# Mange/raingun

Hardware: AMD Instinct MI355X
Metric: Mrays/sec (primary+shadow+secondary) at 3840×2160, depth 5; 1/2/4/8 MI355X (higher is better)
Workload: dtype f64

## Files before the change

include/raingun_debug.h:

```cpp
#ifndef RAINGUN_DEBUG_H
#define RAINGUN_DEBUG_H

#include "raingun.h"

#ifdef __cplusplus
extern "C" {
#endif

rg_status rg_debug_set_path(rg_scene *scene, int32_t path);

typedef struct rg_bvh_info {
    int32_t built;
    int32_t enabled;
    int32_t nodes;
    int32_t leaves;
    int32_t depth;
    float margin;
    float origin_bound;
    int32_t lane_stack;
    int64_t lbuf_bytes;
} rg_bvh_info;
rg_status rg_debug_set_bvh(rg_scene *scene, int32_t enable);
rg_status rg_debug_bvh_info(const rg_scene *scene, rg_bvh_info *info);

rg_status rg_debug_set_lightbuf(rg_scene *scene, int32_t enable);
int32_t rg_debug_lightbuf_count(const rg_scene *scene);

rg_status rg_debug_set_lane_depth(rg_scene *scene, int32_t min_depth);

rg_status rg_debug_set_tile_order(rg_scene *scene, int32_t mode);

rg_status rg_debug_set_image_bands(rg_scene *scene, int32_t bands);

rg_status rg_debug_set_host_split(rg_scene *scene, int32_t pct);

rg_status rg_debug_fail_split_a(rg_scene *scene, int32_t count);

rg_status rg_debug_set_host_ring(rg_scene *scene, int32_t flush_small, int32_t group_small, int32_t flush_big,
                                 int32_t group_big, int32_t multi_light_one);

rg_status rg_debug_set_host_tile_shape(rg_scene *scene, int32_t tile_wlog);

rg_status rg_debug_set_aa_band_rows(rg_scene *scene, int32_t rows);

rg_status rg_debug_set_aa_adaptive_timing(rg_scene *scene, int32_t enable);
rg_status rg_debug_aa_adaptive_info(const rg_scene *scene, float ms[5], uint32_t *flagged, uint32_t *listed_tiles,
                                    uint32_t *bands_launched);

rg_status rg_debug_set_multi(rg_scene *scene, int32_t mode, int32_t stand_in, int32_t bands, int32_t only_rank);

int rg_debug_gather_noop(const void *send, void *recv, size_t count, int datatype, int root, void *comm,
                         void *stream);

rg_status rg_debug_counters(const rg_scene *scene, uint64_t out[16]);

rg_status rg_debug_counter_words(const rg_scene *scene, int32_t first, int32_t n, uint64_t *out);

rg_status rg_debug_last_plain(const rg_scene *scene, int32_t *plain);

rg_status rg_debug_set_exact_div(rg_scene *scene, int32_t enable);
rg_status rg_debug_camera_check(const rg_scene *scene, uint32_t width, uint32_t height, double fov,
                                uint64_t *mismatches, int32_t *admitted);

rg_status rg_debug_unscaled_check(const rg_scene *scene, int32_t op, const double *a, const double *b, uint32_t n,
                                  uint64_t *mismatches);

#ifdef __cplusplus
}
#endif

#endif
```

raingun_amd/_abi.py:

```python
from __future__ import annotations

import ctypes as C
import os
from pathlib import Path

PKG_DIR = Path(__file__).resolve().parent
REPO_DIR = PKG_DIR.parent
LIB_PATH = PKG_DIR / "libraingun_hip.so"

RG_OK = 0
RG_ERR_INVALID_ARGUMENT = -1
RG_ERR_PORTRAIT = -2
RG_ERR_AABB_NORMAL = -3
RG_ERR_NAN_DISTANCE = -4
RG_ERR_TRANSMISSION = -5
RG_ERR_TEXTURE = -6
RG_ERR_DEVICE = -10
RG_ERR_OUT_OF_MEMORY = -11
RG_ERR_CANCELLED = -12
RG_ERR_COLLECTIVE = -13
RG_ERR_PENDING = -14

BODY_SPHERE, BODY_PLANE, BODY_DISK, BODY_AABB = 0, 1, 2, 3
COLORATION_COLOR, COLORATION_TEXTURE = 0, 1
SURFACE_DIFFUSE, SURFACE_REFLECTING, SURFACE_REFRACTIVE = 0, 1, 2
LIGHT_DIRECTIONAL, LIGHT_SPHERICAL = 0, 1


class rg_material(C.Structure):
    _fields_ = [
        ("coloration", C.c_uint32),
        ("color", C.c_float * 3),
        ("texture", C.c_int32),
        ("x_offset", C.c_float),
        ("y_offset", C.c_float),
        ("albedo", C.c_float),
        ("surface", C.c_uint32),
        ("reflectivity", C.c_float),
        ("index", C.c_float),
        ("transparency", C.c_float),
    ]


class rg_body(C.Structure):
    _fields_ = [
        ("kind", C.c_uint32),
        ("_pad", C.c_uint32),
        ("p", C.c_double * 7),
        ("material", rg_material),
    ]


class rg_light(C.Structure):
    _fields_ = [
        ("kind", C.c_uint32),
        ("color", C.c_float * 3),
        ("intensity", C.c_float),
        ("_pad", C.c_uint32),
        ("v", C.c_double * 3),
    ]


class rg_texture(C.Structure):
    _fields_ = [("width", C.c_uint32), ("height", C.c_uint32), ("rgba", C.POINTER(C.c_uint8))]


class rg_scene_desc(C.Structure):
    _fields_ = [
        ("fov", C.c_double),
        ("default_color", C.c_float * 3),
        ("max_recursion_depth", C.c_uint32),
        ("n_bodies", C.c_uint32),
        ("bodies", C.POINTER(rg_body)),
        ("n_lights", C.c_uint32),
        ("lights", C.POINTER(rg_light)),
        ("n_textures", C.c_uint32),
        ("textures", C.POINTER(rg_texture)),
    ]


class rg_ray_counts(C.Structure):
    _fields_ = [("primary", C.c_uint64), ("shadow", C.c_uint64), ("secondary", C.c_uint64)]

    def as_dict(self) -> dict:
        return {"primary": int(self.primary), "shadow": int(self.shadow), "secondary": int(self.secondary)}

    def total(self) -> int:
        return int(self.primary) + int(self.shadow) + int(self.secondary)


class rg_stats(C.Structure):
    _fields_ = [
        ("rays", rg_ray_counts),
        ("kernel_ms", C.c_float),
        ("error_pixel", C.c_int32),
        ("_pad", C.c_uint32),
    ]


class rg_tiling(C.Structure):
    _fields_ = [("tile_rows", C.c_uint32), ("tile_stride", C.c_uint32), ("tile_offset", C.c_uint32)]


class rg_camera(C.Structure):
    _fields_ = [("eye", C.c_double * 3), ("right", C.c_double * 3), ("up", C.c_double * 3),
                ("forward", C.c_double * 3)]


class rg_aov(C.Structure):
    _fields_ = [("body", C.c_void_p), ("depth", C.c_void_p), ("normal", C.c_void_p), ("uv", C.c_void_p),
                ("albedo", C.c_void_p)]


class rg_bvh_info(C.Structure):
    _fields_ = [("built", C.c_int32), ("enabled", C.c_int32), ("nodes", C.c_int32), ("leaves", C.c_int32),
                ("depth", C.c_int32), ("margin", C.c_float), ("origin_bound", C.c_float), ("lane_stack", C.c_int32),
                ("lbuf_bytes", C.c_int64)]


TILE_CALLBACK = C.CFUNCTYPE(C.c_int32, C.c_uint32, C.c_uint32, C.c_uint32, C.POINTER(C.c_uint8), C.c_void_p)

EXPORTED_SYMBOLS = (
    "rg_abi_version",
    "rg_status_string",
    "rg_device_count",
    "rg_scene_create",
    "rg_scene_destroy",
    "rg_scene_set_max_depth",
    "rg_render_image",
    "rg_render_tiles_async",
    "rg_render_tiles_pipelined",
    "rg_render_tiles",
    "rg_tiling_rows",
    "rg_render_stream",
    "rg_trace",
    "rg_host_register",
    "rg_host_unregister",
    "rg_scene_release_stream",
    "rg_stream_status",
    "rg_render_multi",
    "rg_render_image_aa",
    "rg_render_aa_async",
    "rg_resolve_box",
    "rg_render_image_aa_adaptive",
    "rg_render_aa_adaptive",
    "rg_edge_mask",
    "rg_camera_look_at",
    "rg_scene_set_camera",
    "rg_render_aov",
    "rg_render_aov_async",
)
DEBUG_SYMBOLS = ("rg_debug_set_path", "rg_debug_set_bvh", "rg_debug_bvh_info", "rg_debug_counters",
                 "rg_debug_set_lightbuf", "rg_debug_lightbuf_count",
                 "rg_debug_set_tile_order", "rg_debug_set_lane_depth", "rg_debug_set_image_bands", "rg_debug_set_host_split",
                 "rg_debug_fail_split_a", "rg_debug_set_host_ring", "rg_debug_set_host_tile_shape", "rg_debug_set_multi", "rg_debug_gather_noop",
                 "rg_debug_counter_words", "rg_debug_set_aa_band_rows",
                 "rg_debug_set_aa_adaptive_timing", "rg_debug_aa_adaptive_info", "rg_debug_last_plain",
                 "rg_debug_set_exact_div", "rg_debug_camera_check", "rg_debug_unscaled_check")
FRAMES_SYMBOLS = ("rg_frames_create", "rg_frames_destroy", "rg_frames_step", "rg_frames_flush", "rg_frames_image",
                  "rg_frames_read_image", "rg_frames_status", "rg_frames_set_batch", "rg_frames_set_root_tiles", "rg_comm_id_bytes",
                  "rg_comm_unique_id", "rg_comm_init_rank", "rg_comm_info", "rg_comm_destroy", "rg_comm_gather_fn")
PATH_AUTO, PATH_LIGHT, PATH_HEAVY = -1, 0, 1


class RaingunError(RuntimeError):

    def __init__(self, status: int, what: str = ""):
        self.status = status
        msg = status_string(status) if _LIB is not None else str(status)
        super().__init__(f"{what}: {msg} (status {status})" if what else f"{msg} (status {status})")


_LIB: C.CDLL | None = None


def _declare(lib: C.CDLL) -> None:
    P = C.POINTER
    lib.rg_abi_version.restype = C.c_int32
    lib.rg_status_string.restype = C.c_char_p
    lib.rg_status_string.argtypes = [C.c_int32]
    lib.rg_device_count.restype = C.c_int32
    lib.rg_scene_create.restype = C.c_int32
    lib.rg_scene_create.argtypes = [P(rg_scene_desc), C.c_int32, P(C.c_void_p)]
    lib.rg_scene_destroy.restype = None
    lib.rg_scene_destroy.argtypes = [C.c_void_p]
    lib.rg_scene_set_max_depth.restype = C.c_int32
    lib.rg_scene_set_max_depth.argtypes = [C.c_void_p, C.c_uint32]
    lib.rg_camera_look_at.restype = C.c_int32
    lib.rg_camera_look_at.argtypes = [P(C.c_double), P(C.c_double), P(C.c_double), P(rg_camera)]
    lib.rg_scene_set_camera.restype = C.c_int32
    lib.rg_scene_set_camera.argtypes = [C.c_void_p, P(rg_camera)]
    lib.rg_render_image.restype = C.c_int32
    lib.rg_render_image.argtypes = [C.c_void_p, C.c_uint32, C.c_uint32, C.c_void_p, P(rg_stats)]
    lib.rg_render_tiles_async.restype = C.c_int32
    lib.rg_render_tiles_async.argtypes = [C.c_void_p, C.c_uint32, C.c_uint32, P(rg_tiling), C.c_void_p,
                                          C.c_void_p, C.c_void_p, P(rg_stats)]
    if hasattr(lib, "rg_render_tiles_pipelined"):
        lib.rg_render_tiles_pipelined.restype = C.c_int32
        lib.rg_render_tiles_pipelined.argtypes = [C.c_void_p, C.c_uint32, C.c_uint32, P(rg_tiling), C.c_void_p,
                                                  C.c_void_p, C.c_void_p]
    lib.rg_render_tiles.restype = C.c_int32
    lib.rg_render_tiles.argtypes = [C.c_void_p, C.c_uint32, C.c_uint32, P(rg_tiling), C.c_void_p, C.c_void_p,
                                    P(rg_stats)]
    lib.rg_tiling_rows.restype = C.c_uint32
    lib.rg_tiling_rows.argtypes = [C.c_uint32, P(rg_tiling)]
    lib.rg_render_stream.restype = C.c_int32
    lib.rg_render_stream.argtypes = [C.c_void_p, C.c_uint32, C.c_uint32, C.c_uint32, TILE_CALLBACK, C.c_void_p,
                                     P(rg_stats)]
    lib.rg_debug_set_path.restype = C.c_int32
    lib.rg_debug_set_path.argtypes = [C.c_void_p, C.c_int32]
    lib.rg_debug_set_bvh.restype = C.c_int32
    lib.rg_debug_set_bvh.argtypes = [C.c_void_p, C.c_int32]
    if hasattr(lib, "rg_debug_set_lightbuf"):
        lib.rg_debug_set_lightbuf.restype = C.c_int32
        lib.rg_debug_set_lightbuf.argtypes = [C.c_void_p, C.c_int32]
        lib.rg_debug_lightbuf_count.restype = C.c_int32
        lib.rg_debug_lightbuf_count.argtypes = [C.c_void_p]
    lib.rg_debug_bvh_info.restype = C.c_int32
    lib.rg_debug_bvh_info.argtypes = [C.c_void_p, P(rg_bvh_info)]
    lib.rg_debug_set_tile_order.restype = C.c_int32
    lib.rg_debug_set_tile_order.argtypes = [C.c_void_p, C.c_int32]
    lib.rg_debug_set_lane_depth.restype = C.c_int32
    lib.rg_debug_set_lane_depth.argtypes = [C.c_void_p, C.c_int32]
    lib.rg_debug_set_image_bands.restype = C.c_int32
    lib.rg_debug_set_image_bands.argtypes = [C.c_void_p, C.c_int32]
    if hasattr(lib, "rg_debug_set_host_split"):
        lib.rg_debug_set_host_split.restype = C.c_int32
        lib.rg_debug_set_host_split.argtypes = [C.c_void_p, C.c_int32]
    if hasattr(lib, "rg_debug_set_host_ring"):
        lib.rg_debug_set_host_ring.restype = C.c_int32
        lib.rg_debug_set_host_ring.argtypes = [C.c_void_p] + [C.c_int32] * 5
    if hasattr(lib, "rg_debug_fail_split_a"):
        lib.rg_debug_fail_split_a.restype = C.c_int32
        lib.rg_debug_fail_split_a.argtypes = [C.c_void_p, C.c_int32]
    if hasattr(lib, "rg_debug_set_multi"):
        lib.rg_debug_set_multi.restype = C.c_int32
        lib.rg_debug_set_multi.argtypes = [C.c_void_p, C.c_int32, C.c_int32, C.c_int32, C.c_int32]
    if hasattr(lib, "rg_debug_set_host_tile_shape"):
        lib.rg_debug_set_host_tile_shape.restype = C.c_int32
        lib.rg_debug_set_host_tile_shape.argtypes = [C.c_void_p, C.c_int32]
    lib.rg_debug_counters.restype = C.c_int32
    lib.rg_debug_counters.argtypes = [C.c_void_p, P(C.c_uint64)]
    if hasattr(lib, "rg_debug_counter_words"):
        lib.rg_debug_counter_words.restype = C.c_int32
        lib.rg_debug_counter_words.argtypes = [C.c_void_p, C.c_int32, C.c_int32, P(C.c_uint64)]
    if hasattr(lib, "rg_debug_last_plain"):
        lib.rg_debug_last_plain.restype = C.c_int32
        lib.rg_debug_last_plain.argtypes = [C.c_void_p, P(C.c_int32)]
    if hasattr(lib, "rg_debug_set_exact_div"):
        lib.rg_debug_set_exact_div.restype = C.c_int32
        lib.rg_debug_set_exact_div.argtypes = [C.c_void_p, C.c_int32]
        lib.rg_debug_camera_check.restype = C.c_int32
        lib.rg_debug_camera_check.argtypes = [C.c_void_p, C.c_uint32, C.c_uint32, C.c_double, P(C.c_uint64), P(C.c_int32)]
    if hasattr(lib, "rg_debug_unscaled_check"):
        lib.rg_debug_unscaled_check.restype = C.c_int32
        lib.rg_debug_unscaled_check.argtypes = [C.c_void_p, C.c_int32, C.c_void_p, C.c_void_p, C.c_uint32, P(C.c_uint64)]
    lib.rg_frames_create.restype = C.c_int32
    lib.rg_frames_create.argtypes = [C.c_void_p, C.c_uint32, C.c_uint32, C.c_uint32, C.c_int32, C.c_int32,
                                     C.c_int32, C.c_void_p, C.c_void_p, P(C.c_void_p)]
    lib.rg_frames_destroy.restype = None
    lib.rg_frames_destroy.argtypes = [C.c_void_p]
    lib.rg_frames_step.restype = C.c_int32
    lib.rg_frames_step.argtypes = [C.c_void_p]
    lib.rg_frames_flush.restype = C.c_int32
    lib.rg_frames_flush.argtypes = [C.c_void_p]
    lib.rg_frames_image.restype = C.c_void_p
    lib.rg_frames_image.argtypes = [C.c_void_p]
    lib.rg_frames_read_image.restype = C.c_int32
    lib.rg_frames_read_image.argtypes = [C.c_void_p, C.c_void_p]
    lib.rg_trace.restype = C.c_int32
    lib.rg_trace.argtypes = [C.c_void_p, C.c_void_p, C.c_uint32, C.c_void_p, C.c_void_p]
    lib.rg_host_register.restype = C.c_int32
    lib.rg_host_register.argtypes = [C.c_void_p, C.c_size_t]
    lib.rg_host_unregister.restype = C.c_int32
    lib.rg_host_unregister.argtypes = [C.c_void_p]
    lib.rg_scene_release_stream.restype = C.c_int32
    lib.rg_scene_release_stream.argtypes = [C.c_void_p, C.c_void_p]
    lib.rg_stream_status.restype = C.c_int32
    lib.rg_stream_status.argtypes = [C.c_void_p, C.c_void_p, P(C.c_int32)]
    lib.rg_render_multi.restype = C.c_int32
    lib.rg_render_multi.argtypes = [C.c_void_p, C.c_uint32, C.c_uint32, C.c_int32, C.c_uint32, C.c_void_p,
                                    P(rg_stats)]
    if hasattr(lib, "rg_render_image_aa"):
        lib.rg_render_image_aa.restype = C.c_int32
        lib.rg_render_image_aa.argtypes = [C.c_void_p, C.c_uint32, C.c_uint32, C.c_uint32, C.c_void_p, C.c_void_p,
                                           P(rg_stats)]
        lib.rg_render_aa_async.restype = C.c_int32
        lib.rg_render_aa_async.argtypes = [C.c_void_p, C.c_uint32, C.c_uint32, C.c_uint32, C.c_void_p, C.c_void_p,
                                           C.c_void_p, P(rg_stats)]
        lib.rg_resolve_box.restype = C.c_int32
        lib.rg_resolve_box.argtypes = [C.c_int32, C.c_void_p, C.c_uint32, C.c_uint32, C.c_uint32, C.c_void_p,
                                       C.c_void_p]
        lib.rg_debug_set_aa_band_rows.restype = C.c_int32
        lib.rg_debug_set_aa_band_rows.argtypes = [C.c_void_p, C.c_int32]
    if hasattr(lib, "rg_render_image_aa_adaptive"):
        lib.rg_render_image_aa_adaptive.restype = C.c_int32
        lib.rg_render_image_aa_adaptive.argtypes = [C.c_void_p, C.c_uint32, C.c_uint32, C.c_uint32, C.c_uint32,
                                                    C.c_void_p, C.c_void_p, C.c_void_p, P(rg_stats)]
        lib.rg_render_aa_adaptive.restype = C.c_int32
        lib.rg_render_aa_adaptive.argtypes = [C.c_void_p, C.c_uint32, C.c_uint32, C.c_uint32, C.c_uint32, C.c_void_p,
                                              C.c_void_p, C.c_void_p, C.c_void_p, P(rg_stats)]
        lib.rg_debug_set_aa_adaptive_timing.restype = C.c_int32
        lib.rg_debug_set_aa_adaptive_timing.argtypes = [C.c_void_p, C.c_int32]
        lib.rg_debug_aa_adaptive_info.restype = C.c_int32
        lib.rg_debug_aa_adaptive_info.argtypes = [C.c_void_p, P(C.c_float), P(C.c_uint32), P(C.c_uint32), P(C.c_uint32)]
        lib.rg_edge_mask.restype = C.c_int32
        lib.rg_edge_mask.argtypes = [C.c_int32, C.c_void_p, C.c_uint32, C.c_uint32, C.c_uint32, C.c_void_p,
                                     P(C.c_uint32)]
    if hasattr(lib, "rg_render_aov"):
        lib.rg_render_aov.restype = C.c_int32
        lib.rg_render_aov.argtypes = [C.c_void_p, C.c_uint32, C.c_uint32, P(rg_aov), P(rg_stats)]
        lib.rg_render_aov_async.restype = C.c_int32
        lib.rg_render_aov_async.argtypes = [C.c_void_p, C.c_uint32, C.c_uint32, P(rg_tiling), P(rg_aov), C.c_void_p,
                                            P(rg_stats)]
    lib.rg_frames_status.restype = C.c_int32
    lib.rg_frames_status.argtypes = [C.c_void_p, P(C.c_int32)]
    if hasattr(lib, "rg_frames_set_batch"):
        lib.rg_frames_set_batch.restype = C.c_int32
        lib.rg_frames_set_batch.argtypes = [C.c_void_p, C.c_int32]
    if hasattr(lib, "rg_frames_set_root_tiles"):
        lib.rg_frames_set_root_tiles.restype = C.c_int32
        lib.rg_frames_set_root_tiles.argtypes = [C.c_void_p, C.c_int32]
    if hasattr(lib, "rg_comm_init_rank"):
        lib.rg_comm_id_bytes.restype = C.c_int32
        lib.rg_comm_unique_id.restype = C.c_int32
        lib.rg_comm_unique_id.argtypes = [C.c_void_p]
        lib.rg_comm_init_rank.restype = C.c_int32
        lib.rg_comm_init_rank.argtypes = [C.c_void_p, C.c_int32, C.c_int32, C.c_int32, P(C.c_void_p)]
        lib.rg_comm_info.restype = C.c_int32
        lib.rg_comm_info.argtypes = [C.c_void_p, P(C.c_int32), P(C.c_int32), P(C.c_int32)]
        lib.rg_comm_destroy.restype = C.c_int32
        lib.rg_comm_destroy.argtypes = [C.c_void_p]
        lib.rg_comm_gather_fn.restype = C.c_void_p
        lib.rg_comm_gather_fn.argtypes = []


def lib() -> C.CDLL:
    global _LIB
    if _LIB is None:
        path = os.environ.get("RAINGUN_HIP_LIB") or str(LIB_PATH)
        if not Path(path).exists():
            raise RuntimeError(
                f"{path} is missing: build it with `make -C raingun_amd/csrc` (or __graft_entry__.build()). "
                "There is no CPU fallback for the render path.")
        try:
            import torch
        except ImportError:
            pass
        lib_ = C.CDLL(path)
        _declare(lib_)
        _LIB = lib_
    return _LIB


def status_string(status: int) -> str:
    return lib().rg_status_string(int(status)).decode()


def check(status: int, what: str = "") -> None:
    if status != RG_OK:
        raise RaingunError(status, what)


class HostRegistration:

    def __init__(self, arr):
        self.arr = arr
        check(lib().rg_host_register(arr.ctypes.data, arr.nbytes), "rg_host_register")

    def close(self) -> None:
        if self.arr is not None:
            lib().rg_host_unregister(self.arr.ctypes.data)
            self.arr = None

    def __enter__(self):
        return self.arr

    def __exit__(self, *exc):
        self.close()
```

raingun_amd/csrc/rg_aov.hip:

```cpp
#include <hip/hip_runtime.h>

#include "../../include/raingun.h"
#include "rg_aov_kernel.h"
#include "rg_device.h"
#include "rg_internal.h"
#include "rg_launchers.h"

#pragma clang fp contract(off)

#ifndef RG_AOV_TILE_WLOG
#define RG_AOV_TILE_WLOG 5
#endif
#ifndef RG_AOV_BLOCKS_PER_CU
#define RG_AOV_BLOCKS_PER_CU 16
#endif

namespace {

template <bool CAMERA, bool F32F, bool BVH>
hipError_t launch_shade(const RgKernelArgs *a, const RgAovOut *o, dim3 grid, size_t lds, hipStream_t stream) {
    if (o->normal || o->uv || o->albedo)
        hipLaunchKernelGGL((rg_aov_kernel<CAMERA, F32F, BVH, true>), grid, dim3(RG_AOV_BLOCK), lds, stream, *a, *o);
    else
        hipLaunchKernelGGL((rg_aov_kernel<CAMERA, F32F, BVH, false>), grid, dim3(RG_AOV_BLOCK), lds, stream, *a, *o);
    return hipGetLastError();
}

template <bool CAMERA>
hipError_t launch_flavour(const RgKernelArgs *a, const RgAovOut *o, dim3 grid, size_t lds, hipStream_t stream) {
    if (a->n_nodes > 0) return launch_shade<CAMERA, true, true>(a, o, grid, lds, stream);
    if (rg_heavy_path(*a)) return launch_shade<CAMERA, true, false>(a, o, grid, lds, stream);
    return launch_shade<CAMERA, false, false>(a, o, grid, lds, stream);
}

}

extern "C" hipError_t rg_launch_aov(const RgKernelArgs *a, const RgAovOut *o, hipStream_t stream) {
    if (a->out_rows == 0 || a->width == 0 || a->tile_wlog < 3 || a->tile_wlog > 6) return hipErrorInvalidValue;
    int dev = 0, cus = 0;
    hipError_t e = hipGetDevice(&dev);
    if (e == hipSuccess) e = hipDeviceGetAttribute(&cus, hipDeviceAttributeMultiprocessorCount, dev);
    if (e != hipSuccess) return e;
    const unsigned long long ntiles = rg_tile_count(*a), per_block = RG_AOV_BLOCK / 64u;
    const unsigned long long want = (ntiles + per_block - 1ull) / per_block;
    const unsigned long long cap = (unsigned long long)(cus > 0 ? cus : 1) * RG_AOV_BLOCKS_PER_CU;
    const dim3 grid((unsigned)(want < cap ? want : cap));
    const size_t lds = a->lane_stack > 0 ? ((size_t)(a->lane_stack + 1) * 4u) * RG_AOV_BLOCK : 0u;
    return a->camera ? launch_flavour<true>(a, o, grid, lds, stream) : launch_flavour<false>(a, o, grid, lds, stream);
}

namespace {

bool any_layer(const rg_aov *v) { return v->body || v->depth || v->normal || v->uv || v->albedo; }

RgKernelArgs aov_args(const rg_scene *s, rg_launch_ctx *cx, uint32_t W, uint32_t H, const rg_tiling &t, uint32_t rows) {
    RgKernelArgs a = rg_make_args(s);
    a.counters = cx->counters + (size_t)cx->cur * RG_COUNTER_WORDS;
    a.counters_next = cx->counters + (size_t)(1 - cx->cur) * RG_COUNTER_WORDS;
    a.err_sticky = cx->sticky;
    a.width = W;
    a.height = H;
    a.tile_rows = t.tile_rows;
    a.tile_stride = t.tile_stride;
    a.tile_offset = t.tile_offset;
    a.tile_group = 1u;
    a.out_rows = rows;
    a.width_d = (double)W;
    a.height_d = (double)H;
    a.aspect = a.width_d / a.height_d;
    a.tile_wlog = RG_AOV_TILE_WLOG;
    if (s->has_camera) {
        a.camera = 1u;
        for (int k = 0; k < 3; ++k) {
            a.cam_eye[k] = s->camera.eye[k];
            a.cam_right[k] = s->camera.right[k];
            a.cam_up[k] = s->camera.up[k];
            a.cam_forward[k] = s->camera.forward[k];
        }
    }
    return a;
}

}

extern "C" {

rg_status rg_render_aov_async(const rg_scene *s, uint32_t width, uint32_t height, const rg_tiling *tiling,
                              const rg_aov *dev, void *stream, rg_stats *stats) {
    if (!s || !dev || !any_layer(dev) || width == 0 || height == 0 || !tiling || !rg_tiling_valid(tiling))
        return RG_ERR_INVALID_ARGUMENT;
    if (width < height) return RG_ERR_PORTRAIT;
    const uint32_t rows = rg_tiling_rows(height, tiling);
    if ((unsigned long long)rows * width >= (1ull << 32) || (unsigned long long)height * width >= (1ull << 32))
        return RG_ERR_INVALID_ARGUMENT;
    if (!ok(hipSetDevice(s->device))) return RG_ERR_DEVICE;
    hipStream_t st = static_cast<hipStream_t>(stream);
    rg_launch_ctx *cx = rg_ctx_for(s, st);
    if (!cx) return RG_ERR_OUT_OF_MEMORY;
    s->last = cx;
    RgKernelArgs a = aov_args(s, cx, width, height, *tiling, rows);
    const RgAovOut o{dev->body, dev->depth, dev->normal, dev->uv, dev->albedo};
    cx->last_counters = a.counters;
    cx->last_plain = 0;
    if (stats && !ok(hipEventRecord(cx->ev0, st))) return RG_ERR_DEVICE;
    if (rows > 0) {
        if (!ok(rg_launch_aov(&a, &o, st))) return RG_ERR_DEVICE;
        cx->cur = 1 - cx->cur;
    }
    if (!stats) return RG_OK;
    unsigned long long c[4];
    if (!ok(hipEventRecord(cx->ev1, st)) ||
        !ok(hipMemcpyAsync(c, a.counters, sizeof c, hipMemcpyDeviceToHost, st)) || !ok(hipStreamSynchronize(st)))
        return RG_ERR_DEVICE;
    float ms = 0.0f;
    (void)hipEventElapsedTime(&ms, cx->ev0, cx->ev1);
    stats->kernel_ms = ms;
    return rg_snap_status(c, stats);
}

rg_status rg_render_aov(const rg_scene *s, uint32_t width, uint32_t height, const rg_aov *out, rg_stats *stats) {
    if (!s || !out || !any_layer(out) || width == 0 || height == 0) return RG_ERR_INVALID_ARGUMENT;
    if (width < height) return RG_ERR_PORTRAIT;
    const unsigned long long npx = (unsigned long long)width * height;
    if (npx >= (1ull << 32)) return RG_ERR_INVALID_ARGUMENT;
    if (!ok(hipSetDevice(s->device))) return RG_ERR_DEVICE;
    void *const host[5] = {out->body, out->depth, out->normal, out->uv, out->albedo};
    const size_t px_bytes[5] = {4, 8, 12, 8, 12};
    void *d[5] = {nullptr, nullptr, nullptr, nullptr, nullptr};
    rg_status st = RG_OK;
    for (int k = 0; k < 5 && st == RG_OK; ++k)
        if (host[k] && !ok(hipMalloc(&d[k], (size_t)npx * px_bytes[k]))) {
            (void)hipGetLastError();
            st = RG_ERR_OUT_OF_MEMORY;
        }
    if (st == RG_OK) {
        const rg_aov dev{static_cast<int32_t *>(d[0]), static_cast<double *>(d[1]), static_cast<float *>(d[2]),
                         static_cast<float *>(d[3]), static_cast<float *>(d[4])};
        const rg_tiling whole = {height, 1, 0};
        rg_stats local;
        st = rg_render_aov_async(s, width, height, &whole, &dev, nullptr, stats ? stats : &local);
        if (st == RG_OK || st == RG_ERR_AABB_NORMAL || st == RG_ERR_NAN_DISTANCE)
            for (int k = 0; k < 5; ++k)
                if (host[k] && !ok(hipMemcpy(host[k], d[k], (size_t)npx * px_bytes[k], hipMemcpyDeviceToHost)))
                    st = RG_ERR_DEVICE;
    }
    for (int k = 0; k < 5; ++k)
        if (d[k]) (void)hipFree(d[k]);
    return st;
}

}
```

raingun_amd/csrc/rg_capi.hip:

```cpp
#include <hip/hip_runtime.h>

#include <algorithm>
#include <cstring>

#include "../../include/raingun.h"
#include "../../include/raingun_debug.h"
#include "rg_device.h"
#include "rg_exact.h"
#include "rg_internal.h"
#include "rg_launchers.h"

#pragma clang fp contract(off)

#ifndef RG_LANE_MIN_DEPTH
#define RG_LANE_MIN_DEPTH 1
#endif

void rg_image_res_release(rg_image_res &r) {
    rg_bands_release(r);
    if (r.h_frame) (void)hipHostFree(r.h_frame);
    if (r.h_flags) (void)hipHostFree(r.h_flags);
    if (r.h_cancel) (void)hipHostFree(r.h_cancel);
    r = rg_image_res{};
}
// ... 286 lines not shown

rg_status rg_render_stream(const rg_scene *s, uint32_t width, uint32_t height, uint32_t tile_rows,
                           rg_tile_callback on_tile, void *user, rg_stats *stats) {
    if (!s || !on_tile || width == 0 || height == 0 || tile_rows == 0) return RG_ERR_INVALID_ARGUMENT;
    if (width < height) return RG_ERR_PORTRAIT;
    if ((unsigned long long)height * width >= (1ull << 32)) return RG_ERR_INVALID_ARGUMENT;
    if (!ok(hipSetDevice(s->device))) return RG_ERR_DEVICE;
    rg_status st = ensure_image_res(s, 1);
    if (st != RG_OK) return st;
    rg_image_res &r = s->img;
    const size_t row4 = (size_t)width * 4, bytes = (size_t)height * row4;
    const uint32_t wl = (uint32_t)s->host_tile_wlog;
    const auto [TH, tiles_x, grid_rows, ntiles] = host_tile_grid(width, height, wl);
    (void)grid_rows;
    size_t cancel_cap = r.h_cancel ? 64 : 0;
    if ((st = rg_grow(RG_MEM_PINNED_ZEROED, r.h_frame, r.h_frame_cap, bytes + 4)) != RG_OK ||
        (st = rg_grow(RG_MEM_PINNED_ZEROED, r.h_flags, r.h_flags_cap, (ntiles + 1) * 4)) != RG_OK ||
        (st = rg_grow(RG_MEM_PINNED_ZEROED, r.h_cancel, cancel_cap, 64)) != RG_OK)
        return st;
    void *frame_dev = rg_host_device_ptr(r.h_frame, bytes);
    uint32_t *flags_dev = static_cast<uint32_t *>(rg_host_device_ptr(r.h_flags, ntiles * 4 + 4));
    const uint32_t *cancel_dev = static_cast<const uint32_t *>(rg_host_device_ptr(r.h_cancel, 4));
    if (!frame_dev || !flags_dev || !cancel_dev) return RG_ERR_DEVICE;
    __atomic_store_n(r.h_cancel, 0u, __ATOMIC_RELEASE);
    if (++r.seq == 0) r.seq = 1;
    const uint32_t seq = r.seq;
    hipStream_t rs = r.rs[0];
    const rg_tiling whole = {height, 1, 0};
    if (!ok(hipEventRecord(r.ev_t0, rs))) return RG_ERR_DEVICE;
    rg_launch_desc d = frame_launch(width, height, whole, frame_dev, rs, r.h_snap);
    d.tile_flags = flags_dev;
    d.frame_seq = seq;
    d.cancel = cancel_dev;
    d.tile_wlog = wl;
    d.host_frame = true;
    st = rg_launch_tiles(s, d);
    if (st != RG_OK) return rg_bands_drain(r, st);
    if (!ok(hipEventRecord(r.ev_t1, rs))) return rg_bands_drain(r, RG_ERR_DEVICE);
    const uint8_t *frame = static_cast<const uint8_t *>(r.h_frame);
    for (uint32_t y0 = 0; y0 < height; y0 += tile_rows) {
        const uint32_t n = std::min(tile_rows, height - y0);
        if ((st = wait_tiles(r.h_flags, (size_t)(y0 / TH) * tiles_x, ((size_t)(y0 + n) + TH - 1u) / TH * tiles_x, seq,
                             r.ev_t1)) != RG_OK)
            break;
        if (on_tile(y0, n, width, frame + (size_t)y0 * row4, user) != 0) {
            __atomic_store_n(r.h_cancel, 1u, __ATOMIC_RELEASE);
            st = RG_ERR_CANCELLED;
            break;
        }
    }
    if (!ok(hipStreamSynchronize(rs))) return rg_bands_drain(r, RG_ERR_DEVICE);
    const rg_status err = rg_finish_stats(r.h_snap, 1, r.ev_t0, r.ev_t1, stats);
    if (st == RG_OK && err != RG_OK) return err;
    return st;
}

rg_status rg_debug_set_path(rg_scene *s, int32_t path) {
    if (!s || path < RG_PATH_AUTO || path > RG_PATH_HEAVY) return RG_ERR_INVALID_ARGUMENT;
    s->path = path;
    return RG_OK;
}

rg_status rg_debug_set_bvh(rg_scene *s, int32_t enable) {
    if (!s || (enable != 0 && enable != 1)) return RG_ERR_INVALID_ARGUMENT;
    s->bvh_enabled = enable != 0;
    return RG_OK;
}

rg_status rg_debug_set_lightbuf(rg_scene *s, int32_t enable) {
    if (!s || (enable != 0 && enable != 1)) return RG_ERR_INVALID_ARGUMENT;
    s->lbuf_enabled = enable != 0;
    return RG_OK;
}

int32_t rg_debug_lightbuf_count(const rg_scene *s) {
    if (!s || !s->host || !s->bvh_enabled || !s->lbuf_enabled || s->n_nodes == 0) return 0;
    int32_t n = 0;
    for (int32_t i = 0; i < s->n_lbuf; ++i) n += s->host->lbuf[(size_t)i].kind != RG_LB_NONE;
    return n;
}

rg_status rg_debug_bvh_info(const rg_scene *s, rg_bvh_info *info) {
    if (!s || !info) return RG_ERR_INVALID_ARGUMENT;
    *info = s->bvh_info;
    info->enabled = s->bvh_enabled && s->n_nodes > 0;
    return RG_OK;
}

rg_status rg_debug_set_lane_depth(rg_scene *s, int32_t min_depth) {
    if (!s) return RG_ERR_INVALID_ARGUMENT;
    s->lane_min_depth = min_depth < 0 ? RG_LANE_MIN_DEPTH : min_depth;
    return RG_OK;
}

rg_status rg_debug_set_tile_order(rg_scene *s, int32_t mode) {
    if (!s || mode < -1 || mode > 1) return RG_ERR_INVALID_ARGUMENT;
    s->tile_order = mode;
    return RG_OK;
}

rg_status rg_debug_set_image_bands(rg_scene *s, int32_t bands) {
    if (!s || bands < -2 || bands > RG_IMAGE_MAX_BANDS) return RG_ERR_INVALID_ARGUMENT;
    s->image_bands = bands;
    return RG_OK;
}

rg_status rg_debug_set_host_split(rg_scene *s, int32_t pct) {
    if (!s || pct < 0 || pct > 99) return RG_ERR_INVALID_ARGUMENT;
    s->host_split_pct = pct;
    return RG_OK;
}

rg_status rg_debug_set_host_ring(rg_scene *s, int32_t flush_small, int32_t group_small, int32_t flush_big,
                                  int32_t group_big, int32_t multi_light_one) {
    if (!s || flush_small < -1 || flush_small > 16 || group_small < -1 || flush_big < -1 || flush_big > 16 ||
        group_big < -1 || multi_light_one < -1 || multi_light_one > 1)
        return RG_ERR_INVALID_ARGUMENT;
    if (flush_small >= 0) s->ring_flush_small = flush_small;
    if (group_small >= 0) s->ring_group_small = group_small;
    if (flush_big >= 0) s->ring_flush_big = flush_big;
    if (group_big >= 0) s->ring_group_big = group_big;
    if (multi_light_one >= 0) s->multi_light_one = multi_light_one != 0;
    return RG_OK;
}

rg_status rg_debug_fail_split_a(rg_scene *s, int32_t count) {
    if (!s || count < 0) return RG_ERR_INVALID_ARGUMENT;
    s->split_fail_a = count;
    return RG_OK;
}

rg_status rg_debug_set_host_tile_shape(rg_scene *s, int32_t tile_wlog) {
    if (!s || !(tile_wlog == 0 || (tile_wlog >= 3 && tile_wlog <= 6))) return RG_ERR_INVALID_ARGUMENT;
    s->host_tile_wlog = tile_wlog == 0 ? RG_HOST_TILE_WLOG : tile_wlog;
    s->host_tile_forced = tile_wlog != 0;
    return RG_OK;
}

rg_status rg_debug_counters(const rg_scene *s, uint64_t out[16]) {
    if (!s || !out) return RG_ERR_INVALID_ARGUMENT;
    if (!ok(hipSetDevice(s->device))) return RG_ERR_DEVICE;
    if (!ok(hipStreamSynchronize(s->last->stream)) ||
        !ok(hipMemcpy(out, s->last->last_counters, 16 * sizeof(uint64_t), hipMemcpyDeviceToHost)))
        return RG_ERR_DEVICE;
    return RG_OK;
}

rg_status rg_debug_last_plain(const rg_scene *s, int32_t *plain) {
    if (!s || !plain || !s->last) return RG_ERR_INVALID_ARGUMENT;
    *plain = s->last->last_plain;
    return RG_OK;
}

rg_status rg_debug_set_exact_div(rg_scene *s, int32_t enable) {
    if (!s || (enable != 0 && enable != 1)) return RG_ERR_INVALID_ARGUMENT;
    s->exact_div = enable != 0;
    return RG_OK;
}

rg_status rg_debug_camera_check(const rg_scene *s, uint32_t width, uint32_t height, double fov, uint64_t *mismatches,
                                int32_t *admitted) {
    if (!s || !mismatches || width == 0 || height == 0 || (unsigned long long)width * height >= (1ull << 32))
        return RG_ERR_INVALID_ARGUMENT;
    if (!ok(hipSetDevice(s->device))) return RG_ERR_DEVICE;
    RgKernelArgs a = rg_make_args(s);
    a.width = width;
    a.height = height;
    a.width_d = (double)width;
    a.height_d = (double)height;
    a.aspect = a.width_d / a.height_d;
    a.fov_adjustment = rg_fov_adjustment(fov);
    a.inv_w = 1.0 / a.width_d;
    a.inv_h = 1.0 / a.height_d;
    if (admitted)
        *admitted = rg_recip_div_ok(width) && rg_recip_div_ok(height) && rg_camera_unscaled_ok(a.fov_adjustment, a.aspect);
    unsigned long long *d_bad = nullptr, bad = 0;
    if (!ok(hipMalloc(&d_bad, sizeof bad))) return RG_ERR_OUT_OF_MEMORY;
    rg_status st = RG_OK;
    if (!ok(hipMemset(d_bad, 0, sizeof bad)) || !ok(rg_launch_camera_check(&a, d_bad, nullptr)) ||
        !ok(hipMemcpy(&bad, d_bad, sizeof bad, hipMemcpyDeviceToHost)))
        st = RG_ERR_DEVICE;
    (void)hipFree(d_bad);
    *mismatches = bad;
    return st;
}

rg_status rg_debug_unscaled_check(const rg_scene *s, int32_t op, const double *a, const double *b, uint32_t n,
                                  uint64_t *mismatches) {
    if (!s || !a || !mismatches || n == 0 || n > (1u << 24) || op < 0 || op > 3 || (op == 2 && !b))
        return RG_ERR_INVALID_ARGUMENT;
    if (!ok(hipSetDevice(s->device))) return RG_ERR_DEVICE;
    const size_t bytes = (size_t)n * sizeof(double);
    double *d_a = nullptr, *d_b = nullptr, *d_out = nullptr;
    unsigned long long *d_bad = nullptr, bad = 0;
    rg_status st = RG_OK;
    if (!ok(hipMalloc(&d_a, bytes)) || (op == 2 && !ok(hipMalloc(&d_b, bytes))) || !ok(hipMalloc(&d_out, 2 * bytes)) ||
        !ok(hipMalloc(&d_bad, sizeof bad)))
        st = RG_ERR_OUT_OF_MEMORY;
    else if (!ok(hipMemcpy(d_a, a, bytes, hipMemcpyHostToDevice)) ||
             (op == 2 && !ok(hipMemcpy(d_b, b, bytes, hipMemcpyHostToDevice))) || !ok(hipMemset(d_out, 0, 2 * bytes)) ||
             !ok(hipMemset(d_bad, 0, sizeof bad)) || !ok(rg_launch_unscaled_check(op, d_a, d_b, n, d_out, d_bad, nullptr)) ||
             !ok(hipMemcpy(&bad, d_bad, sizeof bad, hipMemcpyDeviceToHost)))
        st = RG_ERR_DEVICE;
    (void)hipFree(d_a);
    (void)hipFree(d_b);
    (void)hipFree(d_out);
    (void)hipFree(d_bad);
    *mismatches = bad;
    return st;
}

rg_status rg_debug_counter_words(const rg_scene *s, int32_t first, int32_t n, uint64_t *out) {
    if (!s || !out || first < 0 || n < 0 || first + n > RG_COUNTER_WORDS) return RG_ERR_INVALID_ARGUMENT;
    if (!ok(hipSetDevice(s->device))) return RG_ERR_DEVICE;
    if (!ok(hipStreamSynchronize(s->last->stream)) ||
        !ok(hipMemcpy(out, s->last->last_counters + first, (size_t)n * sizeof(uint64_t), hipMemcpyDeviceToHost)))
        return RG_ERR_DEVICE;
    return RG_OK;
}

rg_status rg_trace(const rg_scene *s, const double *rays, uint32_t n, double *dist, int32_t *body) {
    if (!s || (n && (!rays || !dist || !body))) return RG_ERR_INVALID_ARGUMENT;
    if (n == 0) return RG_OK;
    if (!ok(hipSetDevice(s->device))) return RG_ERR_DEVICE;
    void *d_rays = nullptr, *d_dist = nullptr, *d_body = nullptr;
    rg_status st = RG_OK;
    if (!ok(hipMalloc(&d_rays, (size_t)n * 48)) || !ok(hipMalloc(&d_dist, (size_t)n * 8)) ||
        !ok(hipMalloc(&d_body, (size_t)n * 4)))
        st = RG_ERR_OUT_OF_MEMORY;
    rg_launch_ctx *cx = rg_ctx_for(s, nullptr);
    if (!cx) st = RG_ERR_OUT_OF_MEMORY;
    RgKernelArgs a = rg_make_args(s);
    unsigned long long c[4] = {0, 0, 0, 0};
    unsigned long long *cs = cx ? cx->counters + (size_t)cx->cur * RG_COUNTER_WORDS : nullptr;
    if (st == RG_OK) { s->last = cx; a.counters = cs; }
    if (st == RG_OK && (!ok(hipMemcpy(d_rays, rays, (size_t)n * 48, hipMemcpyHostToDevice)) ||
                        !ok(hipMemset(cs, 0, sizeof c)) ||
                        !ok(rg_launch_trace(&a, (const double *)d_rays, n, (double *)d_dist, (int32_t *)d_body, nullptr)) ||
                        !ok(hipMemcpy(dist, d_dist, (size_t)n * 8, hipMemcpyDeviceToHost)) ||
                        !ok(hipMemcpy(body, d_body, (size_t)n * 4, hipMemcpyDeviceToHost)) ||
                        !ok(hipMemcpy(c, cs, sizeof c, hipMemcpyDeviceToHost)) ||
                        !ok(hipMemset(cs, 0, RG_COUNTER_WORDS * sizeof(unsigned long long)))))
        st = RG_ERR_DEVICE;
    if (d_rays) (void)hipFree(d_rays);
    if (d_dist) (void)hipFree(d_dist);
    if (d_body) (void)hipFree(d_body);
    if (st == RG_OK && c[3] != 0) st = rg_snap_status(c, nullptr);
    return st;
}

}
```

raingun_amd/csrc/rg_device.h:

```cpp
#pragma once
#include <stdint.h>

#if !defined(__HIP__) && !defined(__HIPCC__)
#define __device__
#define __host__
#define __forceinline__ inline
#endif

#ifdef __HIP_DEVICE_COMPILE__
#define RG_CONST __attribute__((address_space(4)))
#else
#define RG_CONST
#endif
template <class T>
__device__ __forceinline__ const RG_CONST T *rg_cptr(const T *p) { return (const RG_CONST T *)p; }

struct alignas(16) RgSph { double cx, cy, cz, r2; };
struct alignas(16) RgSphF { float cx, cy, cz, r2hi; };
struct alignas(16) RgSphF2 { float cchi, thrp, cc32; int32_t id; };
struct alignas(16) RgPln { double ox, oy, oz, nx, ny, nz, on, pad; };
struct alignas(16) RgDsk { double ox, oy, oz, nx, ny, nz, r, on; };
struct alignas(16) RgBox { double lo[3], hi[3]; };

struct alignas(16) RgBvhNode {
    float lox[4], loy[4], loz[4], hix[4], hiy[4], hiz[4];
    int32_t child[4];
    int32_t nchild;
    int32_t pad[3];
};

#define RG_LANE_NODE_BITS 12
#define RG_LANE_STACK_MAX 16

struct RgBodyDev {
    int32_t kind;
    int32_t pad;
    double p[7];
};

struct RgMatDev {
    int32_t coloration;
    float color[3];
    int32_t tex;
    float xoff, yoff;
    float albedo_pi;
    int32_t surface;
    float reflectivity;
    float index;
    float transparency;
};

struct RgLightDev {
    int32_t kind;
    float color[3];
    float intensity;
    int32_t pad;
    double v[3];
    double dn[3];
    double pad2;
};

struct RgLightBufDev;

struct RgTexDev {
    const uint32_t *texels;
    int32_t w, h;
};

struct RgTexMagic {
    uint32_t mw, shw, mh, shh;
};
struct RgPlnAxes {
    double xa[3], ya[3];
};

struct RgKernelArgs {
    const RgSph *sph;
    const double *sph_cc;
    const RgSphF *sphf;
    const RgSphF2 *sphf2;
    const int32_t *sph_id;
    const RgPln *pln;
    const int32_t *pln_id;
    const RgDsk *dsk;
    const int32_t *dsk_id;
    const RgBox *box;
    const int32_t *box_id;
    int32_t n_sph, n_pln, n_dsk, n_box;
    const RgBvhNode *nodes;
    int32_t n_nodes;
    int32_t lane_stack;
    int32_t lane_min_depth;
    float bvh_obound;
    double bvh_rbound;
    double bvh_margin;
    double bvh_extent;
    const RgBodyDev *bodies;
    const RgMatDev *mats;
    const RgLightDev *lights;
    const RgTexDev *texs;
    int32_t n_bodies, n_lights, n_textures;
    uint32_t lds_lstack_bytes;
    uint32_t lds_sphf, lds_sph, lds_cc, lds_nodes, lds_pln, lds_dsk, lds_box, lds_bodies, lds_mats, lds_lights, lds_texs, lds_hot_bytes, lds_total_bytes;
    int32_t path;
    uint32_t width, height;
    uint32_t tile_rows, tile_stride, tile_offset, out_rows;
    uint32_t tile_group;
    uint32_t tile_base;
    double fov_adjustment;
    double aspect;
    float def[3];
    uint32_t max_depth;
    uint32_t *rgba;
    float *rgb;
    const uint32_t *tile_perm;
    unsigned long long *counters;
    unsigned long long *counters_next;
    void *deep_stack;
    uint32_t deep_stride;
    int32_t nan_scene;
    unsigned long long *err_sticky;
    uint32_t *tile_flags;
    uint32_t frame_seq;
    const uint32_t *cancel;
    uint32_t tile_wlog;
    uint32_t defer_px;
    const double *prim_sx, *prim_sy;
    uint32_t pipelined;
    double width_d, height_d;
    unsigned long long *snap_out;
    uint32_t max_grid_threads;
    uint32_t image_rows;
    uint32_t out_tile_mul, out_tile_add;
    const void *lds_blob;
    const RgLightBufDev *lbuf;
    const uint32_t *lb_start;
    const uint32_t *lb_ent;
    int32_t n_lbuf;
    int32_t lb_cam;
    uint32_t lds_lbuf;
    uint32_t ring_flush, ring_group;
    const uint8_t *px_mask;
    uint32_t tile_limit, px_k, px_w;
    uint32_t plain_veto;
    double inv_w, inv_h;
    uint32_t tiles_x_m, tiles_x_sh, tile_rows_shift, tile_rows_m, tile_rows_sh, rows_identity;
    uint32_t lds_texm, lds_axes, lds_plain_bytes;
    uint32_t camera;
    double cam_eye[3], cam_right[3], cam_up[3], cam_forward[3];
};

__host__ __device__ inline uint32_t rg_tile_w(const RgKernelArgs &a) { return 1u << a.tile_wlog; }
__host__ __device__ inline uint32_t rg_tile_h(const RgKernelArgs &a) { return 64u >> a.tile_wlog; }
__host__ __device__ inline uint32_t rg_tiles_x(const RgKernelArgs &a) { return (a.width + rg_tile_w(a) - 1u) >> a.tile_wlog; }
__host__ __device__ inline uint32_t rg_tiles_y(const RgKernelArgs &a) { return (a.out_rows + rg_tile_h(a) - 1u) / rg_tile_h(a); }
__host__ __device__ inline unsigned long long rg_tile_count(const RgKernelArgs &a) {
    return (unsigned long long)rg_tiles_x(a) * rg_tiles_y(a);
}

#define RG_FRAME_BYTES 88

#ifndef RG_RING_FLUSH_SMALL
#define RG_RING_FLUSH_SMALL 4
#endif
#ifndef RG_RING_GROUP_SMALL
#define RG_RING_GROUP_SMALL 1
#endif
#ifndef RG_RING_FLUSH_BIG
#define RG_RING_FLUSH_BIG 8
#endif
#ifndef RG_RING_GROUP_BIG
#define RG_RING_GROUP_BIG 8
#endif
#ifndef RG_RING_BIG_TILES
#define RG_RING_BIG_TILES 50000u
#endif
#ifndef RG_MULTI_LIGHT_ONE
#define RG_MULTI_LIGHT_ONE 1
#endif
#ifndef RG_LB
#define RG_LB 3
#endif
#ifndef RG_LB_SMALL
#define RG_LB_SMALL 2
#endif
#ifndef RG_LB_ONE
#define RG_LB_ONE 1
#endif
#ifndef RG_HEAVY_WPS
#define RG_HEAVY_WPS 3
#endif
#define RG_BVH_MAX_WAVES 16
#ifndef RG_HEAVY_SCENE_BODIES
#define RG_HEAVY_SCENE_BODIES 32
#endif

#define RG_PATH_AUTO -1
#define RG_PATH_LIGHT 0
#define RG_PATH_HEAVY 1

__host__ __device__ __forceinline__ bool rg_heavy_path(const RgKernelArgs &a) {
    bool heavy = a.n_sph + a.n_pln + a.n_dsk + a.n_box >= RG_HEAVY_SCENE_BODIES;
    if (a.path != RG_PATH_AUTO) heavy = a.path == RG_PATH_HEAVY;
    if (a.n_lights > RG_LB) heavy = true;
    return heavy;
}

#define RG_COUNTER_WORDS (16 + 16 * 16 + 16)
#define RG_DONE_WORD (16 + 16 * 16)
```

raingun_amd/csrc/rg_internal.h:

```cpp
#pragma once
#include <hip/hip_runtime.h>

#include <cstddef>
#include <cstring>
#include <initializer_list>
#include <memory>
#include <vector>

#include "../../include/raingun.h"
#include "../../include/raingun_debug.h"
#include "rg_bands.h"
#include "rg_copy_pool.h"
#include "rg_device.h"
#include "rg_lightbuf_ray.h"
#include "rg_tile_deal.h"

inline bool ok(hipError_t e) { return e == hipSuccess; }

struct rg_launch_ctx {
    hipStream_t stream = nullptr;
    unsigned long long *counters = nullptr;
    int cur = 0;
    unsigned long long *last_counters = nullptr;
    int last_plain = 0;
    unsigned long long *sticky = nullptr;
    uint32_t *tile_cost = nullptr, *tile_perm = nullptr;
    size_t tile_cap = 0;
    struct PermKey {
        uint32_t width, height, tile_rows, tile_stride, tile_offset, tile_base, out_rows, tile_wlog, max_depth, n_lights,
            tile_group;
        double fov;
        const void *mats;
        bool camera = false;
        double cam[12] = {};
        bool operator==(const PermKey &o) const {
            if (camera != o.camera || std::memcmp(cam, o.cam, sizeof cam) != 0) return false;
            return width == o.width && height == o.height && tile_rows == o.tile_rows && tile_stride == o.tile_stride &&
                   tile_offset == o.tile_offset && tile_base == o.tile_base && out_rows == o.out_rows &&
                   tile_group == o.tile_group &&
                   tile_wlog == o.tile_wlog && max_depth == o.max_depth &&
                   n_lights == o.n_lights && fov == o.fov && mats == o.mats;
        }
    };
    bool perm_valid = false;
    PermKey perm_key{};
    void *deep = nullptr;
    size_t deep_bytes = 0;
    double *prim = nullptr;
    size_t prim_cap = 0;
    uint32_t prim_w = 0, prim_h = 0;
    double prim_fov = 0.0;
    uint32_t rdiv_w = 0, rdiv_h = 0;
    bool rdiv_ok = false;
    hipEvent_t ev0 = nullptr, ev1 = nullptr;
};

#ifndef RG_IMAGE_STREAM_CUMASK
#define RG_IMAGE_STREAM_CUMASK 1
#endif
#ifndef RG_HOST_TILE_WLOG_LIGHT
#define RG_HOST_TILE_WLOG_LIGHT 6
#endif
#ifndef RG_HOST_TILE_WLOG
#define RG_HOST_TILE_WLOG 4
#endif
struct rg_image_res : rg_band_res {
    void *h_frame = nullptr;
    size_t h_frame_cap = 0;
    uint32_t *h_flags = nullptr;
    size_t h_flags_cap = 0;
    uint32_t seq = 0;
    uint32_t *h_cancel = nullptr;
};

#define RG_AA_MAX_SAMPLES 8
struct rg_aa_res : rg_band_res {
    hipEvent_t ev_fork = nullptr;
    void *slot_rgba[2] = {nullptr, nullptr};
    void *slot_rgb[2] = {nullptr, nullptr};
    size_t slot_cap[2] = {0, 0};
    hipStream_t base_stream = nullptr;
    hipEvent_t ev_list = nullptr;
    uint8_t *d_mask = nullptr;
    size_t d_mask_cap = 0;
    uint32_t *d_list = nullptr;
    size_t d_list_cap = 0;
    uint32_t *d_counts = nullptr;
    size_t d_counts_cap = 0;
    uint32_t *h_counts = nullptr;
    size_t h_counts_cap = 0;
    bool timing = false;
    std::vector<hipEvent_t> ev_mark;
    size_t n_marks = 0;
    float pass_ms[5] = {0, 0, 0, 0, 0};
    uint32_t flagged = 0, listed_tiles = 0, bands_launched = 0;
};

struct rg_host_tables {
    std::vector<RgSph> sph;
    std::vector<RgSphF> sphf;
    std::vector<RgSphF2> sphf2;
    std::vector<double> sph_cc;
    std::vector<int32_t> sph_id, pln_id, dsk_id, box_id;
    std::vector<RgPln> pln;
    std::vector<RgDsk> dsk;
    std::vector<RgBox> box;
    std::vector<RgBodyDev> bodies;
    std::vector<RgMatDev> mats;
    std::vector<RgLightDev> lights;
    std::vector<RgBvhNode> nodes;
    std::vector<RgLightBufDev> lbuf;
    std::vector<uint32_t> lb_start, lb_ent;
    std::vector<uint32_t> tex_w, tex_h;
    std::vector<std::vector<uint32_t>> texels;
};

struct rg_multi_res;
struct rg_frames;

struct rg_scene {
    int device = 0;
    double fov = 90.0;
    float def[3] = {0, 0, 0};
    uint32_t max_depth = 10;
    int32_t n_sph = 0, n_pln = 0, n_dsk = 0, n_box = 0, n_bodies = 0, n_lights = 0, n_textures = 0;
    bool nan_scene = false;
    std::vector<void *> allocations;
    RgSph *sph = nullptr;
    double *sph_cc = nullptr;
    RgSphF *sphf = nullptr;
    RgSphF2 *sphf2 = nullptr;
    int32_t path = RG_PATH_AUTO;
    int32_t *sph_id = nullptr, *pln_id = nullptr, *dsk_id = nullptr, *box_id = nullptr;
    RgPln *pln = nullptr;
    RgDsk *dsk = nullptr;
    RgBox *box = nullptr;
    RgBodyDev *bodies = nullptr;
    RgMatDev *mats = nullptr;
    RgLightDev *lights = nullptr;
    RgTexDev *texs = nullptr;
    RgBvhNode *nodes = nullptr;
    int32_t n_nodes = 0;
    int32_t lane_stack = 0;
    int32_t lane_min_depth = 1;
    bool bvh_enabled = true;
    RgLightBufDev *lbuf = nullptr;
    uint32_t *lb_start = nullptr, *lb_ent = nullptr;
    int32_t n_lbuf = 0;
    int32_t lb_cam = -1;
    int32_t n_lbdesc = 0;
    bool lbuf_enabled = true;
    bool exact_div = true;
    bool has_camera = false;
    rg_camera camera{};
    float bvh_obound = 0.0f;
    double bvh_rbound = 0.0, bvh_margin = 0.0, bvh_extent = 0.0;
    rg_bvh_info bvh_info{};
    int tile_order = -1;
    int image_bands = 0;
    int host_split_pct = 0;
    mutable int split_fail_a = 0;
    int ring_flush_small = RG_RING_FLUSH_SMALL, ring_group_small = RG_RING_GROUP_SMALL;
    int ring_flush_big = RG_RING_FLUSH_BIG, ring_group_big = RG_RING_GROUP_BIG;
    bool multi_light_one = RG_MULTI_LIGHT_ONE != 0;
    int host_tile_wlog = RG_HOST_TILE_WLOG;
    bool host_tile_forced = false;
    int multi_mode = 0;
    bool multi_stand_in = false;
    int multi_bands = 0;
    int multi_only_rank = -1;
    std::shared_ptr<const rg_host_tables> host;
    std::vector<RgTexDev> tex_desc;
    void *lds_blob = nullptr;
    uint32_t lds_blob_layout[14] = {};
    mutable std::vector<rg_launch_ctx *> ctxs;
    mutable rg_launch_ctx *last = nullptr;
    mutable rg_image_res img;
    int aa_band_rows = 0;
    mutable rg_aa_res aa;
    mutable rg_multi_res *multi = nullptr;
    mutable std::vector<rg_frames *> frames;
};

void rg_frames_detach_scene(rg_frames *f);

RgKernelArgs rg_make_args(const rg_scene *s);

struct rg_launch_desc {
    uint32_t width = 0, height = 0;
    rg_tiling tiling{};
    uint8_t *rgba = nullptr;
    float *rgb = nullptr;
    hipStream_t stream = nullptr;
    unsigned long long *snap = nullptr;
    bool timed = false;
    uint32_t *tile_flags = nullptr;
    uint32_t frame_seq = 0;
    const uint32_t *cancel = nullptr;
    uint32_t tile_wlog = 3;
    bool host_frame = false;
    bool pipelined = false;
    bool image_rows = false;
    uint32_t tile_first = 0, tile_count = 0xFFFFFFFFu;
    uint32_t tile_group = 1;
    const uint32_t *tile_list = nullptr;
    uint32_t tile_limit = 0;
    const uint8_t *px_mask = nullptr;
    uint32_t px_k = 1, px_w = 0;
};

rg_status rg_launch_tiles(const rg_scene *s, const rg_launch_desc &d, rg_launch_ctx **ctx_out = nullptr);

rg_status rg_snap_status(const unsigned long long *snap, rg_stats *stats);

rg_status rg_render_host(const rg_scene *s, uint32_t width, uint32_t height, const rg_tiling *tiling,
                         uint8_t *rgba_out, float *rgb_out, rg_stats *stats);

bool rg_host_is_pinned(const void *p, size_t bytes);
void *rg_host_device_ptr(void *p, size_t bytes);

rg_status rg_scene_replica(const rg_scene *src, int32_t device, rg_scene **out);
void rg_scene_free(rg_scene *s);
void rg_sync_settings(rg_scene *dst, const rg_scene *src);

void rg_multi_release(const rg_scene *s);

#pragma GCC visibility push(hidden)

rg_launch_ctx *rg_ctx_for(const rg_scene *s, hipStream_t stream);
void rg_ctx_destroy(rg_launch_ctx *c);

enum rg_mem { RG_MEM_DEVICE, RG_MEM_PINNED, RG_MEM_PINNED_ZEROED };
struct rg_grow_buf {
    void **p;
    size_t bytes;
    template <class T>
    rg_grow_buf(T *&q, size_t n) : p(reinterpret_cast<void **>(&q)), bytes(n) {}
};
rg_status rg_grow(rg_mem kind, size_t &cap, size_t want, std::initializer_list<rg_grow_buf> bufs,
                  bool clear_error = true);
template <class T>
rg_status rg_grow(rg_mem kind, T *&p, size_t &cap, size_t bytes) {
    return rg_grow(kind, cap, bytes, {{p, bytes}});
}

double rg_fov_adjustment(double fov);
bool rg_scene_heavy(const rg_scene *s);
const void *rg_lds_blob_for(const rg_scene *s, const RgKernelArgs &a);

uint32_t rg_host_tile_wlog(const rg_scene *s);
void rg_image_res_release(rg_image_res &r);
void rg_aa_res_release(rg_aa_res &r);

hipError_t rg_launch_pack_rgb(const void *rgba, void *rgb, size_t npx, hipStream_t stream);
hipError_t rg_launch_reinterleave(const void *gathered, const void *root_part, void *image, uint32_t width,
                                  uint32_t height, uint32_t tile_rows, uint32_t world, size_t slot_bytes,
                                  hipStream_t stream, uint32_t root = 1);

#pragma GCC visibility pop
```

raingun_amd/csrc/rg_k_trace.h:

```cpp
#pragma once
#include <hip/hip_runtime.h>

#include "rg_bvh_ray.h"
#include "rg_device.h"
#include "rg_k_bvh.h"
#include "rg_k_intersect.h"
#include "rg_k_math.h"

#pragma clang fp contract(off)

namespace rgk {

template <bool F32F, bool BVH, bool NODB = false, class Src>
__device__ __forceinline__ void trace_primary(const RgKernelArgs &a, const Src &src, V3 d, Closest &c) {
    if constexpr (!BVH) sph_primary<F32F>(a, src, d, c);
    [[maybe_unused]] LbRange cam{0u, 0u, false};
    if constexpr (BVH) {
        if (a.lb_cam >= 0) cam = lbuf_begin(a, src, a.lb_cam, d, 0.0, 0.0, 0.0);
    }
    for (int i = 0; i < a.n_pln; ++i) {
        RG_REGION(RGR_PRIM_PLANE);
        const RgPln p = src.getp(i);
        double den = (p.nx * d.x + p.ny * d.y) + p.nz * d.z;
        if (den > 1e-6) {
            RG_REGION(RGR_PRIM_PLANE_DIV);
            double dist = p.on / den;
            if (dist >= 0.0) closest_add(c, dist, rg_cptr(a.pln_id)[i]);
        }
    }
    [[maybe_unused]] const V3 o = v3(0.0, 0.0, 0.0);
    if constexpr (!NODB) {
    for (int i = 0; i < a.n_dsk; ++i) {
        RG_REGION(RGR_DISK);
        const RgDsk k = src.getd(i);
        double t;
        if (disk_hit(k, o, d, t)) closest_add(c, t, rg_cptr(a.dsk_id)[i]);
    }
    if (a.n_box > 0) {
        RG_REGION(RGR_BOX);
        V3 inv = v3(1.0 / d.x, 1.0 / d.y, 1.0 / d.z);
        int sx = inv.x < 0.0, sy = inv.y < 0.0, sz = inv.z < 0.0;
        for (int i = 0; i < a.n_box; ++i) {
            RG_REGION(RGR_BOX);
            const RgBox b = src.getb(i);
            double t;
            if (aabb_hit(b, o, inv, sx, sy, sz, t)) closest_add(c, t, rg_cptr(a.box_id)[i]);
        }
    }
    }
    if constexpr (BVH) {
        const bool ok = !c.nan && rg_bvh_ray_ok(a.bvh_obound, 0.0, 0.0, 0.0, d.x, d.y, d.z);
        RG_STAT(8, RG_LANES(!ok));
        if (!ok) {
            [[maybe_unused]] const unsigned long long t0 = RG_CLOCK();
            sph_primary<F32F>(a, src, d, c);
            RG_STAT(13, RG_CLOCK() - t0);
        }
        const bool walk = ok && !cam.use;
        if (ok && cam.use) cambuf_primary(a, src, cam, d, (float)d.x, (float)d.y, (float)d.z, c);
        if (walk) {
            bool need = true, unused = false;
            bvh_spheres<0>(a, src, o, d, false, 0.0, 0.0, c, unused, need);
        }
    }
}

template <bool F32F, bool BVH, bool NODB = false, class Src>
__device__ __forceinline__ void trace_query(const RgKernelArgs &a, const Src &src, const Ray &r, bool shadow, double ld,
                                            Closest &c, bool &occl, bool lane_walk = false, int light = -1) {
    const V3 o = r.o, d = r.d;
    bool need = true;
    if constexpr (!BVH) {
        if (!sph_query<F32F>(a, src, o, d, shadow, ld, c, occl, need)) return;
    }
    [[maybe_unused]] LbRange lbr{0u, 0u, false};
    if constexpr (BVH) {
        if (shadow && light >= 0 && light < a.n_lbuf) {
            const V3 lp = lbuf_light_pos(src, light);
            lbr = lbuf_begin(a, src, light, o, lp.x, lp.y, lp.z);
        }
    }
    for (int i = 0; i < a.n_pln; ++i) {
        const RgPln p = src.getp(i);
        double den = (p.nx * d.x + p.ny * d.y) + p.nz * d.z;
        RG_REGION(RGR_QC_PLANE);
        if (den > 1e-6 && need) {
            double vx = p.ox - o.x, vy = p.oy - o.y, vz = p.oz - o.z;
            double dist = ((vx * p.nx + vy * p.ny) + vz * p.nz) / den;
            if (dist >= 0.0) {
                if (shadow) {
                    if (!(dist > ld)) { occl = true; need = false; }
                } else {
                    closest_add(c, dist, rg_cptr(a.pln_id)[i]);
                }
            }
        }
    }
    if constexpr (NODB && !BVH) return;
    if (!__any(need)) return;
    if constexpr (!NODB) {
    for (int i = 0; i < a.n_dsk; ++i) {
        RG_REGION(RGR_DISK);
        const RgDsk k = src.getd(i);
        double t;
        if (need && disk_hit(k, o, d, t)) {
            if (shadow) {
                if (!(t > ld)) { occl = true; need = false; }
            } else {
                closest_add(c, t, rg_cptr(a.dsk_id)[i]);
            }
        }
    }
    if (a.n_box > 0 && __any(need)) {
        RG_REGION(RGR_BOX);
        V3 inv = v3(1.0 / d.x, 1.0 / d.y, 1.0 / d.z);
        int sx = inv.x < 0.0, sy = inv.y < 0.0, sz = inv.z < 0.0;
        for (int i = 0; i < a.n_box; ++i) {
            RG_REGION(RGR_BOX);
            const RgBox b = src.getb(i);
            double t;
            if (need && aabb_hit(b, o, inv, sx, sy, sz, t)) {
                if (shadow) {
                    if (!(t > ld)) { occl = true; need = false; }
                } else {
                    closest_add(c, t, rg_cptr(a.box_id)[i]);
                }
            }
        }
    }
    }
    if constexpr (BVH) {
        if (!__any(need)) return;
        double t0s = 0.0;
        float grow = 0.0f;
        const int cls = (need && !c.nan) ? rg_bvh_classify(a.bvh_obound, a.bvh_rbound, a.bvh_margin, a.bvh_extent,
                                                           o.x, o.y, o.z, d.x, d.y, d.z, t0s, grow)
                                         : RG_BVH_SCAN;
        const bool lb = shadow && need && cls == RG_BVH_TRAVERSE && grow == 0.0f && lbr.use;
        if (lb) lbuf_shadow(a, src, light, lbr, o, d, ld, occl, need);
        const bool ok = need && cls == RG_BVH_TRAVERSE && !lb;
#ifdef RG_BVH_STATS
        {
            RG_STAT(8, RG_LANES(need && cls == RG_BVH_SCAN));
            RG_STAT(9, RG_LANES(need && cls == RG_BVH_TRAVERSE && grow > 0.0f));
            RG_STAT(10, RG_LANES(need && cls == RG_BVH_NO_SPHERE));
            RG_STAT(11, RG_LANES(need && c.nan));
        }
#endif
        if (need && cls == RG_BVH_SCAN) {
            [[maybe_unused]] const unsigned long long t0 = RG_CLOCK();
            bool nd = true;
            sph_query<F32F>(a, src, o, d, shadow, ld, c, occl, nd);
            RG_STAT(13, RG_CLOCK() - t0);
        }
        const bool grown = ok && grow > 0.0f;
        const bool per_lane = ok && !grown && a.lane_stack > 0 && __any(ok && !grown && lane_walk);
        if (per_lane) bvh_lane(a, src, o, d, shadow, ld, t0s, c, occl, need);
        if (ok && !grown && !per_lane) {
            bvh_spheres<1>(a, src, o, d, shadow, ld, t0s, c, occl, need);
        }
        if (grown) {
            bvh_spheres<1, true>(a, src, o, d, shadow, ld, t0s, c, occl, need, grow);
        }
    }
}

__device__ __forceinline__ bool ray_exotic(V3 o, V3 d) {
    const bool ok = fabs(o.x) < 1e100 && fabs(o.y) < 1e100 && fabs(o.z) < 1e100 && fabs(d.x) < 1e50 &&
                    fabs(d.y) < 1e50 && fabs(d.z) < 1e50;
    return !ok;
}

#ifndef RG_SHADOW_GROUP
#define RG_SHADOW_GROUP 2
#endif

template <int LB>
struct ShadowBatch {
    V3 d[LB];
    double ld[LB];
};

template <int LB, bool NODB = false, class Src>
__device__ __forceinline__ void trace_shadow(const RgKernelArgs &a, const Src &src, V3 o, const ShadowBatch<LB> &sb,
                                             uint32_t full, uint32_t &occl) {
    constexpr int G = RG_SHADOW_GROUP;
    const int n = a.n_sph, nfull = n - n % G;
    for (int i = 0; i < n;) {
        const int g = i < nfull ? G : 1;
        RG_REGION(RGR_SH_GROUP);
        RgSph s[G];
        double hx[G], hy[G], hz[G], hh[G], adj[G][LB], opp[G][LB];
        bool cand[G][LB];
        bool any = false;
#pragma unroll
        for (int k = 0; k < G; ++k) {
            if (k < g) {
                s[k] = src.get(i + k);
                hx[k] = s[k].cx - o.x; hy[k] = s[k].cy - o.y; hz[k] = s[k].cz - o.z;
                hh[k] = (hx[k] * hx[k] + hy[k] * hy[k]) + hz[k] * hz[k];
#pragma unroll
                for (int l = 0; l < LB; ++l) {
                    adj[k][l] = (hx[k] * sb.d[l].x + hy[k] * sb.d[l].y) + hz[k] * sb.d[l].z;
                    opp[k][l] = hh[k] - adj[k][l] * adj[k][l];
                    cand[k][l] = !(opp[k][l] > s[k].r2) && !((occl >> l) & 1u);
                    any |= cand[k][l];
                }
            }
        }
        if (any) {
            RG_REGION(RGR_SH_TAIL);
#pragma unroll
            for (int k = 0; k < G; ++k) {
#pragma unroll
                for (int l = 0; l < LB; ++l) {
                    double t;
#ifdef RG_REGION_STATS
                    if (k < g && cand[k][l]) RG_REGION(RGR_SH_PAIR);
#endif
                    if (k < g && cand[k][l] && sphere_tail(s[k].r2, opp[k][l], adj[k][l], t) && !(t > sb.ld[l]))
                        occl |= 1u << l;
                }
            }
        }
        i += g;
        if ((i & 7) == 0 && !__any(occl != full)) return;
    }
    if (!__any(occl != full)) return;
    for (int i = 0; i < a.n_pln; ++i) {
        const RgPln p = src.getp(i);
        const double vx = p.ox - o.x, vy = p.oy - o.y, vz = p.oz - o.z;
        const double num = (vx * p.nx + vy * p.ny) + vz * p.nz;
        RG_REGION(RGR_SH_PLANE);
#pragma unroll
        for (int l = 0; l < LB; ++l) {
            const double den = (p.nx * sb.d[l].x + p.ny * sb.d[l].y) + p.nz * sb.d[l].z;
            if (den > 1e-6 && !((occl >> l) & 1u)) {
                bool hit;
                if (sb.ld[l] == __builtin_inf() && num >= 0.0) {
                    hit = true;
                } else {
                    RG_REGION(RGR_SH_PLANE_DIV);
                    const double dist = num / den;
                    hit = dist >= 0.0 && !(dist > sb.ld[l]);
                }
                if (hit) occl |= 1u << l;
            }
        }
    }
    if constexpr (NODB) return;
    if (!__any(occl != full)) return;
    for (int i = 0; i < a.n_dsk; ++i) {
        RG_REGION(RGR_DISK);
        const RgDsk k = src.getd(i);
#pragma unroll
        for (int l = 0; l < LB; ++l) {
            double t;
            if (!((occl >> l) & 1u) && disk_hit(k, o, sb.d[l], t) && !(t > sb.ld[l])) occl |= 1u << l;
        }
    }
    if (a.n_box > 0 && __any(occl != full)) {
        RG_REGION(RGR_BOX);
#pragma unroll
        for (int l = 0; l < LB; ++l) {
            const V3 d = sb.d[l];
            const V3 inv = v3(1.0 / d.x, 1.0 / d.y, 1.0 / d.z);
            const int sx = inv.x < 0.0, sy = inv.y < 0.0, sz = inv.z < 0.0;
            for (int i = 0; i < a.n_box; ++i) {
                RG_REGION(RGR_BOX);
                const RgBox b = src.getb(i);
                double t;
                if (!((occl >> l) & 1u) && aabb_hit(b, o, inv, sx, sy, sz, t) && !(t > sb.ld[l])) occl |= 1u << l;
            }
        }
    }
}

}
```

raingun_amd/csrc/rg_launch.hip:

```cpp
#include <hip/hip_runtime.h>

#include <algorithm>
#include <cstddef>
#include <cstring>
#include <new>
#include <vector>

#include "../../include/raingun.h"
#include "../../include/raingun_debug.h"
#include "rg_device.h"
#include "rg_exact.h"
#include "rg_internal.h"
#include "rg_launchers.h"

#pragma clang fp contract(off)

namespace {

int frames_needed(uint32_t max_depth) { return max_depth > 1 ? (int)max_depth - 1 : 1; }

rg_status decode_error(unsigned long long word, int32_t *pixel) {
    if (word == 0) return RG_OK;
    const unsigned long long key = ~word;
    if (pixel) *pixel = (int32_t)(key >> 8);
// ... 28 lines not shown
    a.counters_next = cx->counters + (size_t)(1 - cx->cur) * RG_COUNTER_WORDS;
    a.err_sticky = cx->sticky;
    a.width = d.width;
    a.height = d.height;
    a.tile_rows = d.tiling.tile_rows;
    a.tile_stride = d.tiling.tile_stride;
    a.tile_offset = d.tiling.tile_offset;
    a.tile_group = d.tile_group;
    a.tile_base = d.tile_first;
    a.out_rows = out_rows;
    a.aspect = (double)d.width / (double)d.height;
    a.width_d = (double)d.width;
    a.height_d = (double)d.height;
    if (cx->rdiv_w != d.width || cx->rdiv_h != d.height) {
        cx->rdiv_ok = rg_recip_div_ok(d.width) && rg_recip_div_ok(d.height);
        cx->rdiv_w = d.width;
        cx->rdiv_h = d.height;
    }
    a.inv_w = 1.0 / a.width_d;
    a.inv_h = 1.0 / a.height_d;
    a.plain_veto = (cx->rdiv_ok && s->exact_div) ? 0u : 1u;
    if (s->has_camera) {
        a.camera = 1u;
        for (int k = 0; k < 3; ++k) {
            a.cam_eye[k] = s->camera.eye[k];
            a.cam_right[k] = s->camera.right[k];
            a.cam_up[k] = s->camera.up[k];
            a.cam_forward[k] = s->camera.forward[k];
        }
        a.plain_veto |= 4u;
    }
    a.rgba = reinterpret_cast<uint32_t *>(d.rgba);
    a.rgb = d.rgb;
    a.tile_flags = d.tile_flags;
    a.frame_seq = d.frame_seq;
    a.cancel = d.cancel;
    a.tile_wlog = d.tile_wlog;
    a.defer_px = d.host_frame ? 1u : 0u;
    a.image_rows = d.image_rows ? 1u : 0u;
    a.pipelined = d.pipelined ? 1u : 0u;
    if (d.px_mask) {
        a.px_mask = d.px_mask;
        a.px_k = d.px_k;
        a.px_w = d.px_w;
        a.tile_perm = d.tile_list;
        a.tile_limit = d.tile_limit;
    }
    if (d.host_frame) {
        const bool big = rg_tile_count(a) >= RG_RING_BIG_TILES;
        a.ring_flush = (uint32_t)std::max(0, big ? s->ring_flush_big : s->ring_flush_small);
        a.ring_group = (uint32_t)std::max(0, big ? s->ring_group_big : s->ring_group_small);
    }
    const RgMagicU32 mx = rg_magic_u32(rg_tiles_x(a)), mr = rg_magic_u32(a.tile_rows);
    a.tiles_x_m = mx.m;
    a.tiles_x_sh = mx.sh;
    a.tile_rows_m = mr.m;
    a.tile_rows_sh = mr.sh;
    a.tile_rows_shift = 32u;
    for (uint32_t k = 0; k < 32u; ++k)
        if (a.tile_rows == 1u << k) a.tile_rows_shift = k;
    a.rows_identity = (a.tile_stride == 1u && a.tile_offset == 0u && a.tile_base == 0u && a.tile_group <= 1u &&
                       a.out_tile_mul <= 1u)
                          ? 1u
                          : 0u;
    return a;
}

rg_status size_deep_frames(rg_launch_ctx *cx, RgKernelArgs &a, int frames, int disp) {
    if (!rg_launch_global_frames(&a, disp) || a.out_rows == 0) return RG_OK;
    size_t threads = 0;
    if (!ok(rg_render_grid_threads(&a, disp, &threads)) || threads == 0 || threads > 0xFFFFFFFFull)
        return RG_ERR_DEVICE;
    const size_t per_thread = (size_t)frames * RG_FRAME_BYTES;
    if (threads * per_thread > ((size_t)1 << 30)) {
        size_t free_b = 0, total_b = 0;
        if (!ok(hipMemGetInfo(&free_b, &total_b))) return RG_ERR_DEVICE;
        const size_t budget = std::min<size_t>(free_b / 2, (size_t)16 << 30);
        if (threads * per_thread > budget) {
            a.max_grid_threads = (uint32_t)std::min<size_t>(budget / per_thread, 0xFFFFFFFFu);
            if (!ok(rg_render_grid_threads(&a, disp, &threads)) || threads == 0) return RG_ERR_DEVICE;
            if (threads * per_thread > budget) return RG_ERR_OUT_OF_MEMORY;
        }
    }
    const rg_status st = rg_grow(RG_MEM_DEVICE, cx->deep, cx->deep_bytes, threads * per_thread);
    if (st != RG_OK) return st;
    a.deep_stack = cx->deep;
    a.deep_stride = (uint32_t)threads;
    return RG_OK;
}

rg_status refresh_prim_table(rg_launch_ctx *cx, RgKernelArgs &a, hipStream_t st) {
    const uint32_t width = a.width, height = a.height;
    if (cx->prim_w != width || cx->prim_h != height || cx->prim_fov != a.fov_adjustment || !cx->prim) {
        const size_t n = (size_t)width + height;
        const rg_status g = rg_grow(RG_MEM_DEVICE, cx->prim, cx->prim_cap, n * sizeof(double));
        if (g != RG_OK) return g;
        std::vector<double> tab(n);
        for (uint32_t x = 0; x < width; ++x)
            tab[x] = ((((double)x + 0.5) / (double)width) * 2.0 - 1.0) * a.aspect * a.fov_adjustment;
        for (uint32_t y = 0; y < height; ++y)
            tab[(size_t)width + y] = (1.0 - (((double)y + 0.5) / (double)height) * 2.0) * a.fov_adjustment;
        if (!ok(hipMemcpyAsync(cx->prim, tab.data(), n * sizeof(double), hipMemcpyHostToDevice, st)) ||
            !ok(hipStreamSynchronize(st)))
            return RG_ERR_DEVICE;
        cx->prim_w = width;
        cx->prim_h = height;
        cx->prim_fov = a.fov_adjustment;
    }
    a.prim_sx = cx->prim;
    a.prim_sy = cx->prim + width;
    return RG_OK;
}

rg_status order_tiles(const rg_scene *s, const rg_launch_desc &d, rg_launch_ctx *cx, RgKernelArgs &a) {
    if (!(s->tile_order == 1 || (s->tile_order < 0 && rg_heavy_path(a)))) return RG_OK;
    const size_t ntiles = (size_t)rg_tile_count(a);
    rg_launch_ctx::PermKey key{d.width, d.height, d.tiling.tile_rows, d.tiling.tile_stride,
                               d.tiling.tile_offset, d.tile_first, a.out_rows, d.tile_wlog, s->max_depth,
                               (uint32_t)s->n_lights, d.tile_group, a.fov_adjustment, s->mats};
    key.camera = a.camera != 0;
    for (int k = 0; key.camera && k < 3; ++k) {
        key.cam[k] = a.cam_eye[k];
        key.cam[3 + k] = a.cam_right[k];
        key.cam[6 + k] = a.cam_up[k];
        key.cam[9 + k] = a.cam_forward[k];
    }
    const bool cached = cx->perm_valid && cx->perm_key == key;
    if (!cached && rg_grow(RG_MEM_DEVICE, cx->tile_cap, ntiles,
                           {{cx->tile_cost, rg_tile_order_scratch_words((uint32_t)ntiles) * 4},
                            {cx->tile_perm, ntiles * 4}},
                           false) != RG_OK)
        return RG_ERR_OUT_OF_MEMORY;
    if (ntiles == 0) return RG_OK;
    if (!cached) {
        cx->perm_valid = false;
        if (!ok(rg_launch_tile_order(&a, cx->tile_cost, cx->tile_perm, d.stream))) return RG_ERR_DEVICE;
        cx->perm_valid = true;
        cx->perm_key = key;
    }
    a.tile_perm = cx->tile_perm;
    return RG_OK;
}

rg_status launch_and_snapshot(const rg_launch_desc &d, rg_launch_ctx *cx, RgKernelArgs &a, int disp) {
    hipStream_t st = d.stream;
    cx->last_counters = a.counters;
    unsigned long long *snap_dev =
        (d.snap && a.out_rows > 0)
            ? static_cast<unsigned long long *>(rg_host_device_ptr(d.snap, 4 * sizeof(*d.snap)))
            : nullptr;
    a.snap_out = snap_dev;
    if (a.out_rows > 0) {
        if (!ok(rg_launch_render(&a, disp, st, &cx->last_plain))) return RG_ERR_DEVICE;
        cx->cur = 1 - cx->cur;
    }
    if (d.timed && !ok(hipEventRecord(cx->ev1, st))) return RG_ERR_DEVICE;
    if (d.snap && !snap_dev &&
        !ok(hipMemcpyAsync(d.snap, a.counters, 4 * sizeof(unsigned long long), hipMemcpyDeviceToHost, st)))
        return RG_ERR_DEVICE;
    return RG_OK;
}

rg_launch_desc device_frame(uint32_t width, uint32_t height, const rg_tiling *tiling, uint8_t *rgba_dev,
                            float *rgb_dev, hipStream_t stream) {
    rg_launch_desc d;
    d.width = width;
    d.height = height;
    d.tiling = tiling ? *tiling : rg_tiling{};
    d.rgba = rgba_dev;
    d.rgb = rgb_dev;
    d.stream = stream;
    return d;
}

}

void rg_ctx_destroy(rg_launch_ctx *c) {
    if (c->counters) (void)hipFree(c->counters);
    if (c->sticky) (void)hipFree(c->sticky);
    if (c->tile_cost) (void)hipFree(c->tile_cost);
    if (c->tile_perm) (void)hipFree(c->tile_perm);
    if (c->deep) (void)hipFree(c->deep);
    if (c->prim) (void)hipFree(c->prim);
    if (c->ev0) (void)hipEventDestroy(c->ev0);
    if (c->ev1) (void)hipEventDestroy(c->ev1);
    delete c;
}

rg_launch_ctx *rg_ctx_for(const rg_scene *s, hipStream_t stream) {
    for (rg_launch_ctx *c : s->ctxs)
        if (c->stream == stream) return c;
    rg_launch_ctx *c = new (std::nothrow) rg_launch_ctx();
    if (!c) return nullptr;
    c->stream = stream;
    void *p = nullptr, *q = nullptr;
    if (!ok(hipMalloc(&p, 2 * RG_COUNTER_WORDS * sizeof(unsigned long long)))) { delete c; return nullptr; }
    c->counters = static_cast<unsigned long long *>(p);
    c->last_counters = c->counters;
    if (!ok(hipMemsetAsync(p, 0, 2 * RG_COUNTER_WORDS * sizeof(unsigned long long), stream))) {
        rg_ctx_destroy(c);
        return nullptr;
    }
    if (!ok(hipMalloc(&q, sizeof(unsigned long long))) || !ok(hipMemsetAsync(q, 0, sizeof(unsigned long long), stream))) {
        if (q) (void)hipFree(q);
        rg_ctx_destroy(c);
        return nullptr;
    }
    c->sticky = static_cast<unsigned long long *>(q);
    if (!ok(hipEventCreate(&c->ev0)) || !ok(hipEventCreate(&c->ev1))) {
        rg_ctx_destroy(c);
        return nullptr;
    }
    s->ctxs.push_back(c);
    return c;
}

rg_status rg_grow(rg_mem kind, size_t &cap, size_t want, std::initializer_list<rg_grow_buf> bufs, bool clear_error) {
    if (want <= cap) return RG_OK;
    for (const rg_grow_buf &b : bufs)
        if (*b.p) (void)(kind == RG_MEM_DEVICE ? hipFree(*b.p) : hipHostFree(*b.p));
    for (const rg_grow_buf &b : bufs) *b.p = nullptr;
    cap = 0;
    for (const rg_grow_buf &b : bufs) {
        void *q = nullptr;
        const hipError_t e = kind == RG_MEM_DEVICE   ? hipMalloc(&q, b.bytes)
                             : kind == RG_MEM_PINNED ? hipHostMalloc(&q, b.bytes, hipHostMallocDefault)
                                                     : hipHostMalloc(&q, b.bytes, hipHostMallocCoherent);
        if (!ok(e)) {
            if (clear_error) (void)hipGetLastError();
            return RG_ERR_OUT_OF_MEMORY;
        }
        if (kind == RG_MEM_PINNED_ZEROED) std::memset(q, 0, b.bytes);
        *b.p = q;
    }
    cap = want;
    return RG_OK;
}

rg_status rg_launch_tiles(const rg_scene *s, const rg_launch_desc &d, rg_launch_ctx **ctx_out) {
    uint32_t out_rows = 0;
    rg_status st = validate(s, d, &out_rows);
    if (st != RG_OK) return st;
    if (!ok(hipSetDevice(s->device))) return RG_ERR_DEVICE;
    rg_launch_ctx *cx = rg_ctx_for(s, d.stream);
    if (!cx) return RG_ERR_OUT_OF_MEMORY;
    s->last = cx;
    if (ctx_out) *ctx_out = cx;
    RgKernelArgs a = fill_args(s, d, cx, out_rows);
    const int frames = frames_needed(s->max_depth);
    const bool host_arrays = frames <= rg_host_array_frames() && rg_heavy_path(a);
    const int disp = ((d.host_frame && !host_arrays) || d.px_mask) ? std::max(frames, rg_max_array_frames() + 1) : frames;
    if ((st = size_deep_frames(cx, a, frames, disp)) != RG_OK) return st;
    if ((st = refresh_prim_table(cx, a, d.stream)) != RG_OK) return st;
    if (!rg_heavy_path(a)) {
        a.lds_blob = rg_lds_blob_for(s, a);
        if (!a.lds_blob) a.plain_veto |= 2u;
    }
    if (d.timed && !ok(hipEventRecord(cx->ev0, d.stream))) return RG_ERR_DEVICE;
    if (!d.px_mask && (st = order_tiles(s, d, cx, a)) != RG_OK) return st;
    return launch_and_snapshot(d, cx, a, disp);
}

rg_status rg_snap_status(const unsigned long long *snap, rg_stats *stats) {
    if (stats) {
        stats->rays.primary = snap[0];
        stats->rays.shadow = snap[1];
        stats->rays.secondary = snap[2];
        stats->error_pixel = -1;
    }
    return decode_error(snap[3], stats ? &stats->error_pixel : nullptr);
}

extern "C" {

uint32_t rg_tiling_rows(uint32_t height, const rg_tiling *t) { return rg_tiling_rows_grouped(height, t, 1); }

rg_status rg_scene_release_stream(rg_scene *s, void *stream) {
    if (!s) return RG_ERR_INVALID_ARGUMENT;
    hipStream_t hs = static_cast<hipStream_t>(stream);
    if (!hs) return RG_OK;
    if (!ok(hipSetDevice(s->device))) return RG_ERR_DEVICE;
    for (size_t i = 0; i < s->ctxs.size(); ++i) {
        if (s->ctxs[i]->stream != hs) continue;
        rg_launch_ctx *c = s->ctxs[i];
        (void)hipStreamSynchronize(hs);
        if (s->last == c) s->last = rg_ctx_for(s, nullptr);
        s->ctxs.erase(s->ctxs.begin() + (std::ptrdiff_t)i);
        rg_ctx_destroy(c);
        break;
    }
    return RG_OK;
}

rg_status rg_stream_status(const rg_scene *s, void *stream, int32_t *error_pixel) {
    if (!s) return RG_ERR_INVALID_ARGUMENT;
    if (error_pixel) *error_pixel = -1;
    if (!ok(hipSetDevice(s->device))) return RG_ERR_DEVICE;
    hipStream_t hs = static_cast<hipStream_t>(stream);
    for (rg_launch_ctx *c : s->ctxs) {
        if (c->stream != hs) continue;
        unsigned long long w = 0;
        if (!ok(hipStreamSynchronize(hs)) || !ok(hipMemcpy(&w, c->sticky, sizeof w, hipMemcpyDeviceToHost)) ||
            !ok(hipMemset(c->sticky, 0, sizeof w)))
            return RG_ERR_DEVICE;
        return decode_error(w, error_pixel);
    }
// ... 29 lines not shown
```

raingun_amd/csrc/rg_render_kernel.h:

```cpp
#pragma once
#include <hip/hip_runtime.h>

#include "../../include/raingun.h"
#include "rg_camera.h"
#include "rg_device.h"
#include "rg_k_bvh.h"
#include "rg_k_diag.h"
#include "rg_k_frames.h"
#include "rg_k_intersect.h"
#include "rg_k_math.h"
#include "rg_k_pool.h"
#include "rg_k_shade.h"
#include "rg_k_trace.h"
#include "rg_render_cfg.h"

#pragma clang fp contract(off)

using namespace rgk;

#ifndef RG_NQ
#define RG_NQ 8
#endif
#define RG_QUEUE_BASE 16
#define RG_QUEUE_STRIDE 16
#ifndef RG_PLAIN_CAMERA
#define RG_PLAIN_CAMERA 1
#endif
#ifndef RG_PLAIN_TILE
#define RG_PLAIN_TILE 1
#endif

struct Cold {
    const RgBodyDev *bodies;
    const RgMatDev *mats;
    const RgLightDev *lights;
    const RgTexDev *texs;
};

__device__ __forceinline__ void stage16(unsigned char *dst, const void *src, uint32_t bytes) {
    uint4 *d = reinterpret_cast<uint4 *>(dst);
    const uint4 *g = reinterpret_cast<const uint4 *>(src);
    for (uint32_t k = threadIdx.x; k < bytes / 16u; k += blockDim.x) d[k] = g[k];
}

template <int MAXD, bool LSPH, bool LCOLD, int WPS, int LBT, bool F32F, bool BVH, bool TASKS, int TPW = 0,
          bool HF = false, bool SPARSE = false, bool PLAIN = false>
__global__ __launch_bounds__(64 * rg_block_waves(LBT, WPS), rg_min_waves_per_eu(LBT, WPS))
void rg_render_kernel(RgKernelArgs a) {
    using K = RenderCfg<MAXD, LSPH, LCOLD, WPS, LBT, F32F, BVH, TASKS, TPW, HF, SPARSE, PLAIN>;
    constexpr int LB = K::lights_per_batch;
    constexpr bool UL = PLAIN && RG_PLAIN_ULIGHT != 0;
#ifdef RG_WAVE_TIMES
    const unsigned long long t_wave0 = wall_clock64();
    uint32_t wt_tiles = 0;
#endif
    const int n_lights = PLAIN ? LB : a.n_lights;
    const bool nan_scene = PLAIN ? false : a.nan_scene != 0;
    float *const out_rgb = PLAIN ? nullptr : a.rgb;
    const uint32_t *const tile_perm = PLAIN ? nullptr : a.tile_perm;
    if (blockIdx.x == 0 && a.counters_next)
        for (uint32_t k = threadIdx.x; k < RG_COUNTER_WORDS; k += blockDim.x) a.counters_next[k] = 0ull;
    extern __shared__ __attribute__((aligned(16))) unsigned char smem[];
    typename std::conditional<LSPH, SphLds, typename std::conditional<K::lds_nodes_only, SphNodesLds, SphScalar>::type>::type src;
    Cold T;
    const bool blob = K::light && LSPH && LCOLD && a.lds_blob != nullptr;
    if (blob) {
        const uint4 *g = reinterpret_cast<const uint4 *>(a.lds_blob);
        uint4 *d = reinterpret_cast<uint4 *>(smem);
        const uint32_t n16 = (PLAIN ? a.lds_plain_bytes : a.lds_total_bytes) / 16u;
        const uint32_t last = n16 - 1u;
        for (uint32_t k0 = threadIdx.x; k0 < n16; k0 += 4u * blockDim.x) {
            const uint32_t k1 = k0 + blockDim.x, k2 = k1 + blockDim.x, k3 = k2 + blockDim.x;
            const uint4 v0 = g[k0], v1 = g[min(k1, last)], v2 = g[min(k2, last)], v3 = g[min(k3, last)];
            d[k0] = v0;
            if (k1 < n16) d[k1] = v1;
            if (k2 < n16) d[k2] = v2;
            if (k3 < n16) d[k3] = v3;
        }
    }
    if constexpr (LSPH) {
        if (!blob) {
        stage16(smem + a.lds_sphf, a.sphf, (uint32_t)a.n_sph * (uint32_t)sizeof(RgSphF));
        stage16(smem + a.lds_sphf + (size_t)a.n_sph * sizeof(RgSphF), a.sphf2, (uint32_t)a.n_sph * (uint32_t)sizeof(RgSphF2));
        stage16(smem + a.lds_sph, a.sph, (uint32_t)a.n_sph * (uint32_t)sizeof(RgSph));
        stage16(smem + a.lds_cc, a.sph_cc, a.lds_nodes - a.lds_cc);
        if constexpr (BVH) {
            stage16(smem + a.lds_nodes, a.nodes, (uint32_t)a.n_nodes * (uint32_t)sizeof(RgBvhNode));
        }
        stage16(smem + a.lds_pln, a.pln, (uint32_t)a.n_pln * (uint32_t)sizeof(RgPln));
        stage16(smem + a.lds_dsk, a.dsk, (uint32_t)a.n_dsk * (uint32_t)sizeof(RgDsk));
        stage16(smem + a.lds_box, a.box, a.lds_lights - a.lds_box);
        stage16(smem + a.lds_lights, a.lights, (uint32_t)a.n_lights * (uint32_t)sizeof(RgLightDev));
        stage16(smem + a.lds_texs, a.texs, a.lds_lbuf - a.lds_texs);
        if constexpr (!PLAIN)
            if (a.lbuf) stage16(smem + a.lds_lbuf, a.lbuf, a.lds_bodies - a.lds_lbuf);
        }
        src.f = reinterpret_cast<const RgSphF *>(smem + a.lds_sphf);
        src.f2 = reinterpret_cast<const RgSphF2 *>(smem + a.lds_sphf + (size_t)a.n_sph * sizeof(RgSphF));
        src.s = reinterpret_cast<const RgSph *>(smem + a.lds_sph);
        src.cc = reinterpret_cast<const double *>(smem + a.lds_cc);
        src.pl = reinterpret_cast<const RgPln *>(smem + a.lds_pln);
        src.dk = reinterpret_cast<const RgDsk *>(smem + a.lds_dsk);
        src.bx = reinterpret_cast<const RgBox *>(smem + a.lds_box);
        src.nd = reinterpret_cast<const RgBvhNode *>(smem + a.lds_nodes);
        src.lb = reinterpret_cast<const RgLightBufDev *>(smem + a.lds_lbuf);
        src.lt = reinterpret_cast<const RgLightDev *>(smem + a.lds_lights);
    } else {
        src.s = rg_cptr(a.sph);
        src.cc = rg_cptr(a.sph_cc);
        src.f = rg_cptr(a.sphf);
        src.f2 = rg_cptr(a.sphf2);
        src.pl = rg_cptr(a.pln);
        src.dk = rg_cptr(a.dsk);
        src.bx = rg_cptr(a.box);
        if constexpr (K::lds_nodes_only) {
            stage16(smem + a.lds_lstack_bytes, a.nodes, (uint32_t)a.n_nodes * (uint32_t)sizeof(RgBvhNode));
            src.nd = reinterpret_cast<const RgBvhNode *>(smem + a.lds_lstack_bytes);
        } else {
            src.nd = rg_cptr(a.nodes);
        }
        src.lb = a.lbuf;
        src.lt = a.lights;
    }
    if constexpr (LSPH && LCOLD) {
        if (!blob) {
            stage16(smem + a.lds_bodies, a.bodies, (uint32_t)a.n_bodies * (uint32_t)sizeof(RgBodyDev));
            stage16(smem + a.lds_mats, a.mats, (uint32_t)a.n_bodies * (uint32_t)sizeof(RgMatDev));
        }
        T.bodies = reinterpret_cast<const RgBodyDev *>(smem + a.lds_bodies);
        T.mats = reinterpret_cast<const RgMatDev *>(smem + a.lds_mats);
    } else {
        T.bodies = a.bodies;
        T.mats = a.mats;
    }
    if constexpr (LSPH) {
        T.lights = reinterpret_cast<const RgLightDev *>(smem + a.lds_lights);
        T.texs = reinterpret_cast<const RgTexDev *>(smem + a.lds_texs);
    } else {
        T.lights = a.lights;
        T.texs = a.texs;
    }
    [[maybe_unused]] const PlainTex PT{reinterpret_cast<const RgTexMagic *>(smem + a.lds_texm),
                                       reinterpret_cast<const RgPlnAxes *>(smem + a.lds_axes)};
    if (TASKS || LSPH || LCOLD) {
        if constexpr (TASKS) pool_init();
        __syncthreads();
    }

    const int lane = threadIdx.x & 63;
    __shared__ uint32_t tile_px[K::tile_px_rows][64];
    uint32_t *my_px = &tile_px[K::host_frames ? threadIdx.x >> 6 : 0][lane];
    constexpr int RING = K::ring;
    __shared__ uint32_t ring_px[RING > 0 ? RG_LIGHT_BLOCK_WAVES : 1][RING > 0 ? RING : 1][64];
    __shared__ uint32_t ring_tile[RING > 0 ? RG_LIGHT_BLOCK_WAVES : 1][RING > 0 ? RING : 1];
    [[maybe_unused]] const uint32_t rw = RING > 0 ? (threadIdx.x >> 6) % RG_LIGHT_BLOCK_WAVES : 0u;
    [[maybe_unused]] uint32_t nring = 0;
    [[maybe_unused]] uint32_t grp_next = 0, grp_end = 0;
    constexpr int PK_PP = 0, PK_LIN = LB, PK_REFL = 2 * LB, PK_COL = 2 * LB + 1, PK_KIND = 2 * LB + 4,
                  PK_R = 2 * LB + 5, PK_N = 2 * LB + 6;
    __shared__ float park_lds[K::light ? RG_LIGHT_BLOCK_WAVES : 1][K::light ? PK_N : 1][64];
    float *park = &park_lds[K::light ? (threadIdx.x >> 6) % RG_LIGHT_BLOCK_WAVES : 0][0][lane];
#ifdef RG_BVH_STATS
    if (lane < 16) rg_stat_lds[(threadIdx.x >> 6) % RG_BVH_MAX_WAVES][lane] = 0ull;
#endif
    [[maybe_unused]] const unsigned long long t_kernel = RG_CLOCK();
#ifdef RG_WAVE_TIMES
    const unsigned long long t_staged = wall_clock64();
#endif
    const uint32_t twlog = K::host_frames ? a.tile_wlog : 3u, twmask = (1u << twlog) - 1u, th = 64u >> twlog;
    const uint32_t tiles_x = (a.width + twmask) >> twlog;
    const uint32_t ntiles = tiles_x * ((a.out_rows + th - 1u) / th);
    const C3 def = c3(a.def[0], a.def[1], a.def[2]);
    const int max_depth = (int)a.max_depth;
    [[maybe_unused]] const bool use_ring = RING > 0 && a.defer_px;
    [[maybe_unused]] const uint32_t ring_n = RING > 0 ? (a.ring_flush ? min(a.ring_flush, (uint32_t)(RING > 0 ? RING : 1)) : (uint32_t)RING) : 1u;
    [[maybe_unused]] const uint32_t ring_g = RING > 0 ? (a.ring_group ? min(a.ring_group, ring_n) : ring_n) : 1u;
    [[maybe_unused]] auto flush_ring = [&]() {
        for (uint32_t k = 0; k < nring; ++k) {
            const uint32_t tile = ring_tile[rw][k];
            const uint32_t ty = tile / tiles_x, tx = tile - ty * tiles_x;
            const uint32_t x = (tx << twlog) + ((uint32_t)lane & twmask);
            const uint32_t orow = ty * th + ((uint32_t)lane >> twlog);
            if (x < a.width && orow < a.out_rows) {
                const uint32_t row = a.image_rows ? out_row_to_y(a, orow) : out_row_of(a, orow);
                if (row != 0xFFFFFFFFu) a.rgba[(size_t)row * a.width + x] = ring_px[rw][k][lane];
            }
        }
        if (a.tile_flags) {
            __builtin_amdgcn_fence(__ATOMIC_RELEASE, "");
            if ((uint32_t)lane < nring)
                __hip_atomic_store(&a.tile_flags[ring_tile[rw][lane]], a.frame_seq, __ATOMIC_RELAXED,
                                   __HIP_MEMORY_SCOPE_SYSTEM);
        }
        nring = 0;
    };
    uint32_t n_prim = 0, n_shadow = 0, n_sec = 0;
    FrameStack<K::array_frames> stk;
    stk.init(a);

    uint32_t qi = blockIdx.x % RG_NQ, qtried = 0;
    int mode = MODE_DONE;
    Ray q;
    ShadowBatch<LB> sb;
    uint32_t occl_full = 0u;
    int qdepth = 0;
    V3 hp = v3(0, 0, 0), hn = v3(0, 0, 0);
    int hb = 0, hdepth = 0, li = 0;
    int nfan = 0;
    uint32_t fan_lanes = 0u;
    uint32_t fan_bits = 0u;
    C3 fin = c3(0, 0, 0), bcol = c3(0, 0, 0), ret = def;
    int sp = 0;
    Closest c;
    closest_init(c);
    bool have_result = false;
    uint32_t occl = 0u;
    size_t oidx = 0;
    uint32_t pixel = 0;
    int task = -1;
    bool tiles_left = true;
    [[maybe_unused]] uint32_t pf_k = 0u;
    [[maybe_unused]] bool pf_valid = false;
    uint32_t my_tile = 0xFFFFFFFFu;
    [[maybe_unused]] uint32_t tiles_taken = 0;
    [[maybe_unused]] bool counted = false;
#ifdef RG_TILE_TIMES
    uint32_t cur_tile = 0xFFFFFFFFu;
    unsigned long long t_tile = 0, t_query = 0;
    uint32_t tile_iters = 0;
#endif
    for (;;) {
        RG_REGION(RGR_LOOP);
        if constexpr (K::shadow_fan) {
            if (__any(nfan > 0)) {
                fan_bits = 0u;
#pragma unroll
                for (int k = 0; k < RG_SHADOW_FAN; ++k) {
                    const uint32_t b = (uint32_t)__shfl((int)occl, (int)((fan_lanes >> (6 * k)) & 63u), 64);
                    if (k < nfan) fan_bits |= (b & 1u) << k;
                }
            }
            if (mode == MODE_SHADOW_H) {
                mode = MODE_DONE;
                have_result = false;
            }
        }
        if (have_result) {
            bool unwind = false;
            bool shade = false;
            const int rmode = mode;
            if (TASKS && rmode == MODE_WAIT) {
                unwind = true;
            } else if (rmode == MODE_CLOSEST) {
                if (c.nan && c.nhit >= 2) raise_error(a, pixel, RG_ERR_NAN_DISTANCE);
                if (c.id < 0) {
                    ret = def;
                    unwind = true;
                } else {
                    const RgBodyDev b = T.bodies[c.id];
                    const RgMatDev m = T.mats[c.id];
                    RG_REGION(RGR_GETCOLOR);
                    if (b.kind == RG_BODY_SPHERE) RG_REGION(RGR_NORMAL_SPHERE);
                    V3 h = add(q.o, scl(q.d, c.t));
                    V3 n;
                    if (!surface_normal(b, h, n)) raise_error(a, pixel, RG_ERR_AABB_NORMAL);
                    if (m.surface != RG_SURFACE_REFRACTIVE) {
                        if constexpr (K::light) {
                            const bool textured = m.coloration != RG_COLORATION_COLOR;
                            uint32_t texel = 0u;
                            RG_REGION(RGR_BATCH);
#ifdef RG_REGION_STATS
                            if (textured) {
                                RG_REGION(RGR_TEXEL);
                                if (b.kind == RG_BODY_SPHERE) RG_REGION(RGR_UV_SPHERE);
                                else if (b.kind != RG_BODY_AABB) RG_REGION(RGR_UV_PLANE);
                            }
#endif
                            if (textured) texel = PLAIN ? texel_fetch_plain(T.texs, PT, m, b, c.id, h) : texel_fetch(T.texs, m, b, h);
                            else { park[64 * PK_COL] = m.color[0]; park[64 * (PK_COL + 1)] = m.color[1]; park[64 * (PK_COL + 2)] = m.color[2]; }
                            park[64 * PK_REFL] = m.albedo_pi;
                            const int kind = m.surface == RG_SURFACE_DIFFUSE ? 0 : qdepth + 1 < max_depth ? 2 : 1;
                            park[64 * PK_KIND] = __int_as_float(kind);
                            park[64 * PK_R] = m.reflectivity;
                            q.o = add(h, scl(n, SHADOW_BIAS));
                            if (kind == 2) q.d = sub(q.d, scl(n, 2.0 * dot(q.d, n)));
                            occl_full = 0u;
#pragma unroll
                            for (int l = 0; l < LB; ++l) {
                                if (l < n_lights) {
                                    const RgLightDev L = T.lights[l];
                                    if (L.kind != RG_LIGHT_DIRECTIONAL) RG_REGION(RGR_LIGHT_SPH);
                                    light_dir_dist<UL>(L, h, sb.d[l], sb.ld[l]);
                                    park[64 * (PK_PP + l)] = fmaxf((float)dot(n, sb.d[l]), 0.0f);
                                    park[64 * (PK_LIN + l)] = light_intensity(L, h);
                                    occl_full |= 1u << l;
                                    n_shadow++;
                                } else {
                                    sb.d[l] = v3(0.0, 0.0, 1.0);
                                    sb.ld[l] = 0.0;
                                }
                            }
                            if (textured) {
                                const C3 col = texel_color(texel);
                                park[64 * PK_COL] = col.r; park[64 * (PK_COL + 1)] = col.g; park[64 * (PK_COL + 2)] = col.b;
                            }
                            if (n_lights > 0) mode = MODE_SHADOW;
                            else shade = true;
                        } else {
                            bcol = surface_color(T.texs, m, b, h);
                            hb = c.id; hdepth = qdepth;
                            fin = c3(0.0f, 0.0f, 0.0f);
                            hp = h; hn = n; li = 0;
                            if (m.surface == RG_SURFACE_REFLECTING && qdepth + 1 < max_depth)
                                q.d = sub(q.d, scl(n, 2.0 * dot(q.d, n)));
                            shade = true;
                        }
                    } else {
                        RG_REGION(RGR_REFRACT);
                        float kr = (float)fresnel(q.d, n, m.index);
                        C3 surf = PLAIN ? surface_color_plain(T.texs, PT, m, b, c.id, h) : surface_color(T.texs, m, b, h);
                        int cd = qdepth + 1;
                        if (cd >= max_depth) {
                            Ray tr;
                            if (kr < 1.0f && !transmission(n, q.d, h, m.index, tr)) raise_error(a, pixel, RG_ERR_TRANSMISSION);
                            C3 col = cadd(cscl(def, kr), cscl(def, 1.0f - kr));
                            ret = cmul(cscl(col, m.transparency), surf);
                            unwind = true;
                        } else {
                            RG_REGION(RGR_PUSH_REFR);
                            auto &&f = stk[sp++];
                            f.f[0] = kr; f.f[1] = m.transparency;
                            f.f[2] = surf.r; f.f[3] = surf.g; f.f[4] = surf.b;
                            if constexpr (TASKS) f.cdepth = cd;
                            bool trace_t = false;
                            if (kr < 1.0f) {
                                if constexpr (TASKS) {
                                    Ray tr;
                                    if (transmission(n, q.d, h, m.index, tr)) {
                                        trace_t = true;
                                        const Ray rr = reflection(n, q.d, h);
                                        const int slot = pool_alloc(lane);
                                        if (slot >= 0) {
                                            double *pr = pool_of().ray[slot];
                                            pr[0] = rr.o.x; pr[1] = rr.o.y; pr[2] = rr.o.z;
                                            pr[3] = rr.d.x; pr[4] = rr.d.y; pr[5] = rr.d.z;
                                            pool_of().depth[slot] = cd;
                                            pool_of().pix[slot] = pixel;
                                            pool_publish(slot);
                                            f.type = FR_REFR_TASK | (slot << 8);
                                        } else {
                                            f.type = FR_REFR_T;
                                            f.rr[0] = rr.o.x; f.rr[1] = rr.o.y; f.rr[2] = rr.o.z;
                                            f.rr[3] = rr.d.x; f.rr[4] = rr.d.y; f.rr[5] = rr.d.z;
                                        }
                                        q = tr;
                                    }
                                } else {
                                    const Ray rr = reflection(n, q.d, h);
                                    f.rr[0] = rr.o.x; f.rr[1] = rr.o.y; f.rr[2] = rr.o.z;
                                    f.rr[3] = rr.d.x; f.rr[4] = rr.d.y; f.rr[5] = rr.d.z;
                                    f.type = FR_REFR_T;
                                    trace_t = transmission(n, q.d, h, m.index, q);
                                }
                                if (!trace_t) raise_error(a, pixel, RG_ERR_TRANSMISSION);
                            }
                            if (!trace_t) {
                                f.type = FR_REFR_R;
                                f.f[5] = def.r; f.f[6] = def.g; f.f[7] = def.b;
                                q = reflection(n, q.d, h);
                            }
                            qdepth = cd;
                            mode = MODE_CLOSEST;
                            n_sec++;
                        }
                    }
                }
            } else if (rmode == MODE_SHADOW) {
                shade = true;
            }
            if constexpr (K::light) {
              if (shade) {
                RG_REGION(RGR_SHADE);
                const C3 bc = c3(park[64 * PK_COL], park[64 * (PK_COL + 1)], park[64 * (PK_COL + 2)]);
                const float refl = park[64 * PK_REFL];
                C3 acc = c3(0.0f, 0.0f, 0.0f);
#pragma unroll
                for (int l = 0; l < LB; ++l) {
                    if (l < n_lights) {
                        const RgLightDev L = T.lights[l];
                        const float inten = !((occl >> l) & 1u) ? park[64 * (PK_LIN + l)] : 0.0f;
                        const float power = park[64 * (PK_PP + l)] * inten;
                        C3 lc = cscl(cscl(c3(L.color[0], L.color[1], L.color[2]), power), refl);
                        acc = cadd(acc, cmul(bc, lc));
                    }
                }
                C3 dcol = cclamp(acc);
                const int kind = __float_as_int(park[64 * PK_KIND]);
                if (kind == 0) {
                    ret = dcol;
                    unwind = true;
                } else {
                    if (kind == 1) {
                        const float r = park[64 * PK_R];
                        ret = cadd(cscl(dcol, 1.0f - r), cscl(def, r));
                        unwind = true;
                    } else {
                        RG_REGION(RGR_PUSH_REFL);
                        auto &&f = stk[sp++];
                        f.type = FR_REFL;
                        f.f[0] = dcol.r; f.f[1] = dcol.g; f.f[2] = dcol.b; f.f[3] = park[64 * PK_R];
                        qdepth = TASKS ? qdepth + 1 : sp;
                        mode = MODE_CLOSEST;
                        n_sec++;
                    }
                }
              }
            } else if (shade) {
                const RgMatDev m = T.mats[hb];
                if (rmode == MODE_SHADOW) {
                    const float refl = m.albedo_pi;
#pragma unroll
                    for (int l = 0; l < LB; ++l) {
                        if (li + l < a.n_lights) {
                            const RgLightDev L = T.lights[li + l];
                            float inten = !((occl >> l) & 1u) ? light_intensity(L, hp) : 0.0f;
                            float power = fmaxf((float)dot(hn, sb.d[l]), 0.0f) * inten;
                            C3 lc = cscl(cscl(c3(L.color[0], L.color[1], L.color[2]), power), refl);
                            fin = cadd(fin, cmul(bcol, lc));
                        }
                    }
                    if constexpr (K::shadow_fan) {
                        for (int k = 0; k < nfan; ++k) {
                            const RgLightDev L = T.lights[li + 1 + k];
                            V3 ldir;
                            double ldist;
                            light_dir_dist<UL>(L, hp, ldir, ldist);
                            float inten = !((fan_bits >> k) & 1u) ? light_intensity(L, hp) : 0.0f;
// ... 258 lines not shown
                        have_result = false;
                    } else {
                    q.o = v3(0.0, 0.0, 0.0);
                    if constexpr (fast_camera) q.d = normalize_camera(sx, sy);
                    else q.d = normalize(v3(sx, sy, -1.0));
                    n_prim++;
                    closest_init(c);
                    trace_primary<F32F, BVH, PLAIN>(a, src, q.d, c);
                    have_result = true;
                    }
                    mode = MODE_CLOSEST;
                    qdepth = 0;
                    task = -1;
                }
                continue;
            }
        }
        if constexpr (K::shadow_fan) {
            const int want = mode == MODE_SHADOW ? min(a.n_lights - li - 1, RG_SHADOW_FAN) : 0;
            unsigned long long owners = __ballot(want > 0);
            if (owners != 0ull) {
                unsigned long long idle = __ballot(mode == MODE_DONE);
                while (owners != 0ull && idle != 0ull) {
                    const int o = __builtin_ctzll(owners);
                    owners &= owners - 1ull;
                    const int w = __builtin_amdgcn_readlane(want, o);
                    const int oli = __builtin_amdgcn_readlane(li, o);
                    const int ohd = __builtin_amdgcn_readlane(hdepth, o);
                    const uint32_t opix = (uint32_t)__builtin_amdgcn_readlane((int)pixel, o);
                    const V3 ohp = v3(readlane_d(hp.x, o), readlane_d(hp.y, o), readlane_d(hp.z, o));
                    const V3 oso = v3(readlane_d(q.o.x, o), readlane_d(q.o.y, o), readlane_d(q.o.z, o));
                    uint32_t packed = 0u;
                    int k = 0;
                    for (; k < w && idle != 0ull; ++k) {
                        const int hl = __builtin_ctzll(idle);
                        idle &= idle - 1ull;
                        packed |= (uint32_t)hl << (6 * k);
                        if (lane == hl) {
                            hp = ohp;
                            q.o = oso;
                            hdepth = ohd;
                            pixel = opix;
                            light_dir_dist<UL>(T.lights[oli + 1 + k], hp, sb.d[0], sb.ld[0]);
                            li = oli + 1 + k;
                            mode = MODE_SHADOW_H;
                        }
                    }
                    if (lane == o) {
                        nfan = k;
                        fan_lanes = packed;
                        n_shadow += (uint32_t)k;
                    }
                }
            }
        }
        if constexpr (TASKS) {
            const bool idle = mode == MODE_DONE;
            const unsigned long long want = __ballot(idle);
            if (want != 0ull && pool_any_pending()) {
                if (idle) {
                    const int slot = pool_take((int)__builtin_amdgcn_mbcnt_hi((uint32_t)(want >> 32),
                                                   __builtin_amdgcn_mbcnt_lo((uint32_t)want, 0u)));
                    if (slot >= 0) {
                        const double *r = pool_of().ray[slot];
                        q.o = v3(r[0], r[1], r[2]);
                        q.d = v3(r[3], r[4], r[5]);
                        qdepth = pool_of().depth[slot];
                        pixel = pool_of().pix[slot];
                        task = slot;
                        mode = MODE_CLOSEST;
                        n_sec++;
                    }
                }
            }
        }
        const bool live = mode != MODE_DONE;
        const bool wave_live = __any(live);
        if constexpr (TASKS) {
            if (wave_live != counted) {
                if (lane == 0) atomicAdd(&pool_of().busy, wave_live ? 1 : -1);
                counted = wave_live;
            }
        }
        if (!wave_live) {
            if (tiles_left) continue;
            if constexpr (!TASKS) break;
            if (!pool_any_pending() && __hip_atomic_load(&pool_of().busy, __ATOMIC_RELAXED, __HIP_MEMORY_SCOPE_WORKGROUP) == 0)
                break;
            __builtin_amdgcn_s_sleep(4);
            continue;
        }
        const bool querying = mode == MODE_CLOSEST || mode == MODE_SHADOW || mode == MODE_SHADOW_H;
        if (!__any(querying)) {
            __builtin_amdgcn_s_sleep(2);
            have_result = mode == MODE_WAIT;
            continue;
        }
        KDiag::iter_stats<K::light>(a, lane, querying, mode, mode == MODE_CLOSEST ? qdepth : hdepth);
#ifdef RG_TILE_TIMES
        ++tile_iters;
        const unsigned long long t_q0 = wall_clock64();
#endif
        if (querying) {
            closest_init(c);
            occl = 0u;
        }
        if constexpr (!K::light) {
            if (querying) {
                bool o1 = false;
                Ray r1;
                r1.o = q.o;
                const bool shadow = mode == MODE_SHADOW || mode == MODE_SHADOW_H;
                r1.d = shadow ? sb.d[0] : q.d;
                const bool lane_walk = (shadow ? hdepth : qdepth) >= (int)a.lane_min_depth &&
                                       !(K::camera && !shadow && qdepth == 0);
                const bool exact = shadow && (a.nan_scene || ray_exotic(r1.o, r1.d));
                trace_query<F32F, BVH>(a, src, r1, shadow && !exact, sb.ld[0], c, o1, lane_walk, shadow ? li : -1);
                if (exact) {
                    o1 = c.id >= 0 && !(c.t > sb.ld[0]);
                    if (c.nan && c.nhit >= 2) raise_error(a, pixel, RG_ERR_NAN_DISTANCE);
                }
                occl = o1 ? 1u : 0u;
            }
        } else {
            bool exact = false;
            if (mode == MODE_SHADOW) {
                exact = nan_scene;
#pragma unroll
                for (int l = 0; l < LB; ++l) exact |= ((occl_full >> l) & 1u) && ray_exotic(q.o, sb.d[l]);
            }
            const int passes = mode == MODE_CLOSEST ? 1 : exact ? LB : 0;
            if (exact) occl = ~occl_full & ((1u << LB) - 1u);
            for (int l = 0; __any(l < passes); ++l) {
                if (l < passes && (mode == MODE_CLOSEST || ((occl_full >> l) & 1u))) {
                    RG_REGION(RGR_Q_CLOSEST);
                    Ray rq;
                    rq.o = q.o;
                    rq.d = q.d;
                    double ld = 0.0;
                    if (exact) {
#pragma unroll
                        for (int k = 0; k < LB; ++k)
                            if (k == l) { rq.d = sb.d[k]; ld = sb.ld[k]; }
                        closest_init(c);
                    }
                    bool unused = false;
                    trace_query<F32F, BVH, PLAIN>(a, src, rq, false, 0.0, c, unused);
                    if (exact) {
                        if (c.id >= 0 && !(c.t > ld)) occl |= 1u << l;
                        if (c.nan && c.nhit >= 2) raise_error(a, pixel, RG_ERR_NAN_DISTANCE);
                    }
                }
            }
            if (mode == MODE_SHADOW && !exact) {
                RG_REGION(RGR_Q_SHADOW);
                occl = ~occl_full & ((1u << LB) - 1u);
                trace_shadow<LB, PLAIN>(a, src, q.o, sb, (1u << LB) - 1u, occl);
            }
        }
#ifdef RG_TILE_TIMES
        t_query += wall_clock64() - t_q0;
#endif
        have_result = querying || mode == MODE_WAIT;
    }
    if (K::host_frames && my_tile != 0xFFFFFFFFu && (a.defer_px || a.tile_flags)) {
        bool ringed = false;
        if constexpr (RING > 0) {
            if (use_ring) {
                ring_px[rw][nring][lane] = *my_px;
                if (lane == 0) ring_tile[rw][nring] = my_tile;
                ++nring;
                ringed = true;
            }
        }
        if (!ringed) flush_tile(a, oidx, *my_px, my_tile, lane);
    }
    if constexpr (RING > 0) {
        if (use_ring) flush_ring();
    }
#ifdef RG_TILE_TIMES
    if (cur_tile != 0xFFFFFFFFu && lane == 0 && a.rgb) {
        a.rgb[cur_tile] = (float)(wall_clock64() - t_tile) * 0.01f;
        a.rgb[ntiles + cur_tile] = (float)tile_iters;
        a.rgb[2 * ntiles + cur_tile] = (float)(t_tile & 0xFFFFFFull);
        a.rgb[3 * ntiles + cur_tile] = (float)t_query * 0.01f;
    }
#endif

    RG_STAT(14, RG_CLOCK() - t_kernel);
    RG_STAT(15, 1);
#ifdef RG_WAVE_TIMES
    if (lane == 0 && a.rgb) {
        const unsigned long long t_end = wall_clock64();
        uint32_t *wt = reinterpret_cast<uint32_t *>(a.rgb) + 4u * (blockIdx.x * (blockDim.x / 64u) + (threadIdx.x >> 6));
        wt[0] = (uint32_t)t_wave0;
        wt[1] = (uint32_t)(t_staged - t_wave0);
        wt[2] = (uint32_t)(t_end - t_wave0);
        wt[3] = wt_tiles;
    }
#endif
#ifdef RG_BVH_STATS
    if (lane >= 4 && lane < 16) atomicAdd(&a.counters[lane], rg_stat_lds[(threadIdx.x >> 6) % RG_BVH_MAX_WAVES][lane]);
#endif
    unsigned long long p64 = wave_sum(n_prim), s64 = wave_sum(n_shadow), q64 = wave_sum(n_sec);
    if (lane == 0) {
        if (p64) atomicAdd(&a.counters[0], p64);
        if (s64) atomicAdd(&a.counters[1], s64);
        if (q64) atomicAdd(&a.counters[2], q64);
        if (a.snap_out) {
            __builtin_amdgcn_s_waitcnt(0);
            const unsigned long long waves = (unsigned long long)gridDim.x * (blockDim.x >> 6);
            if (atomicAdd(&a.counters[RG_DONE_WORD], 1ull) == waves - 1ull) {
#pragma unroll
                for (int k = 0; k < 4; ++k)
                    a.snap_out[k] = __hip_atomic_load(&a.counters[k], __ATOMIC_RELAXED, __HIP_MEMORY_SCOPE_AGENT);
            }
        }
    }
}
```

raingun_amd/csrc/rg_scene.hip:

```cpp
#include <hip/hip_runtime.h>

#include <algorithm>
#include <cmath>
#include <cstring>
#include <memory>
#include <new>
#include <vector>

#include "../../include/raingun.h"
#include "../../include/raingun_debug.h"
#include "rg_bvh.h"
#include "rg_camera.h"
#include "rg_device.h"
#include "rg_exact.h"
#include "rg_lightbuf.h"
#include "rg_internal.h"

#pragma clang fp contract(off)

#ifndef RG_BVH_MIN_SPHERES
#define RG_BVH_MIN_SPHERES 16
#endif

namespace {

template <class T>
rg_status upload(rg_scene *s, T **dst, const T *src, size_t n) {
    *dst = nullptr;
    if (n == 0) return RG_OK;
    void *p = nullptr;
    if (!ok(hipMalloc(&p, n * sizeof(T)))) return RG_ERR_OUT_OF_MEMORY;
    s->allocations.push_back(p);
    if (!ok(hipMemcpy(p, src, n * sizeof(T), hipMemcpyHostToDevice))) return RG_ERR_DEVICE;
    *dst = static_cast<T *>(p);
    return RG_OK;
}

double dot3(const double *a, const double *b) { return (a[0] * b[0] + a[1] * b[1]) + a[2] * b[2]; }

float f32_up(double v) {
    float f = (float)v;
    if ((double)f < v) f = std::nextafter(f, HUGE_VALF);
    return f;
}

void make_filter_records(const double *p, RgSphF &f, RgSphF2 &f2) {
    const double u = 5.9604644775390625e-08;
    const double r2 = p[3] * p[3];
    const double cc = dot3(p, p);
    f.cx = (float)p[0];
    f.cy = (float)p[1];
    f.cz = (float)p[2];
    f.r2hi = std::max(f32_up(r2 * (1.0 + 4.0 * u)), 1e-30f);
    f2.cchi = f32_up(cc * (1.0 + 1e-6));
    f2.cc32 = (float)cc;
    const double kd1 = u * (16.2 + 26.2 * 1.00001) * 1.01;
    f2.thrp = f32_up(((double)f.r2hi + kd1 * (double)f2.cchi) * (1.0 + 1e-6));
    f2.id = -1;
}

double fov_adjustment(double fov) { return std::tan(fov * (3.14159265358979323846 / 180.0) / 2.0); }

int body_params(uint32_t kind) { return kind == RG_BODY_SPHERE ? 4 : kind == RG_BODY_DISK ? 7 : 6; }

bool exotic_value(double v) { return !(std::fabs(v) < 1e100); }

void release(rg_scene *s) {
    if (!s) return;
    (void)hipSetDevice(s->device);
    for (rg_frames *f : s->frames) rg_frames_detach_scene(f);
    s->frames.clear();
    rg_multi_release(s);
    rg_image_res_release(s->img);
    rg_aa_res_release(s->aa);
    for (void *p : s->allocations) (void)hipFree(p);
    s->allocations.clear();
    if (s->lds_blob) (void)hipFree(s->lds_blob);
    s->lds_blob = nullptr;
    for (rg_launch_ctx *c : s->ctxs) rg_ctx_destroy(c);
    s->ctxs.clear();
    delete s;
}

rg_status upload_tables(rg_scene *s, const rg_host_tables &h) {
    rg_status st = RG_OK;
#define RG_UP(dst, vec) \
    if (st == RG_OK) st = upload(s, &s->dst, h.vec.data(), h.vec.size())
    RG_UP(sph, sph);
    RG_UP(sph_cc, sph_cc);
    RG_UP(sphf, sphf);
    RG_UP(sphf2, sphf2);
    RG_UP(sph_id, sph_id);
    RG_UP(pln, pln);
    RG_UP(pln_id, pln_id);
    RG_UP(dsk, dsk);
    RG_UP(dsk_id, dsk_id);
    RG_UP(box, box);
    RG_UP(box_id, box_id);
    RG_UP(bodies, bodies);
    RG_UP(mats, mats);
    RG_UP(lights, lights);
    RG_UP(nodes, nodes);
    RG_UP(lbuf, lbuf);
    RG_UP(lb_start, lb_start);
    RG_UP(lb_ent, lb_ent);
#undef RG_UP
    std::vector<RgTexDev> texs(h.tex_w.size());
    for (size_t i = 0; st == RG_OK && i < texs.size(); ++i) {
        texs[i].w = (int32_t)h.tex_w[i];
        texs[i].h = (int32_t)h.tex_h[i];
        texs[i].texels = nullptr;
        if (h.texels[i].empty()) continue;
        uint32_t *dp = nullptr;
        st = upload(s, &dp, h.texels[i].data(), h.texels[i].size());
        texs[i].texels = dp;
    }
    if (st == RG_OK) st = upload(s, &s->texs, texs.data(), texs.size());
    s->tex_desc = texs;
    return st;
}

void copy_scalars(rg_scene *dst, const rg_scene *src) {
    dst->fov = src->fov;
    std::memcpy(dst->def, src->def, sizeof dst->def);
    dst->max_depth = src->max_depth;
    dst->n_sph = src->n_sph;
    dst->n_pln = src->n_pln;
    dst->n_dsk = src->n_dsk;
    dst->n_box = src->n_box;
    dst->n_bodies = src->n_bodies;
    dst->n_lights = src->n_lights;
    dst->n_textures = src->n_textures;
    dst->n_nodes = src->n_nodes;
    dst->n_lbuf = src->n_lbuf;
    dst->lb_cam = src->lb_cam;
    dst->n_lbdesc = src->n_lbdesc;
    dst->lane_stack = src->lane_stack;
    dst->nan_scene = src->nan_scene;
    dst->bvh_obound = src->bvh_obound;
    dst->bvh_rbound = src->bvh_rbound;
    dst->bvh_margin = src->bvh_margin;
    dst->bvh_extent = src->bvh_extent;
    dst->bvh_info = src->bvh_info;
}

}


RgKernelArgs rg_make_args(const rg_scene *s) {
    RgKernelArgs a;
    std::memset(&a, 0, sizeof a);
    a.sph = s->sph;
    a.sph_cc = s->sph_cc;
    a.sphf = s->sphf;
    a.sphf2 = s->sphf2;
    a.path = s->path;
    a.sph_id = s->sph_id;
    a.pln = s->pln;
    a.pln_id = s->pln_id;
    a.dsk = s->dsk;
    a.dsk_id = s->dsk_id;
    a.box = s->box;
    a.box_id = s->box_id;
    a.n_sph = s->n_sph;
    a.n_pln = s->n_pln;
    a.n_dsk = s->n_dsk;
    a.n_box = s->n_box;
    const bool bvh = s->bvh_enabled && s->n_nodes > 0;
    a.nodes = bvh ? s->nodes : nullptr;
    a.n_nodes = bvh ? s->n_nodes : 0;
    a.bvh_obound = s->bvh_obound;
    a.bvh_rbound = s->bvh_rbound;
    a.bvh_margin = s->bvh_margin;
    a.bvh_extent = s->bvh_extent;
    const bool lbuf = bvh && s->lbuf_enabled && (s->n_lbuf > 0 || s->lb_cam >= 0);
    a.lbuf = lbuf ? s->lbuf : nullptr;
    a.lb_start = lbuf ? s->lb_start : nullptr;
    a.lb_ent = lbuf ? s->lb_ent : nullptr;
    a.n_lbuf = lbuf ? s->n_lbuf : 0;
    a.lb_cam = lbuf ? s->lb_cam : -1;
    a.bodies = s->bodies;
    a.mats = s->mats;
    a.lights = s->lights;
    a.texs = s->texs;
    a.n_bodies = s->n_bodies;
    a.n_lights = s->n_lights;
    a.n_textures = s->n_textures;
    a.nan_scene = s->nan_scene ? 1 : 0;
    const bool lane = bvh && rg_heavy_path(a) && s->lane_stack > 0 && s->lane_min_depth < 1 << 20;
    a.lane_stack = lane ? s->lane_stack : 0;
    a.lane_min_depth = lane ? s->lane_min_depth : 1 << 30;
    a.lds_lstack_bytes = lane ? ((uint32_t)(a.lane_stack + 1) * 4u) * 256u * RG_HEAVY_WPS : 0u;
    auto al16 = [](uint32_t v) { return (v + 15u) & ~15u; };
    a.lds_sphf = a.lds_lstack_bytes;
    a.lds_sph = a.lds_sphf + (uint32_t)s->n_sph * (uint32_t)(sizeof(RgSphF) + sizeof(RgSphF2));
    a.lds_cc = a.lds_sph + (uint32_t)s->n_sph * (uint32_t)sizeof(RgSph);
    a.lds_nodes = al16(a.lds_cc + (uint32_t)s->n_sph * 8u);
    a.lds_pln = a.lds_nodes + (uint32_t)a.n_nodes * (uint32_t)sizeof(RgBvhNode);
    a.lds_dsk = a.lds_pln + (uint32_t)s->n_pln * (uint32_t)sizeof(RgPln);
    a.lds_box = a.lds_dsk + (uint32_t)s->n_dsk * (uint32_t)sizeof(RgDsk);
    a.lds_lights = al16(a.lds_box + (uint32_t)s->n_box * (uint32_t)sizeof(RgBox));
    a.lds_texs = a.lds_lights + (uint32_t)s->n_lights * (uint32_t)sizeof(RgLightDev);
    a.lds_lbuf = al16(a.lds_texs + (uint32_t)s->n_textures * (uint32_t)sizeof(RgTexDev));
    a.lds_bodies = a.lds_lbuf + (a.lbuf ? (uint32_t)s->n_lbdesc * (uint32_t)sizeof(RgLightBufDev) : 0u);
    a.lds_hot_bytes = a.lds_bodies;
    a.lds_mats = a.lds_bodies + (uint32_t)s->n_bodies * (uint32_t)sizeof(RgBodyDev);
    a.lds_total_bytes = a.lds_mats + (uint32_t)s->n_bodies * (uint32_t)sizeof(RgMatDev);
    a.lds_texm = a.lds_total_bytes;
    a.lds_axes = a.lds_texm + (uint32_t)s->n_textures * (uint32_t)sizeof(RgTexMagic);
    a.lds_plain_bytes = a.lds_axes + (uint32_t)s->n_bodies * (uint32_t)sizeof(RgPlnAxes);
    a.def[0] = s->def[0];
    a.def[1] = s->def[1];
    a.def[2] = s->def[2];
    a.max_depth = s->max_depth;
    a.fov_adjustment = fov_adjustment(s->fov);
    a.tile_wlog = 3;
    return a;
}

double rg_fov_adjustment(double fov) { return fov_adjustment(fov); }

bool rg_scene_heavy(const rg_scene *s) {
    RgKernelArgs a;
    std::memset(&a, 0, sizeof a);
    a.n_sph = s->n_sph;
    a.n_pln = s->n_pln;
    a.n_dsk = s->n_dsk;
    a.n_box = s->n_box;
    a.path = s->path;
    a.n_lights = s->n_lights;
    return rg_heavy_path(a);
}

const void *rg_lds_blob_for(const rg_scene *s, const RgKernelArgs &a) {
    const uint32_t layout[14] = {a.lds_sphf, a.lds_sph, a.lds_cc, a.lds_nodes, a.lds_pln, a.lds_dsk, a.lds_box,
                                 a.lds_bodies, a.lds_mats, a.lds_lights, a.lds_texs, a.lds_total_bytes,
                                 (uint32_t)a.n_nodes, (uint32_t)a.n_sph};
    rg_scene *m = const_cast<rg_scene *>(s);
    if (m->lds_blob && std::memcmp(layout, m->lds_blob_layout, sizeof layout) == 0) return m->lds_blob;
    if (!s->host || a.lds_total_bytes == 0 || a.lds_total_bytes % 16u != 0u || a.lds_plain_bytes % 16u != 0u)
        return nullptr;
    const rg_host_tables &h = *s->host;
    std::vector<unsigned char> img(a.lds_plain_bytes, 0);
    auto put = [&](uint32_t off, const void *src, size_t bytes) {
        if (bytes && off + bytes <= img.size()) std::memcpy(img.data() + off, src, bytes);
    };
    put(a.lds_sphf, h.sphf.data(), h.sphf.size() * sizeof(RgSphF));
    put(a.lds_sphf + (uint32_t)(h.sphf.size() * sizeof(RgSphF)), h.sphf2.data(), h.sphf2.size() * sizeof(RgSphF2));
    put(a.lds_sph, h.sph.data(), h.sph.size() * sizeof(RgSph));
    put(a.lds_cc, h.sph_cc.data(), h.sph_cc.size() * sizeof(double));
    if (a.n_nodes > 0) put(a.lds_nodes, h.nodes.data(), h.nodes.size() * sizeof(RgBvhNode));
    put(a.lds_pln, h.pln.data(), h.pln.size() * sizeof(RgPln));
    put(a.lds_dsk, h.dsk.data(), h.dsk.size() * sizeof(RgDsk));
    put(a.lds_box, h.box.data(), h.box.size() * sizeof(RgBox));
    put(a.lds_bodies, h.bodies.data(), h.bodies.size() * sizeof(RgBodyDev));
    put(a.lds_mats, h.mats.data(), h.mats.size() * sizeof(RgMatDev));
    put(a.lds_lights, h.lights.data(), h.lights.size() * sizeof(RgLightDev));
    put(a.lds_texs, s->tex_desc.data(), s->tex_desc.size() * sizeof(RgTexDev));
    if (a.lbuf) put(a.lds_lbuf, h.lbuf.data(), h.lbuf.size() * sizeof(RgLightBufDev));
    std::vector<RgTexMagic> texm(h.tex_w.size(), RgTexMagic{0, 0, 0, 0});
    for (size_t t = 0; t < texm.size(); ++t) {
        if (h.tex_w[t] == 0 || h.tex_h[t] == 0) continue;
        const RgMagicU32 mw = rg_magic_u32(h.tex_w[t]), mh = rg_magic_u32(h.tex_h[t]);
        texm[t] = RgTexMagic{mw.m, mw.sh, mh.m, mh.sh};
    }
    put(a.lds_texm, texm.data(), texm.size() * sizeof(RgTexMagic));
    std::vector<RgPlnAxes> axes(h.bodies.size());
    std::memset(axes.data(), 0, axes.size() * sizeof(RgPlnAxes));
    for (size_t b = 0; b < axes.size(); ++b)
        if (h.bodies[b].kind == RG_BODY_PLANE) rg_plane_axes(&h.bodies[b].p[3], axes[b].xa, axes[b].ya);
    put(a.lds_axes, axes.data(), axes.size() * sizeof(RgPlnAxes));
    void *p = nullptr;
    if (!ok(hipMalloc(&p, img.size()))) { (void)hipGetLastError(); return nullptr; }
    if (!ok(hipMemcpy(p, img.data(), img.size(), hipMemcpyHostToDevice))) { (void)hipFree(p); return nullptr; }
    if (m->lds_blob) {
        m->allocations.push_back(m->lds_blob);
    }
    m->lds_blob = p;
    std::memcpy(m->lds_blob_layout, layout, sizeof layout);
    return p;
}

rg_status rg_scene_replica(const rg_scene *src, int32_t device, rg_scene **out) {
    *out = nullptr;
    if (!src->host) return RG_ERR_INVALID_ARGUMENT;
    rg_scene *s = new (std::nothrow) rg_scene();
    if (!s) return RG_ERR_OUT_OF_MEMORY;
    s->device = device;
    copy_scalars(s, src);
    rg_sync_settings(s, src);
    s->host = src->host;
    if (!ok(hipSetDevice(device))) { release(s); return RG_ERR_DEVICE; }
    rg_status st = upload_tables(s, *src->host);
    if (st == RG_OK && !(s->last = rg_ctx_for(s, nullptr))) st = RG_ERR_OUT_OF_MEMORY;
    if (st != RG_OK) { release(s); return st; }
    *out = s;
    return RG_OK;
}

void rg_scene_free(rg_scene *s) { release(s); }

void rg_sync_settings(rg_scene *dst, const rg_scene *src) {
    dst->max_depth = src->max_depth;
    dst->path = src->path;
    dst->bvh_enabled = src->bvh_enabled;
    dst->lbuf_enabled = src->lbuf_enabled;
    dst->exact_div = src->exact_div;
    dst->has_camera = src->has_camera;
    dst->camera = src->camera;
    dst->lane_min_depth = src->lane_min_depth;
    dst->tile_order = src->tile_order;
    dst->ring_flush_small = src->ring_flush_small;
    dst->ring_group_small = src->ring_group_small;
    dst->ring_flush_big = src->ring_flush_big;
    dst->ring_group_big = src->ring_group_big;
}

extern "C" {

rg_status rg_scene_create(const rg_scene_desc *d, int32_t device, rg_scene **out) {
    if (!d || !out) return RG_ERR_INVALID_ARGUMENT;
    *out = nullptr;
    if ((d->n_bodies && !d->bodies) || (d->n_lights && !d->lights) || (d->n_textures && !d->textures))
        return RG_ERR_INVALID_ARGUMENT;
    int ndev = 0;
    if (hipGetDeviceCount(&ndev) != hipSuccess || device < 0 || device >= ndev) return RG_ERR_DEVICE;
    bool nan_scene = false;
    for (uint32_t i = 0; i < d->n_bodies; ++i) {
        const rg_body &b = d->bodies[i];
        if (b.kind > RG_BODY_AABB || b.material.coloration > RG_COLORATION_TEXTURE ||
            b.material.surface > RG_SURFACE_REFRACTIVE)
            return RG_ERR_INVALID_ARGUMENT;
        if (b.material.coloration == RG_COLORATION_TEXTURE) {
            int32_t t = b.material.texture;
            if (t < 0 || (uint32_t)t >= d->n_textures || !d->textures[t].rgba || d->textures[t].width == 0 ||
                d->textures[t].height == 0 || d->textures[t].width > 0x7fffffffu || d->textures[t].height > 0x7fffffffu)
                return RG_ERR_TEXTURE;
        }
        for (int k = 0; k < body_params(b.kind); ++k) nan_scene |= exotic_value(b.p[k]);
    }
    for (uint32_t i = 0; i < d->n_lights; ++i) {
        if (d->lights[i].kind > RG_LIGHT_SPHERICAL) return RG_ERR_INVALID_ARGUMENT;
        for (int k = 0; k < 3; ++k) nan_scene |= exotic_value(d->lights[i].v[k]);
    }

    rg_scene *s = new (std::nothrow) rg_scene();
    if (!s) return RG_ERR_OUT_OF_MEMORY;
    std::shared_ptr<rg_host_tables> hp(new (std::nothrow) rg_host_tables());
    if (!hp) { delete s; return RG_ERR_OUT_OF_MEMORY; }
    rg_host_tables &h = *hp;
    s->device = device;
    s->fov = d->fov;
    std::memcpy(s->def, d->default_color, sizeof s->def);
    s->max_depth = d->max_recursion_depth;
    s->nan_scene = nan_scene;
    if (!ok(hipSetDevice(device))) { release(s); return RG_ERR_DEVICE; }

    std::vector<double> sph_raw;
    h.bodies.resize(d->n_bodies);
    h.mats.resize(d->n_bodies);
    for (uint32_t i = 0; i < d->n_bodies; ++i) {
        const rg_body &b = d->bodies[i];
        const double *p = b.p;
        h.bodies[i].kind = (int32_t)b.kind;
        h.bodies[i].pad = 0;
        std::memcpy(h.bodies[i].p, b.p, sizeof h.bodies[i].p);
        const rg_material &m = b.material;
        RgMatDev &md = h.mats[i];
        md.coloration = (int32_t)m.coloration;
        std::memcpy(md.color, m.color, sizeof md.color);
        md.tex = m.texture;
        md.xoff = m.x_offset;
        md.yoff = m.y_offset;
        md.albedo_pi = m.albedo / 3.14159265358979323846f;
        md.surface = (int32_t)m.surface;
        md.reflectivity = m.reflectivity;
        md.index = m.index;
        md.transparency = m.transparency;
        switch (b.kind) {
        case RG_BODY_SPHERE:
            h.sph.push_back(RgSph{p[0], p[1], p[2], p[3] * p[3]});
            h.sphf.emplace_back();
            h.sphf2.emplace_back();
            make_filter_records(p, h.sphf.back(), h.sphf2.back());
            h.sphf2.back().id = (int32_t)i;
            h.sph_cc.push_back(dot3(p, p));
            h.sph_id.push_back((int32_t)i);
            sph_raw.insert(sph_raw.end(), p, p + 4);
            break;
        case RG_BODY_PLANE:
            h.pln.push_back(RgPln{p[0], p[1], p[2], p[3], p[4], p[5], dot3(p, p + 3), 0.0});
            h.pln_id.push_back((int32_t)i);
            break;
        case RG_BODY_DISK:
            h.dsk.push_back(RgDsk{p[0], p[1], p[2], p[3], p[4], p[5], p[6], dot3(p, p + 3)});
            h.dsk_id.push_back((int32_t)i);
            break;
        default:
            h.box.push_back(RgBox{{p[0], p[1], p[2]}, {p[3], p[4], p[5]}});
            h.box_id.push_back((int32_t)i);
            break;
        }
    }
    RgBvhBuild bvh;
    if (!nan_scene && (int)h.sph.size() >= RG_BVH_MIN_SPHERES && rg_build_bvh(sph_raw.data(), (int)h.sph.size(), bvh)) {
        auto permute = [&](auto &v) {
            auto old = v;
            for (size_t j = 0; j < bvh.order.size(); ++j) v[j] = old[bvh.order[j]];
        };
        permute(h.sph);
        permute(h.sphf);
        permute(h.sphf2);
        permute(h.sph_cc);
        permute(h.sph_id);
        s->bvh_obound = bvh.obound;
        s->bvh_rbound = bvh.rbound;
        s->bvh_margin = bvh.margin;
        s->bvh_extent = bvh.extent;
        s->bvh_info.built = 1;
        s->bvh_info.nodes = (int32_t)bvh.nodes.size();
        s->bvh_info.leaves = bvh.leaves;
        s->bvh_info.depth = bvh.depth;
        s->bvh_info.lane_stack = bvh.lane_stack;
        s->bvh_info.margin = (float)bvh.margin;
        s->bvh_info.origin_bound = bvh.obound;
        h.nodes = bvh.nodes;
    }
    if (h.sph_cc.size() % 2) h.sph_cc.push_back(0.0);
    h.lights.resize(d->n_lights);
    for (uint32_t i = 0; i < d->n_lights; ++i) {
        const rg_light &l = d->lights[i];
        RgLightDev &ld = h.lights[i];
        ld.kind = (int32_t)l.kind;
        std::memcpy(ld.color, l.color, sizeof ld.color);
        ld.intensity = l.intensity;
        ld.pad = 0;
        std::memcpy(ld.v, l.v, sizeof ld.v);
        double nx = -l.v[0], ny = -l.v[1], nz = -l.v[2];
        double inv = 1.0 / std::sqrt((nx * nx + ny * ny) + nz * nz);
        ld.dn[0] = nx * inv;
        ld.dn[1] = ny * inv;
        ld.dn[2] = nz * inv;
        ld.pad2 = 0.0;
    }
    if (!h.nodes.empty()) {
        std::vector<double> sp(4 * h.sph.size());
        for (size_t j = 0; j < h.sph.size(); ++j) {
            const double *p = &sph_raw[4 * (size_t)bvh.order[j]];
            std::memcpy(&sp[4 * j], p, 4 * sizeof(double));
        }
        const uint32_t nl = std::min<uint32_t>(d->n_lights, RG_LB_MAX_LIGHTS);
        h.lbuf.assign(nl, RgLightBufDev{});
        int built = 0;
        for (uint32_t i = 0; i < nl; ++i) {
            RgLightBufBuild lb;
            if (!rg_build_lightbuf(sp.data(), (int)h.sph.size(), h.lights[i].kind, h.lights[i].dn, h.lights[i].v,
                                   bvh.extent, (double)bvh.obound, lb))
                continue;
            if (h.lb_ent.size() + lb.ent.size() + h.lb_start.size() + lb.start.size() > RG_LB_TOTAL_WORDS) continue;
            const uint32_t ebase = (uint32_t)h.lb_ent.size(), cbase = (uint32_t)h.lb_start.size();
            for (uint32_t &v : lb.start) v += ebase;
            lb.dev.cell_off = cbase;
            lb.dev.always0 += ebase;
            lb.dev.always1 += ebase;
            h.lb_start.insert(h.lb_start.end(), lb.start.begin(), lb.start.end());
            h.lb_ent.insert(h.lb_ent.end(), lb.ent.begin(), lb.ent.end());
            h.lbuf[i] = lb.dev;
            ++built;
        }
        const double zero[3] = {0.0, 0.0, 0.0};
        RgLightBufBuild cam;
        if (rg_build_lightbuf(sp.data(), (int)h.sph.size(), RG_LIGHT_SPHERICAL, zero, zero, bvh.extent,
                              (double)bvh.obound, cam) &&
            h.lb_ent.size() + cam.ent.size() + h.lb_start.size() + cam.start.size() <= RG_LB_TOTAL_WORDS) {
            const uint32_t ebase = (uint32_t)h.lb_ent.size(), cbase = (uint32_t)h.lb_start.size();
            for (uint32_t &v : cam.start) v += ebase;
            cam.dev.cell_off = cbase;
            cam.dev.always0 += ebase;
            cam.dev.always1 += ebase;
            h.lb_start.insert(h.lb_start.end(), cam.start.begin(), cam.start.end());
            h.lb_ent.insert(h.lb_ent.end(), cam.ent.begin(), cam.ent.end());
            s->lb_cam = (int32_t)h.lbuf.size();
            h.lbuf.push_back(cam.dev);
        }
        if (!built && s->lb_cam < 0) h.lbuf.clear();
        s->n_lbuf = built ? (int32_t)nl : 0;
        s->n_lbdesc = (int32_t)h.lbuf.size();
        s->bvh_info.lbuf_bytes = (int64_t)((h.lb_ent.size() + h.lb_start.size()) * sizeof(uint32_t) +
                                           h.lbuf.size() * sizeof(RgLightBufDev));
    }
    h.tex_w.resize(d->n_textures);
    h.tex_h.resize(d->n_textures);
    h.texels.resize(d->n_textures);
    for (uint32_t i = 0; i < d->n_textures; ++i) {
        const rg_texture &t = d->textures[i];
        h.tex_w[i] = t.width;
        h.tex_h[i] = t.height;
        const size_t n = (size_t)t.width * t.height;
        if (n == 0 || !t.rgba) continue;
        h.texels[i].resize(n);
        std::memcpy(h.texels[i].data(), t.rgba, n * 4);
    }
    s->n_sph = (int32_t)h.sph.size();
    s->n_pln = (int32_t)h.pln.size();
    s->n_dsk = (int32_t)h.dsk.size();
    s->n_box = (int32_t)h.box.size();
    s->n_bodies = (int32_t)d->n_bodies;
    s->n_lights = (int32_t)d->n_lights;
    s->n_textures = (int32_t)d->n_textures;
    s->n_nodes = (int32_t)h.nodes.size();
    s->lane_stack = (s->n_nodes <= (1 << RG_LANE_NODE_BITS) && bvh.lane_stack <= RG_LANE_STACK_MAX)
                        ? std::max(bvh.lane_stack, 1) : 0;

    rg_status st = upload_tables(s, h);
    s->host = hp;
    if (st == RG_OK && !(s->last = rg_ctx_for(s, nullptr))) st = RG_ERR_OUT_OF_MEMORY;
    if (st != RG_OK) { release(s); return st; }
    *out = s;
    return RG_OK;
}

void rg_scene_destroy(rg_scene *s) { release(s); }

rg_status rg_scene_set_max_depth(rg_scene *s, uint32_t max_depth) {
    if (!s) return RG_ERR_INVALID_ARGUMENT;
    s->max_depth = max_depth;
    return RG_OK;
}

rg_status rg_camera_look_at(const double eye[3], const double target[3], const double up[3], rg_camera *out) {
    if (!eye || !target || !up || !out) return RG_ERR_INVALID_ARGUMENT;
    rg_camera c;
    if (!rg_camera_look_at_basis(eye, target, up, c.right, c.up, c.forward)) return RG_ERR_INVALID_ARGUMENT;
    for (int k = 0; k < 3; ++k) c.eye[k] = eye[k];
    *out = c;
    return RG_OK;
}

rg_status rg_scene_set_camera(rg_scene *s, const rg_camera *camera) {
    if (!s) return RG_ERR_INVALID_ARGUMENT;
    if (!camera) {
        s->has_camera = false;
        return RG_OK;
    }
    if (!rg_camera_valid(camera->eye, camera->right, camera->up, camera->forward)) return RG_ERR_INVALID_ARGUMENT;
    s->camera = *camera;
    s->has_camera = true;
    return RG_OK;
}

}
```

raingun_amd/scene.py:

```python
from __future__ import annotations

import ctypes as C
import os
from dataclasses import dataclass, field
from pathlib import Path
from typing import Callable, List, Optional, Sequence, Union

import numpy as np

from . import _abi, aov
from .camera import Camera
from .color import Color



class SceneError(ValueError):
    """The YAML does not deserialise into a Scene (serde_yaml's Err)."""


@dataclass
class Texture:
    path: str
    image: np.ndarray
    x_offset: float
# ... 99 lines not shown
        p = tuple(b.p)
        mat = material(b.material)
        if b.kind == _abi.BODY_SPHERE:
            bodies.append(Sphere(p[0:3], p[3], mat))
        elif b.kind == _abi.BODY_PLANE:
            bodies.append(Plane(p[0:3], p[3:6], mat))
        elif b.kind == _abi.BODY_DISK:
            bodies.append(Disk(p[0:3], p[3:6], p[6], mat))
        else:
            bodies.append(AABB((p[0:3], p[3:6]), mat))
    lights: List[Light] = []
    for i in range(d.n_lights):
        l = d.lights[i]
        cls = DirectionalLight if l.kind == _abi.LIGHT_DIRECTIONAL else SphericalLight
        lights.append(cls(tuple(l.v), Color(*l.color), l.intensity))
    return Scene(d.fov, Color(*d.default_color), d.max_recursion_depth, bodies, lights)


class SceneDesc:

    def __init__(self, scene: "Scene"):
        nb, nl = len(scene.bodies), len(scene.lights)
        self.bodies = (_abi.rg_body * max(nb, 1))()
        self.lights = (_abi.rg_light * max(nl, 1))()
        tex_index: dict = {}
        self._images: List[np.ndarray] = []
        for i, b in enumerate(scene.bodies):
            rb = self.bodies[i]
            if isinstance(b, Sphere):
                rb.kind, p = _abi.BODY_SPHERE, [*b.center, b.radius]
            elif isinstance(b, Plane):
                rb.kind, p = _abi.BODY_PLANE, [*b.origin, *b.normal]
            elif isinstance(b, Disk):
                rb.kind, p = _abi.BODY_DISK, [*b.origin, *b.normal, b.radius]
            elif isinstance(b, AABB):
                rb.kind, p = _abi.BODY_AABB, [*b.bounds[0], *b.bounds[1]]
            else:
                raise TypeError(f"not a body: {b!r}")
            for k, v in enumerate(p):
                rb.p[k] = v
            m = b.material
            rm = rb.material
            if isinstance(m.coloration, Texture):
                key = id(m.coloration.image)
                if key not in tex_index:
                    tex_index[key] = len(self._images)
                    self._images.append(np.ascontiguousarray(m.coloration.image, dtype=np.uint8))
                rm.coloration = _abi.COLORATION_TEXTURE
                rm.texture = tex_index[key]
                rm.x_offset = m.coloration.x_offset
                rm.y_offset = m.coloration.y_offset
            else:
                rm.coloration = _abi.COLORATION_COLOR
                rm.color[:] = [float(m.coloration.red), float(m.coloration.green), float(m.coloration.blue)]
                rm.texture = -1
            rm.albedo = m.albedo
            rm.surface = {"Diffuse": _abi.SURFACE_DIFFUSE, "Reflecting": _abi.SURFACE_REFLECTING,
                          "Refractive": _abi.SURFACE_REFRACTIVE}[m.surface]
            rm.reflectivity = m.reflectivity
            rm.index = m.index
            rm.transparency = m.transparency
        for i, l in enumerate(scene.lights):
            rl = self.lights[i]
            if isinstance(l, DirectionalLight):
                rl.kind, v = _abi.LIGHT_DIRECTIONAL, l.direction
            else:
                rl.kind, v = _abi.LIGHT_SPHERICAL, l.position
            rl.v[:] = list(v)
            rl.color[:] = [float(l.color.red), float(l.color.green), float(l.color.blue)]
            rl.intensity = l.intensity
        self.textures = (_abi.rg_texture * max(len(self._images), 1))()
        for i, im in enumerate(self._images):
            self.textures[i].height, self.textures[i].width = im.shape[0], im.shape[1]
            self.textures[i].rgba = im.ctypes.data_as(C.POINTER(C.c_uint8))
        d = _abi.rg_scene_desc()
        d.fov = scene.fov
        d.default_color[:] = [float(scene.default_color.red), float(scene.default_color.green),
                              float(scene.default_color.blue)]
        d.max_recursion_depth = scene.max_recursion_depth
        d.n_bodies, d.bodies = nb, C.cast(self.bodies, C.POINTER(_abi.rg_body))
        d.n_lights, d.lights = nl, C.cast(self.lights, C.POINTER(_abi.rg_light))
        d.n_textures, d.textures = len(self._images), C.cast(self.textures, C.POINTER(_abi.rg_texture))
        self.desc = d

    def ptr(self):
        return C.byref(self.desc)


class DeviceScene:

    def __init__(self, scene: "Scene", device: int = 0, path: Optional[int] = None, bvh: Optional[bool] = None):
        self._desc = SceneDesc(scene)
        h = C.c_void_p()
        _abi.check(_abi.lib().rg_scene_create(self._desc.ptr(), int(device), C.byref(h)), "rg_scene_create")
        self.handle = h
        self.device = device
        if path is not None:
            self.set_path(path)
        if bvh is not None:
            self.set_bvh(bvh)

    def close(self) -> None:
        if getattr(self, "handle", None):
            _abi.lib().rg_scene_destroy(self.handle)
            self.handle = None

    def __del__(self):
        try:
            self.close()
        except Exception:
            pass

    def set_path(self, path: int) -> None:
        _abi.check(_abi.lib().rg_debug_set_path(self.handle, int(path)))

    def set_bvh(self, enable: bool) -> None:
        _abi.check(_abi.lib().rg_debug_set_bvh(self.handle, 1 if enable else 0))

    def set_lightbuf(self, enable: bool) -> None:
        _abi.check(_abi.lib().rg_debug_set_lightbuf(self.handle, 1 if enable else 0))

    def lightbuf_count(self) -> int:
        return int(_abi.lib().rg_debug_lightbuf_count(self.handle))

    def set_tile_order(self, mode) -> None:
        _abi.check(_abi.lib().rg_debug_set_tile_order(self.handle, int(mode)))

    def set_lane_depth(self, min_depth: int) -> None:
        _abi.check(_abi.lib().rg_debug_set_lane_depth(self.handle, int(min_depth)))

    def set_image_bands(self, bands: int) -> None:
        _abi.check(_abi.lib().rg_debug_set_image_bands(self.handle, int(bands)))

    def set_multi(self, mode: int = 0, stand_in: bool = False, bands: int = 0, only_rank: int = -1) -> None:
        _abi.check(_abi.lib().rg_debug_set_multi(self.handle, int(mode), 1 if stand_in else 0, int(bands),
                                                 int(only_rank)))

    def set_host_ring(self, flush_small: int = -1, group_small: int = -1, flush_big: int = -1, group_big: int = -1,
                      multi_light_one: int = -1) -> None:
        _abi.check(_abi.lib().rg_debug_set_host_ring(self.handle, int(flush_small), int(group_small), int(flush_big),
                                                     int(group_big), int(multi_light_one)))

    def set_host_split(self, pct: int) -> None:
        _abi.check(_abi.lib().rg_debug_set_host_split(self.handle, int(pct)))

    def set_host_tile_shape(self, tile_wlog: int) -> None:
        _abi.check(_abi.lib().rg_debug_set_host_tile_shape(self.handle, int(tile_wlog)))

    def last_plain(self) -> bool:
        plain = C.c_int32(-1)
        _abi.check(_abi.lib().rg_debug_last_plain(self.handle, C.byref(plain)))
        return plain.value == 1

    def set_exact_div(self, enable: bool) -> None:
        _abi.check(_abi.lib().rg_debug_set_exact_div(self.handle, 1 if enable else 0))

    def camera_check(self, width: int, height: int, fov: float):
        bad, admitted = C.c_uint64(0), C.c_int32(-1)
        _abi.check(_abi.lib().rg_debug_camera_check(self.handle, int(width), int(height), float(fov), C.byref(bad),
                                                    C.byref(admitted)))
        return int(bad.value), admitted.value == 1

    def unscaled_check(self, op: int, a, b=None) -> int:
        import numpy as np

        a = np.ascontiguousarray(a, dtype=np.float64)
        bp = None
        if b is not None:
            b = np.ascontiguousarray(b, dtype=np.float64)
            assert b.shape == a.shape
            bp = b.ctypes.data_as(C.c_void_p)
        bad = C.c_uint64(0)
        _abi.check(_abi.lib().rg_debug_unscaled_check(self.handle, int(op), a.ctypes.data_as(C.c_void_p), bp, a.size,
                                                      C.byref(bad)))
        return int(bad.value)

    def bvh_info(self) -> _abi.rg_bvh_info:
        info = _abi.rg_bvh_info()
        _abi.check(_abi.lib().rg_debug_bvh_info(self.handle, C.byref(info)))
        return info

    def set_max_depth(self, depth: int) -> None:
        _abi.check(_abi.lib().rg_scene_set_max_depth(self.handle, int(depth)))

    def set_camera(self, camera: Optional[Camera]) -> None:
        if camera is None:
            _abi.check(_abi.lib().rg_scene_set_camera(self.handle, None), "rg_scene_set_camera")
            return
        c = _abi.rg_camera((C.c_double * 3)(*camera.eye), (C.c_double * 3)(*camera.right),
                           (C.c_double * 3)(*camera.up), (C.c_double * 3)(*camera.forward))
        _abi.check(_abi.lib().rg_scene_set_camera(self.handle, C.byref(c)), "rg_scene_set_camera")

    def render_image(self, width: int, height: int, stats: Optional[_abi.rg_stats] = None,
                     out: Optional[np.ndarray] = None) -> np.ndarray:
        if out is None:
            out = np.empty((height, width, 4), dtype=np.uint8)
        assert out.shape == (height, width, 4) and out.dtype == np.uint8 and out.flags.c_contiguous
        st = stats if stats is not None else _abi.rg_stats()
        _abi.check(_abi.lib().rg_render_image(self.handle, width, height, out.ctypes.data, C.byref(st)),
                   "rg_render_image")
        return out

    def render_image_aa(self, width: int, height: int, samples: int, want_rgb: bool = False,
                        stats: Optional[_abi.rg_stats] = None, out: Optional[np.ndarray] = None):
        if out is None:
            out = np.empty((height, width, 4), dtype=np.uint8)
        assert out.shape == (height, width, 4) and out.dtype == np.uint8 and out.flags.c_contiguous
        rgb = np.empty((height, width, 3), dtype=np.float32) if want_rgb else None
        st = stats if stats is not None else _abi.rg_stats()
        _abi.check(_abi.lib().rg_render_image_aa(self.handle, width, height, int(samples), out.ctypes.data,
                                                 rgb.ctypes.data if rgb is not None else None, C.byref(st)),
                   "rg_render_image_aa")
        return (out, rgb) if want_rgb else out

    def render_image_aa_adaptive(self, width: int, height: int, samples: int, threshold: int, want_rgb: bool = False,
                                 want_mask: bool = False, stats: Optional[_abi.rg_stats] = None,
                                 out: Optional[np.ndarray] = None):
        if out is None:
            out = np.empty((height, width, 4), dtype=np.uint8)
        assert out.shape == (height, width, 4) and out.dtype == np.uint8 and out.flags.c_contiguous
        rgb = np.empty((height, width, 3), dtype=np.float32) if want_rgb else None
        mask = np.empty((height, width), dtype=np.uint8) if want_mask else None
        st = stats if stats is not None else _abi.rg_stats()
        _abi.check(_abi.lib().rg_render_image_aa_adaptive(
            self.handle, width, height, int(samples), int(threshold), out.ctypes.data,
            rgb.ctypes.data if rgb is not None else None, mask.ctypes.data if mask is not None else None,
            C.byref(st)), "rg_render_image_aa_adaptive")
        res = (out,) + ((rgb,) if want_rgb else ()) + ((mask,) if want_mask else ())
        return res if len(res) > 1 else out

    def edge_mask(self, rgba: np.ndarray, threshold: int):
        rgba = np.ascontiguousarray(rgba, dtype=np.uint8)
        if rgba.ndim != 3 or rgba.shape[2] != 4 or rgba.size == 0:
            raise ValueError("expected (height, width, 4) uint8 RGBA")
        h, w = rgba.shape[:2]
        mask = np.empty((h, w), dtype=np.uint8)
        n = C.c_uint32(0)
        _abi.check(_abi.lib().rg_edge_mask(int(self.device), rgba.ctypes.data, w, h, int(threshold), mask.ctypes.data,
                                           C.byref(n)), "rg_edge_mask")
        return mask, int(n.value)

    def resolve_box(self, rgb: np.ndarray, samples: int):
        k = int(samples)
        rgb = np.ascontiguousarray(rgb, dtype=np.float32)
        if rgb.ndim != 3 or rgb.shape[2] != 3 or k < 1 or rgb.shape[0] % k or rgb.shape[1] % k:
            raise ValueError("expected (samples*height, samples*width, 3) float32 samples")
        h, w = rgb.shape[0] // k, rgb.shape[1] // k
        mean = np.empty((h, w, 3), dtype=np.float32)
        rgba = np.empty((h, w, 4), dtype=np.uint8)
        _abi.check(_abi.lib().rg_resolve_box(int(self.device), rgb.ctypes.data, w, h, k, rgba.ctypes.data,
                                             mean.ctypes.data), "rg_resolve_box")
        return mean, rgba

    def set_aa_band_rows(self, rows: int) -> None:
        _abi.check(_abi.lib().rg_debug_set_aa_band_rows(self.handle, int(rows)))

    def render_multi(self, width: int, height: int, ngpus: int, tile_rows: int = 0,
                     stats: Optional[_abi.rg_stats] = None, out: Optional[np.ndarray] = None) -> np.ndarray:
        if out is None:
            out = np.empty((height, width, 4), dtype=np.uint8)
        st = stats if stats is not None else _abi.rg_stats()
        _abi.check(_abi.lib().rg_render_multi(self.handle, width, height, int(ngpus), int(tile_rows),
                                              out.ctypes.data, C.byref(st)), "rg_render_multi")
        return out

    def render_stream(self, width: int, height: int, on_tile, tile_rows: int = 16,
                      stats: Optional[_abi.rg_stats] = None) -> int:
        st = stats if stats is not None else _abi.rg_stats()

        def cb(row0, rows, w, ptr, _user):
            band = np.ctypeslib.as_array(ptr, shape=(rows * w * 4,)).reshape(rows, w, 4).copy()
            return 1 if on_tile(int(row0), band) else 0

        fn = _abi.TILE_CALLBACK(cb)
        return _abi.lib().rg_render_stream(self.handle, width, height, tile_rows, fn, None, C.byref(st))

    def stream_status(self, stream: int):
        px = C.c_int32(-1)
        st = _abi.lib().rg_stream_status(self.handle, C.c_void_p(stream), C.byref(px))
        return st, px.value

    def release_stream(self, stream: int) -> None:
        _abi.check(_abi.lib().rg_scene_release_stream(self.handle, C.c_void_p(stream)), "rg_scene_release_stream")

    def render_tiles(self, width: int, height: int, tile_rows: int = 0, stride: int = 1, offset: int = 0,
                     want_rgb: bool = False, stats: Optional[_abi.rg_stats] = None):
        t = _abi.rg_tiling(tile_rows or height, stride, offset)
        rows = _abi.lib().rg_tiling_rows(height, C.byref(t))
        rgba = np.empty((rows, width, 4), dtype=np.uint8)
        rgb = np.empty((rows, width, 3), dtype=np.float32) if want_rgb else None
        st = stats if stats is not None else _abi.rg_stats()
        status = _abi.lib().rg_render_tiles(self.handle, width, height, C.byref(t), rgba.ctypes.data,
                                            rgb.ctypes.data if rgb is not None else None, C.byref(st))
        _abi.check(status, "rg_render_tiles")
        return (rgba, rgb) if want_rgb else rgba

    def render_aov(self, width: int, height: int, layers=aov.LAYERS, stats: Optional[_abi.rg_stats] = None) -> dict:
        layers = aov.parse_layers(layers)
        out = {n: np.empty(aov.layer_shape(n, height, width), dtype=aov.DTYPES[n]) for n in layers}
        v = _abi.rg_aov(**{n: out[n].ctypes.data for n in layers})
        st = stats if stats is not None else _abi.rg_stats()
        _abi.check(_abi.lib().rg_render_aov(self.handle, width, height, C.byref(v), C.byref(st)), "rg_render_aov")
        return out

    def render_aov_tiles(self, width: int, height: int, tile_rows: int = 0, stride: int = 1, offset: int = 0,
                         layers=aov.LAYERS, stream: int = 0, stats: Optional[_abi.rg_stats] = None,
# ... 85 lines not shown
```

Baseline: 147,400.

## Add precomputed shadow-volume grid to cull sphere/plane shadow tests per cell

At scene build, the host computes a 64^3 grid covering the scene. Each cell gets a bitmask of the spheres and planes that could occlude any light from points in that cell, using conservative distance margins. The plain render kernel looks up the shadow-ray origin's cell, ORs the masks across the wavefront with DPP, and tests only the flagged spheres and planes. This cuts per-ray shadow intersection work but adds a host-side build, a per-hit grid lookup, a wave reduction, and some risk of incorrect culling if the conservative bounds are wrong.

Measured after the change: 159,600 (median of 6 runs). 8.3% higher.

```diff
diff --git a/include/raingun_debug.h b/include/raingun_debug.h
--- a/include/raingun_debug.h
+++ b/include/raingun_debug.h
@@ -58,6 +58,19 @@
 
 rg_status rg_debug_last_plain(const rg_scene *scene, int32_t *plain);
 
+typedef struct rg_shadow_volume_info {
+    int32_t built;
+    int32_t enabled;
+    int32_t g;
+    int32_t pad;
+    int64_t bytes;
+    double build_ms;
+    double set_share;
+} rg_shadow_volume_info;
+rg_status rg_debug_set_shadow_volume(rg_scene *scene, int32_t on);
+rg_status rg_debug_shadow_volume_info(const rg_scene *scene, rg_shadow_volume_info *info);
+rg_status rg_debug_last_shadow_volume(const rg_scene *scene, int32_t *used);
+
 rg_status rg_debug_set_exact_div(rg_scene *scene, int32_t enable);
 rg_status rg_debug_camera_check(const rg_scene *scene, uint32_t width, uint32_t height, double fov,
                                 uint64_t *mismatches, int32_t *admitted);
diff --git a/raingun_amd/_abi.py b/raingun_amd/_abi.py
--- a/raingun_amd/_abi.py
+++ b/raingun_amd/_abi.py
@@ -116,6 +116,11 @@
     _fields_ = [("built", C.c_int32), ("enabled", C.c_int32), ("nodes", C.c_int32), ("leaves", C.c_int32),
                 ("depth", C.c_int32), ("margin", C.c_float), ("origin_bound", C.c_float), ("lane_stack", C.c_int32),
                 ("lbuf_bytes", C.c_int64)]
+
+
+class rg_shadow_volume_info(C.Structure):
+    _fields_ = [("built", C.c_int32), ("enabled", C.c_int32), ("g", C.c_int32), ("pad", C.c_int32),
+                ("bytes", C.c_int64), ("build_ms", C.c_double), ("set_share", C.c_double)]
 
 
 TILE_CALLBACK = C.CFUNCTYPE(C.c_int32, C.c_uint32, C.c_uint32, C.c_uint32, C.POINTER(C.c_uint8), C.c_void_p)
@@ -156,6 +161,7 @@
                  "rg_debug_fail_split_a", "rg_debug_set_host_ring", "rg_debug_set_host_tile_shape", "rg_debug_set_multi", "rg_debug_gather_noop",
                  "rg_debug_counter_words", "rg_debug_set_aa_band_rows",
                  "rg_debug_set_aa_adaptive_timing", "rg_debug_aa_adaptive_info", "rg_debug_last_plain",
+                 "rg_debug_set_shadow_volume", "rg_debug_shadow_volume_info", "rg_debug_last_shadow_volume",
                  "rg_debug_set_exact_div", "rg_debug_camera_check", "rg_debug_unscaled_check")
 FRAMES_SYMBOLS = ("rg_frames_create", "rg_frames_destroy", "rg_frames_step", "rg_frames_flush", "rg_frames_image",
                   "rg_frames_read_image", "rg_frames_status", "rg_frames_set_batch", "rg_frames_set_root_tiles", "rg_comm_id_bytes",
@@ -247,6 +253,13 @@
     if hasattr(lib, "rg_debug_last_plain"):
         lib.rg_debug_last_plain.restype = C.c_int32
         lib.rg_debug_last_plain.argtypes = [C.c_void_p, P(C.c_int32)]
+    if hasattr(lib, "rg_debug_set_shadow_volume"):
+        lib.rg_debug_set_shadow_volume.restype = C.c_int32
+        lib.rg_debug_set_shadow_volume.argtypes = [C.c_void_p, C.c_int32]
+        lib.rg_debug_shadow_volume_info.restype = C.c_int32
+        lib.rg_debug_shadow_volume_info.argtypes = [C.c_void_p, P(rg_shadow_volume_info)]
+        lib.rg_debug_last_shadow_volume.restype = C.c_int32
+        lib.rg_debug_last_shadow_volume.argtypes = [C.c_void_p, P(C.c_int32)]
     if hasattr(lib, "rg_debug_set_exact_div"):
         lib.rg_debug_set_exact_div.restype = C.c_int32
         lib.rg_debug_set_exact_div.argtypes = [C.c_void_p, C.c_int32]
diff --git a/raingun_amd/csrc/rg_aov.hip b/raingun_amd/csrc/rg_aov.hip
--- a/raingun_amd/csrc/rg_aov.hip
+++ b/raingun_amd/csrc/rg_aov.hip
@@ -102,6 +102,7 @@
     const RgAovOut o{dev->body, dev->depth, dev->normal, dev->uv, dev->albedo};
     cx->last_counters = a.counters;
     cx->last_plain = 0;
+    cx->last_shvol = 0;
     if (stats && !ok(hipEventRecord(cx->ev0, st))) return RG_ERR_DEVICE;
     if (rows > 0) {
         if (!ok(rg_launch_aov(&a, &o, st))) return RG_ERR_DEVICE;
diff --git a/raingun_amd/csrc/rg_capi.hip b/raingun_amd/csrc/rg_capi.hip
--- a/raingun_amd/csrc/rg_capi.hip
+++ b/raingun_amd/csrc/rg_capi.hip
@@ -462,6 +462,25 @@
     return RG_OK;
 }
 
+rg_status rg_debug_set_shadow_volume(rg_scene *s, int32_t on) {
+    if (!s || (on != 0 && on != 1)) return RG_ERR_INVALID_ARGUMENT;
+    s->shvol_enabled = on != 0;
+    return RG_OK;
+}
+
+rg_status rg_debug_shadow_volume_info(const rg_scene *s, rg_shadow_volume_info *info) {
+    if (!s || !info) return RG_ERR_INVALID_ARGUMENT;
+    *info = s->shvol_info;
+    info->enabled = s->shvol_info.built && s->shvol_enabled;
+    return RG_OK;
+}
+
+rg_status rg_debug_last_shadow_volume(const rg_scene *s, int32_t *used) {
+    if (!s || !used || !s->last) return RG_ERR_INVALID_ARGUMENT;
+    *used = s->last->last_shvol;
+    return RG_OK;
+}
+
 rg_status rg_debug_set_exact_div(rg_scene *s, int32_t enable) {
     if (!s || (enable != 0 && enable != 1)) return RG_ERR_INVALID_ARGUMENT;
     s->exact_div = enable != 0;
diff --git a/raingun_amd/csrc/rg_device.h b/raingun_amd/csrc/rg_device.h
--- a/raingun_amd/csrc/rg_device.h
+++ b/raingun_amd/csrc/rg_device.h
@@ -148,6 +148,10 @@
     uint32_t lds_texm, lds_axes, lds_plain_bytes;
     uint32_t camera;
     double cam_eye[3], cam_right[3], cam_up[3], cam_forward[3];
+    const uint32_t *shvol;
+    uint32_t shvol_g;
+    float shvol_inv, shvol_off;
+    uint32_t shvol_pad[3];
 };
 
 __host__ __device__ inline uint32_t rg_tile_w(const RgKernelArgs &a) { return 1u << a.tile_wlog; }
@@ -187,6 +191,15 @@
 #ifndef RG_LB_ONE
 #define RG_LB_ONE 1
 #endif
+#ifndef RG_PLAIN_SHVOL
+#define RG_PLAIN_SHVOL 1
+#endif
+#ifndef RG_PLAIN_SHVOL_SPHERES
+#define RG_PLAIN_SHVOL_SPHERES 1
+#endif
+#ifndef RG_PLAIN_SHVOL_PLANES
+#define RG_PLAIN_SHVOL_PLANES 1
+#endif
 #ifndef RG_HEAVY_WPS
 #define RG_HEAVY_WPS 3
 #endif
diff --git a/raingun_amd/csrc/rg_internal.h b/raingun_amd/csrc/rg_internal.h
--- a/raingun_amd/csrc/rg_internal.h
+++ b/raingun_amd/csrc/rg_internal.h
@@ -23,6 +23,7 @@
     int cur = 0;
     unsigned long long *last_counters = nullptr;
     int last_plain = 0;
+    int last_shvol = 0;
     unsigned long long *sticky = nullptr;
     uint32_t *tile_cost = nullptr, *tile_perm = nullptr;
     size_t tile_cap = 0;
@@ -111,6 +112,7 @@
     std::vector<RgBvhNode> nodes;
     std::vector<RgLightBufDev> lbuf;
     std::vector<uint32_t> lb_start, lb_ent;
+    std::vector<uint32_t> shvol;
     std::vector<uint32_t> tex_w, tex_h;
     std::vector<std::vector<uint32_t>> texels;
 };
@@ -150,6 +152,10 @@
     int32_t lb_cam = -1;
     int32_t n_lbdesc = 0;
     bool lbuf_enabled = true;
+    uint32_t *shvol = nullptr;
+    bool shvol_enabled = true;
+    rg_shadow_volume_info shvol_info{};
+    float shvol_inv = 0.0f, shvol_off = 0.0f;
     bool exact_div = true;
     bool has_camera = false;
     rg_camera camera{};
diff --git a/raingun_amd/csrc/rg_k_trace.h b/raingun_amd/csrc/rg_k_trace.h
--- a/raingun_amd/csrc/rg_k_trace.h
+++ b/raingun_amd/csrc/rg_k_trace.h
@@ -6,6 +6,7 @@
 #include "rg_k_bvh.h"
 #include "rg_k_intersect.h"
 #include "rg_k_math.h"
+#include "rg_shadow_vol_cell.h"
 
 #pragma clang fp contract(off)
 
@@ -181,11 +182,84 @@
     double ld[LB];
 };
 
-template <int LB, bool NODB = false, class Src>
+__device__ __forceinline__ uint32_t wave_or(uint32_t v) {
+    v |= (uint32_t)__builtin_amdgcn_update_dpp(0, (int)v, 0x111, 0xf, 0xf, false);
+    v |= (uint32_t)__builtin_amdgcn_update_dpp(0, (int)v, 0x112, 0xf, 0xf, false);
+    v |= (uint32_t)__builtin_amdgcn_update_dpp(0, (int)v, 0x114, 0xf, 0xf, false);
+    v |= (uint32_t)__builtin_amdgcn_update_dpp(0, (int)v, 0x118, 0xf, 0xf, false);
+    v |= (uint32_t)__builtin_amdgcn_update_dpp(0, (int)v, 0x142, 0xa, 0xf, false);
+    v |= (uint32_t)__builtin_amdgcn_update_dpp(0, (int)v, 0x143, 0xc, 0xf, false);
+    return (uint32_t)__builtin_amdgcn_readlane((int)v, 63);
+}
+
+template <int LB, class Src>
+__device__ __forceinline__ void shadow_group([[maybe_unused]] const RgKernelArgs &a, const Src &src, V3 o, const ShadowBatch<LB> &sb,
+                                             const int (&idx)[RG_SHADOW_GROUP], int g, uint32_t &occl) {
+    constexpr int G = RG_SHADOW_GROUP;
+    RG_REGION(RGR_SH_GROUP);
+    RgSph s[G];
+    double hx[G], hy[G], hz[G], hh[G], adj[G][LB], opp[G][LB];
+    bool cand[G][LB];
+    bool any = false;
+#pragma unroll
+    for (int k = 0; k < G; ++k) {
+        if (k < g) {
+            s[k] = src.get(idx[k]);
+            hx[k] = s[k].cx - o.x; hy[k] = s[k].cy - o.y; hz[k] = s[k].cz - o.z;
+            hh[k] = (hx[k] * hx[k] + hy[k] * hy[k]) + hz[k] * hz[k];
+#pragma unroll
+            for (int l = 0; l < LB; ++l) {
+                adj[k][l] = (hx[k] * sb.d[l].x + hy[k] * sb.d[l].y) + hz[k] * sb.d[l].z;
+                opp[k][l] = hh[k] - adj[k][l] * adj[k][l];
+                cand[k][l] = !(opp[k][l] > s[k].r2) && !((occl >> l) & 1u);
+                any |= cand[k][l];
+            }
+        }
+    }
+    if (any) {
+        RG_REGION(RGR_SH_TAIL);
+#pragma unroll
+        for (int k = 0; k < G; ++k) {
+#pragma unroll
+            for (int l = 0; l < LB; ++l) {
+                double t;
+#ifdef RG_REGION_STATS
+                if (k < g && cand[k][l]) RG_REGION(RGR_SH_PAIR);
+#endif
+                if (k < g && cand[k][l] && sphere_tail(s[k].r2, opp[k][l], adj[k][l], t) && !(t > sb.ld[l]))
+                    occl |= 1u << l;
+            }
+        }
+    }
+}
+
+template <int LB, bool NODB = false, bool SHV = false, class Src>
 __device__ __forceinline__ void trace_shadow(const RgKernelArgs &a, const Src &src, V3 o, const ShadowBatch<LB> &sb,
-                                             uint32_t full, uint32_t &occl) {
+                                             uint32_t full, uint32_t &occl, [[maybe_unused]] uint32_t smask = ~0u,
+                                             [[maybe_unused]] uint32_t pmask = ~0u) {
     constexpr int G = RG_SHADOW_GROUP;
-    const int n = a.n_sph, nfull = n - n % G;
+    const int n = a.n_sph;
+    if constexpr (SHV && RG_PLAIN_SHVOL_SPHERES != 0) {
+        for (int base = 0; base < n; base += 32) {
+            const uint32_t lim = n - base >= 32 ? ~0u : (1u << (n - base)) - 1u;
+            uint32_t left = base == 0 ? smask & lim : lim;
+            for (int ng = 1; left != 0u; ++ng) {
+                int idx[G], g = 0;
+#pragma unroll
+                for (int k = 0; k < G; ++k) {
+                    idx[k] = 0;
+                    if (left != 0u) {
+                        idx[k] = base + __builtin_ctz(left);
+                        left &= left - 1u;
+                        g = k + 1;
+                    }
+                }
+                shadow_group<LB>(a, src, o, sb, idx, g, occl);
+                if ((ng & 3) == 0 && !__any(occl != full)) return;
+            }
+        }
+    } else {
+    const int nfull = n - n % G;
     for (int i = 0; i < n;) {
         const int g = i < nfull ? G : 1;
         RG_REGION(RGR_SH_GROUP);
@@ -226,8 +300,12 @@
         i += g;
         if ((i & 7) == 0 && !__any(occl != full)) return;
     }
+    }
     if (!__any(occl != full)) return;
     for (int i = 0; i < a.n_pln; ++i) {
+        if constexpr (SHV && RG_PLAIN_SHVOL_PLANES != 0) {
+            if (i < RG_SHVOL_MAX_BODIES && !((pmask >> i) & 1u)) continue;
+        }
         const RgPln p = src.getp(i);
         const double vx = p.ox - o.x, vy = p.oy - o.y, vz = p.oz - o.z;
         const double num = (vx * p.nx + vy * p.ny) + vz * p.nz;
diff --git a/raingun_amd/csrc/rg_launch.hip b/raingun_amd/csrc/rg_launch.hip
--- a/raingun_amd/csrc/rg_launch.hip
+++ b/raingun_amd/csrc/rg_launch.hip
@@ -204,6 +204,7 @@
     a.snap_out = snap_dev;
     if (a.out_rows > 0) {
         if (!ok(rg_launch_render(&a, disp, st, &cx->last_plain))) return RG_ERR_DEVICE;
+        cx->last_shvol = cx->last_plain && a.shvol != nullptr;
         cx->cur = 1 - cx->cur;
     }
     if (d.timed && !ok(hipEventRecord(cx->ev1, st))) return RG_ERR_DEVICE;
diff --git a/raingun_amd/csrc/rg_render_kernel.h b/raingun_amd/csrc/rg_render_kernel.h
--- a/raingun_amd/csrc/rg_render_kernel.h
+++ b/raingun_amd/csrc/rg_render_kernel.h
@@ -13,6 +13,7 @@
 #include "rg_k_shade.h"
 #include "rg_k_trace.h"
 #include "rg_render_cfg.h"
+#include "rg_shadow_vol_cell.h"
 
 #pragma clang fp contract(off)
 
@@ -50,6 +51,7 @@
     using K = RenderCfg<MAXD, LSPH, LCOLD, WPS, LBT, F32F, BVH, TASKS, TPW, HF, SPARSE, PLAIN>;
     constexpr int LB = K::lights_per_batch;
     constexpr bool UL = PLAIN && RG_PLAIN_ULIGHT != 0;
+    constexpr bool SHV = PLAIN && RG_PLAIN_SHVOL != 0;
 #ifdef RG_WAVE_TIMES
     const unsigned long long t_wave0 = wall_clock64();
     uint32_t wt_tiles = 0;
@@ -203,6 +205,7 @@
     Ray q;
     ShadowBatch<LB> sb;
     uint32_t occl_full = 0u;
+    [[maybe_unused]] uint32_t shw = 0u;
     int qdepth = 0;
     V3 hp = v3(0, 0, 0), hn = v3(0, 0, 0);
     int hb = 0, hdepth = 0, li = 0;
@@ -283,6 +286,15 @@
                             park[64 * PK_KIND] = __int_as_float(kind);
                             park[64 * PK_R] = m.reflectivity;
                             q.o = add(h, scl(n, SHADOW_BIAS));
+                            if constexpr (SHV) {
+                                shw = RG_SHVOL_ALL;
+                                if (a.shvol) {
+                                    const int cell = rg_shvol_cell((float)q.o.x, (float)q.o.y, (float)q.o.z, a.shvol_inv,
+                                                                   a.shvol_off, (int)a.shvol_g);
+                                    const uint32_t w = a.shvol[cell >= 0 ? cell : 0];
+                                    if (cell >= 0) shw = w;
+                                }
+                            }
                             if (kind == 2) q.d = sub(q.d, scl(n, 2.0 * dot(q.d, n)));
                             occl_full = 0u;
 #pragma unroll
@@ -847,10 +859,18 @@
                     }
                 }
             }
+            [[maybe_unused]] uint32_t smask = ~0u, pmask = ~0u;
+            if constexpr (SHV) {
+                if (a.shvol) {
+                    const uint32_t wm = wave_or(mode == MODE_SHADOW && !exact ? shw : 0u);
+                    smask = wm & 0xFFFFu;
+                    pmask = wm >> 16;
+                }
+            }
             if (mode == MODE_SHADOW && !exact) {
                 RG_REGION(RGR_Q_SHADOW);
                 occl = ~occl_full & ((1u << LB) - 1u);
-                trace_shadow<LB, PLAIN>(a, src, q.o, sb, (1u << LB) - 1u, occl);
+                trace_shadow<LB, PLAIN, SHV>(a, src, q.o, sb, (1u << LB) - 1u, occl, smask, pmask);
             }
         }
 #ifdef RG_TILE_TIMES
diff --git a/raingun_amd/csrc/rg_scene.hip b/raingun_amd/csrc/rg_scene.hip
--- a/raingun_amd/csrc/rg_scene.hip
+++ b/raingun_amd/csrc/rg_scene.hip
@@ -14,6 +14,7 @@
 #include "rg_device.h"
 #include "rg_exact.h"
 #include "rg_lightbuf.h"
+#include "rg_shadow_vol.h"
 #include "rg_internal.h"
 
 #pragma clang fp contract(off)
@@ -104,6 +105,7 @@
     RG_UP(lbuf, lbuf);
     RG_UP(lb_start, lb_start);
     RG_UP(lb_ent, lb_ent);
+    RG_UP(shvol, shvol);
 #undef RG_UP
     std::vector<RgTexDev> texs(h.tex_w.size());
     for (size_t i = 0; st == RG_OK && i < texs.size(); ++i) {
@@ -142,6 +144,9 @@
     dst->bvh_margin = src->bvh_margin;
     dst->bvh_extent = src->bvh_extent;
     dst->bvh_info = src->bvh_info;
+    dst->shvol_info = src->shvol_info;
+    dst->shvol_inv = src->shvol_inv;
+    dst->shvol_off = src->shvol_off;
 }
 
 }
@@ -215,6 +220,11 @@
     a.max_depth = s->max_depth;
     a.fov_adjustment = fov_adjustment(s->fov);
     a.tile_wlog = 3;
+    const bool shvol = RG_PLAIN_SHVOL != 0 && s->shvol_enabled && s->shvol != nullptr;
+    a.shvol = shvol ? s->shvol : nullptr;
+    a.shvol_g = shvol ? (uint32_t)s->shvol_info.g : 0u;
+    a.shvol_inv = s->shvol_inv;
+    a.shvol_off = s->shvol_off;
     return a;
 }
 
@@ -305,6 +315,7 @@
     dst->path = src->path;
     dst->bvh_enabled = src->bvh_enabled;
     dst->lbuf_enabled = src->lbuf_enabled;
+    dst->shvol_enabled = src->shvol_enabled;
     dst->exact_div = src->exact_div;
     dst->has_camera = src->has_camera;
     dst->camera = src->camera;
@@ -489,6 +500,35 @@
         s->bvh_info.lbuf_bytes = (int64_t)((h.lb_ent.size() + h.lb_start.size()) * sizeof(uint32_t) +
                                            h.lbuf.size() * sizeof(RgLightBufDev));
     }
+    if (RG_PLAIN_SHVOL != 0 && h.dsk.empty() && h.box.empty() && !nan_scene) {
+        std::vector<double> sp(sph_raw);
+        for (size_t j = 0; !h.nodes.empty() && j < h.sph.size(); ++j)
+            std::memcpy(&sp[4 * j], &sph_raw[4 * (size_t)bvh.order[j]], 4 * sizeof(double));
+        std::vector<double> pl(6 * h.pln.size());
+        for (size_t j = 0; j < h.pln.size(); ++j) {
+            const RgPln &p = h.pln[j];
+            const double v[6] = {p.ox, p.oy, p.oz, p.nx, p.ny, p.nz};
+            std::memcpy(&pl[6 * j], v, sizeof v);
+        }
+        std::vector<RgShadowVolLight> ls(h.lights.size());
+        for (size_t l = 0; l < ls.size(); ++l) {
+            ls[l].kind = h.lights[l].kind;
+            std::memcpy(ls[l].v, h.lights[l].v, sizeof ls[l].v);
+            std::memcpy(ls[l].dn, h.lights[l].dn, sizeof ls[l].dn);
+        }
+        RgShadowVolBuild sv;
+        if (rg_build_shadow_vol(sp.data(), (int)h.sph.size(), pl.data(), (int)h.pln.size(), ls.data(), (int)ls.size(),
+                                RG_SHVOL_G, sv)) {
+            s->shvol_info.built = 1;
+            s->shvol_info.g = sv.g;
+            s->shvol_info.bytes = (int64_t)(sv.words.size() * sizeof(uint32_t));
+            s->shvol_info.build_ms = sv.build_ms;
+            s->shvol_info.set_share = sv.set_share;
+            s->shvol_inv = sv.inv;
+            s->shvol_off = sv.off;
+            h.shvol = std::move(sv.words);
+        }
+    }
     h.tex_w.resize(d->n_textures);
     h.tex_h.resize(d->n_textures);
     h.texels.resize(d->n_textures);
diff --git a/raingun_amd/csrc/rg_shadow_vol.cpp b/raingun_amd/csrc/rg_shadow_vol.cpp
--- /dev/null
+++ b/raingun_amd/csrc/rg_shadow_vol.cpp
@@ -0,0 +1,144 @@
+#if defined(__HIP__)
+#include <hip/hip_runtime.h>
+#endif
+#include "rg_shadow_vol.h"
+
+#include <algorithm>
+#include <chrono>
+#include <cmath>
+
+#include "../../include/raingun.h"
+#include "rg_device.h"
+
+namespace {
+
+double dot3(const double *a, const double *b) { return (a[0] * b[0] + a[1] * b[1]) + a[2] * b[2]; }
+
+double seg_dist2(const double *c, const double *b, const double *L) {
+    const double p[3] = {c[0] - b[0], c[1] - b[1], c[2] - b[2]};
+    const double e[3] = {L[0] - b[0], L[1] - b[1], L[2] - b[2]};
+    const double ee = dot3(e, e);
+    double t = ee > 0.0 ? dot3(p, e) / ee : 0.0;
+    t = std::min(std::max(t, 0.0), 1.0);
+    const double w[3] = {p[0] - t * e[0], p[1] - t * e[1], p[2] - t * e[2]};
+    return dot3(w, w);
+}
+
+double ray_dist2(const double *c, const double *b, const double *d) {
+    const double p[3] = {c[0] - b[0], c[1] - b[1], c[2] - b[2]};
+    const double t = std::max(dot3(p, d) / dot3(d, d), 0.0);
+    const double w[3] = {p[0] - t * d[0], p[1] - t * d[1], p[2] - t * d[2]};
+    return dot3(w, w);
+}
+
+bool small_finite(double v) { return std::isfinite(v) && std::fabs(v) <= RG_SHVOL_MAX_MAG; }
+
+#ifdef RG_SHVOL_TEST_NO_MARGIN
+constexpr double kShrink = 0.99, kMargin = 0.0;
+#else
+constexpr double kShrink = 1.0, kMargin = 1.0;
+#endif
+
+}
+
+bool rg_shadow_vol_admits(const double *spheres, int n_sph, const double *planes, int n_pln,
+                          const RgShadowVolLight *lights, int n_lights) {
+    if (n_sph < 0 || n_pln < 0 || n_sph + n_pln < 1 || n_sph > RG_SHVOL_MAX_BODIES || n_pln > RG_SHVOL_MAX_BODIES)
+        return false;
+    if (n_lights < 1 || n_lights > RG_LB) return false;
+    for (int i = 0; i < 4 * n_sph; ++i)
+        if (!small_finite(spheres[i])) return false;
+    for (int i = 0; i < 6 * n_pln; ++i)
+        if (!small_finite(planes[i])) return false;
+    for (int l = 0; l < n_lights; ++l)
+        for (int k = 0; k < 3; ++k) {
+            if (!small_finite(lights[l].v[k])) return false;
+            if (lights[l].kind == RG_LIGHT_DIRECTIONAL && !small_finite(lights[l].dn[k])) return false;
+        }
+    return true;
+}
+
+bool rg_build_shadow_vol(const double *spheres, int n_sph, const double *planes, int n_pln,
+                         const RgShadowVolLight *lights, int n_lights, int g, RgShadowVolBuild &out) {
+    out = RgShadowVolBuild();
+    if (g < 1 || g > RG_SHVOL_MAX_G || !rg_shadow_vol_admits(spheres, n_sph, planes, n_pln, lights, n_lights))
+        return false;
+    const auto t0 = std::chrono::steady_clock::now();
+    double S = 0.0;
+    for (int i = 0; i < n_sph; ++i) {
+        const double *p = spheres + 4 * i, r = std::fabs(p[3]);
+        for (int k = 0; k < 3; ++k) S = std::max(S, std::max(std::fabs(p[k] - r), std::fabs(p[k] + r)));
+    }
+    const double O = 4.0 * S + 1.0;
+    const double m = kMargin * 1.52587890625e-05 * (S + O);
+    const double e = 2.0 * O / (double)g;
+    const double rho = kShrink * e * 0.8660254037844387;
+    constexpr int B = 8;
+    const double rho_block = rho + (double)(B - 1) * e * 0.8660254037844387;
+
+    uint32_t plane_all = 0u;
+    struct PlanePair { int j; double nl[3], thr; };
+    std::vector<PlanePair> cellwise;
+    for (int j = 0; j < n_pln; ++j) {
+        const double *po = planes + 6 * j, *n = po + 3;
+        const double N = std::sqrt(dot3(n, n));
+        for (int l = 0; l < n_lights; ++l) {
+            const RgShadowVolLight &L = lights[l];
+            if (L.kind == RG_LIGHT_DIRECTIONAL) {
+                const double den = (n[0] * L.dn[0] + n[1] * L.dn[1]) + n[2] * L.dn[2];
+                if (den > 1e-6) plane_all |= 1u << (16 + j);
+                continue;
+            }
+            if (!(N > 0.0)) continue;
+            const double v[3] = {po[0] - L.v[0], po[1] - L.v[1], po[2] - L.v[2]};
+            if (dot3(n, v) / N >= m) continue;
+            cellwise.push_back(PlanePair{j, {n[0] / N, n[1] / N, n[2] / N}, dot3(n, L.v) / N + rho + m});
+        }
+    }
+
+    out.words.assign((size_t)g * g * g, plane_all);
+    struct Pair { int i, l; };
+    std::vector<Pair> live;
+    live.reserve((size_t)n_sph * n_lights);
+    auto centre = [&](int k) { return -O + ((double)k + 0.5) * e; };
+    auto sphere_near = [&](int i, int l, const double *b, double reach) {
+        const double *c = spheres + 4 * i;
+        const RgShadowVolLight &L = lights[l];
+        const double thr = kShrink * std::fabs(c[3]) + reach + 2.0 * m;
+        const double d2 = L.kind == RG_LIGHT_DIRECTIONAL ? ray_dist2(c, b, L.dn) : seg_dist2(c, b, L.v);
+        return d2 <= thr * thr;
+    };
+    for (int bz = 0; bz < g; bz += B)
+        for (int by = 0; by < g; by += B)
+            for (int bx = 0; bx < g; bx += B) {
+                const double bb[3] = {-O + ((double)bx + 0.5 * B) * e, -O + ((double)by + 0.5 * B) * e,
+                                      -O + ((double)bz + 0.5 * B) * e};
+                live.clear();
+                for (int i = 0; i < n_sph; ++i)
+                    for (int l = 0; l < n_lights; ++l)
+                        if (sphere_near(i, l, bb, rho_block)) live.push_back(Pair{i, l});
+                if (live.empty() && cellwise.empty()) continue;
+                for (int z = bz; z < std::min(bz + B, g); ++z)
+                    for (int y = by; y < std::min(by + B, g); ++y)
+                        for (int x = bx; x < std::min(bx + B, g); ++x) {
+                            const double b[3] = {centre(x), centre(y), centre(z)};
+                            uint32_t w = 0u;
+                            for (const Pair &p : live)
+                                if (!((w >> p.i) & 1u) && sphere_near(p.i, p.l, b, rho)) w |= 1u << p.i;
+                            for (const PlanePair &p : cellwise)
+                                if (!(dot3(p.nl, b) >= p.thr)) w |= 1u << (16 + p.j);
+                            out.words[((size_t)z * g + y) * g + x] |= w;
+                        }
+            }
+    unsigned long long set = 0;
+    for (uint32_t w : out.words) set += (unsigned long long)__builtin_popcount(w);
+    out.g = g;
+    out.inv = (float)((double)g / (2.0 * O));
+    out.off = 0.5f * (float)g;
+    out.extent = S;
+    out.obound = O;
+    out.margin = m;
+    out.set_share = (double)set / ((double)out.words.size() * (double)(n_sph + n_pln));
+    out.build_ms = std::chrono::duration<double, std::milli>(std::chrono::steady_clock::now() - t0).count();
+    return true;
+}
diff --git a/raingun_amd/csrc/rg_shadow_vol.h b/raingun_amd/csrc/rg_shadow_vol.h
--- /dev/null
+++ b/raingun_amd/csrc/rg_shadow_vol.h
@@ -0,0 +1,32 @@
+#pragma once
+#include <cstdint>
+#include <vector>
+
+#include "rg_shadow_vol_cell.h"
+
+#ifndef RG_SHVOL_G
+#define RG_SHVOL_G 64
+#endif
+#define RG_SHVOL_MAX_G 256
+#define RG_SHVOL_MAX_MAG 1048576.0
+
+struct RgShadowVolLight {
+    int kind;
+    double v[3];
+    double dn[3];
+};
+
+struct RgShadowVolBuild {
+    std::vector<uint32_t> words;
+    int g = 0;
+    float inv = 0.0f, off = 0.0f;
+    double extent = 0.0, obound = 0.0, margin = 0.0;
+    double build_ms = 0.0;
+    double set_share = 0.0;
+};
+
+bool rg_shadow_vol_admits(const double *spheres, int n_sph, const double *planes, int n_pln,
+                          const RgShadowVolLight *lights, int n_lights);
+
+bool rg_build_shadow_vol(const double *spheres, int n_sph, const double *planes, int n_pln,
+                         const RgShadowVolLight *lights, int n_lights, int g, RgShadowVolBuild &out);
diff --git a/raingun_amd/csrc/rg_shadow_vol_cell.h b/raingun_amd/csrc/rg_shadow_vol_cell.h
--- /dev/null
+++ b/raingun_amd/csrc/rg_shadow_vol_cell.h
@@ -0,0 +1,20 @@
+#pragma once
+#include <stdint.h>
+
+#if defined(__HIP__) || defined(__HIPCC__)
+#define RG_SHVOL_FN __host__ __device__ __forceinline__
+#else
+#define RG_SHVOL_FN inline
+#endif
+
+#define RG_SHVOL_NO_CELL (-1)
+#define RG_SHVOL_ALL 0xFFFFFFFFu
+#define RG_SHVOL_MAX_BODIES 16
+
+RG_SHVOL_FN int rg_shvol_cell(float ox, float oy, float oz, float inv, float off, int g) {
+    const float fx = __builtin_fmaf(ox, inv, off), fy = __builtin_fmaf(oy, inv, off), fz = __builtin_fmaf(oz, inv, off);
+    const float fg = (float)g;
+    const bool in = fx >= 0.0f && fx < fg && fy >= 0.0f && fy < fg && fz >= 0.0f && fz < fg;
+    if (!in) return RG_SHVOL_NO_CELL;
+    return ((int)fz * g + (int)fy) * g + (int)fx;
+}
diff --git a/raingun_amd/scene.py b/raingun_amd/scene.py
--- a/raingun_amd/scene.py
+++ b/raingun_amd/scene.py
@@ -275,6 +275,20 @@
         _abi.check(_abi.lib().rg_debug_last_plain(self.handle, C.byref(plain)))
         return plain.value == 1
 
+    def set_shadow_volume(self, on: bool) -> None:
+        _abi.check(_abi.lib().rg_debug_set_shadow_volume(self.handle, 1 if on else 0))
+
+    def shadow_volume_info(self) -> dict:
+        info = _abi.rg_shadow_volume_info()
+        _abi.check(_abi.lib().rg_debug_shadow_volume_info(self.handle, C.byref(info)))
+        return {"built": bool(info.built), "enabled": bool(info.enabled), "g": info.g, "bytes": info.bytes,
+                "build_ms": info.build_ms, "set_share": info.set_share}
+
+    def last_shadow_volume(self) -> bool:
+        used = C.c_int32(-1)
+        _abi.check(_abi.lib().rg_debug_last_shadow_volume(self.handle, C.byref(used)))
+        return used.value == 1
+
     def set_exact_div(self, enable: bool) -> None:
         _abi.check(_abi.lib().rg_debug_set_exact_div(self.handle, 1 if enable else 0))
 
```
